# Gnnng/SVDFeature

Hardware: AMD Instinct MI355X
Metric: training instances/sec (SGD updates/s), basicMF k=64 (higher is better)
Workload: dtype f32; 1 GPU; basicMF synthetic 1000000x100000, 100000000 ratings, k=64 fp32 (BASELINE configs[1]); order=uniform random (file order preserved: result == sequential SGD), conflict_free_batches_per_pass=903, parallelism=1 GPU

## Files before the change

include/svdfeature_amd.h:

```cpp
#ifndef SVDFEATURE_AMD_H_
#define SVDFEATURE_AMD_H_

#include <stddef.h>
#include <stdint.h>
#include <stdio.h>

#ifdef __cplusplus
extern "C" {
#endif

typedef struct svdf_trainer svdf_trainer;
typedef struct svdf_dataset svdf_dataset;
typedef struct svdf_ranker svdf_ranker;

const char *svdf_version(void);
void svdf_set_error_mode(int mode);
const char *svdf_last_error(void);
int svdf_device_count(void);

svdf_trainer *svdf_create(uint8_t format_type, uint8_t active_type, uint8_t extend_type, uint8_t variant_type,
                          int device);
void svdf_destroy(svdf_trainer *t);

int svdf_set_param(svdf_trainer *t, const char *name, const char *val);
void svdf_seed(unsigned seed);
int svdf_init_model(svdf_trainer *t);
int svdf_load_model(svdf_trainer *t, FILE *fi);
int svdf_save_model(svdf_trainer *t, FILE *fo);
int svdf_save_model_begin(svdf_trainer *t, FILE *fo);
int svdf_save_model_end(svdf_trainer *t);
int svdf_init_trainer(svdf_trainer *t);
int svdf_set_round(svdf_trainer *t, int nround);
int svdf_finish_round(svdf_trainer *t);

int svdf_update_csr(svdf_trainer *t, float label, int num_global, int num_ufactor, int num_ifactor,
                    const unsigned *index, const float *value);
float svdf_predict_csr(svdf_trainer *t, float label, int num_global, int num_ufactor, int num_ifactor,
                       const unsigned *index, const float *value);
int svdf_update_csr_batch(svdf_trainer *t, int num_row, const float *row_label, const int *row_ptr,
                          const unsigned *feat_index, const float *feat_value);
int svdf_predict_csr_batch(svdf_trainer *t, int num_row, const float *row_label, const int *row_ptr,
                           const unsigned *feat_index, const float *feat_value, float *out);

int svdf_update_block(svdf_trainer *t, int num_ufeedback, int extend_tag,
                      const unsigned *index_ufeedback, const float *value_ufeedback,
                      int num_row, const float *row_label, const int *row_ptr,
                      const unsigned *feat_index, const float *feat_value);
int svdf_predict_block(svdf_trainer *t, int num_ufeedback, int extend_tag,
                       const unsigned *index_ufeedback, const float *value_ufeedback,
                       int num_row, const float *row_label, const int *row_ptr,
                       const unsigned *feat_index, const float *feat_value, float *out);

svdf_dataset *svdf_dataset_from_csr(svdf_trainer *t, long num_row, const float *row_label, const int64_t *row_ptr,
                                    const unsigned *feat_index, const float *feat_value);
svdf_dataset *svdf_dataset_from_triples(svdf_trainer *t, long n, const unsigned *user, const unsigned *item,
                                        const float *label);
svdf_dataset *svdf_dataset_from_pairs(svdf_trainer *t, long n, const unsigned *user, const unsigned *pos_item,
                                      const unsigned *neg_item);
svdf_dataset *svdf_dataset_from_blocks(svdf_trainer *t, long num_block, const int *extend_tag, const int64_t *fb_ptr,
                                       const unsigned *fb_index, const float *fb_value, const int64_t *block_row_ptr,
                                       const float *row_label, const int64_t *row_ptr, const unsigned *feat_index,
                                       const float *feat_value);
svdf_dataset *svdf_dataset_from_buffer_file(svdf_trainer *t, const char *path, int user_group_format);
svdf_dataset *svdf_dataset_from_rank_buffer_file(svdf_trainer *t, const char *path);
int svdf_rank_prefetch_buffer_file(svdf_trainer *t, const char *path);
int64_t svdf_rank_sample_buffer_file(svdf_trainer *t, const char *in_path, const char *out_path);
void svdf_dataset_destroy(svdf_dataset *ds);
int svdf_train_dataset(svdf_trainer *t, svdf_dataset *ds);
int svdf_predict_dataset(svdf_trainer *t, svdf_dataset *ds, float *out);
int64_t svdf_dataset_info(const svdf_dataset *ds, int what);

int svdf_item_delta_begin(svdf_trainer *t);
void *svdf_item_delta_buffer(svdf_trainer *t, int64_t *count);
int svdf_item_delta_apply(svdf_trainer *t);
int svdf_item_delta_export(svdf_trainer *t, float *device_dst);
int svdf_item_delta_import(svdf_trainer *t, const float *device_src);
int svdf_item_delta_into(svdf_trainer *t, float *device_dst, int64_t *count);
int svdf_item_delta_apply_from(svdf_trainer *t, const float *device_src);
int svdf_item_delta_pack(svdf_trainer *t, void *device_dst, int half, int64_t *count);
int svdf_item_delta_select(svdf_trainer *t, int part, int nparts);
int svdf_item_delta_unpack(svdf_trainer *t, const void *device_src, int half, int refresh_snapshot);

svdf_dataset *svdf_dataset_window_from_triples(svdf_trainer *t, long n, const unsigned *user, const unsigned *item, const float *label);
svdf_dataset *svdf_dataset_window_from_pairs(svdf_trainer *t, long n, const unsigned *user, const unsigned *pos_item, const unsigned *neg_item);
svdf_dataset *svdf_dataset_window_from_csr(svdf_trainer *t, long num_row, const float *row_label, const int64_t *row_ptr,
                                           const unsigned *feat_index, const float *feat_value);
svdf_dataset *svdf_dataset_window_from_blocks(svdf_trainer *t, long num_block, const int *extend_tag, const int64_t *fb_ptr,
                                              const unsigned *fb_index, const float *fb_value, const int64_t *block_row_ptr,
                                              const float *row_label, const int64_t *row_ptr, const unsigned *feat_index,
                                              const float *feat_value);
int svdf_window_delta_pack(svdf_trainer *t, svdf_dataset *ds, void *device_dst, int half, int64_t *count);
int svdf_window_delta_apply(svdf_trainer *t, const void *device_src, int half);
int svdf_window_delta_apply_local(svdf_trainer *t, svdf_dataset *ds);
int svdf_item_block_get(svdf_trainer *t, float *device_dst, int64_t *count);
int svdf_item_block_set(svdf_trainer *t, const float *device_src);
int svdf_stratum_step(svdf_trainer *t, svdf_dataset *const *windows, int num_windows, int block, int nblocks, float *device_out);
int svdf_item_block_set_at(svdf_trainer *t, int block, int nblocks, const float *device_src);
int svdf_ipc_setup(svdf_trainer *t, int rank, int world, int64_t wire_bytes, int64_t block_floats, unsigned char *handles_out);
int svdf_ipc_connect(svdf_trainer *t, const unsigned char *all_handles);
int svdf_ipc_window_pack(svdf_trainer *t, svdf_dataset *ds, int half);
int svdf_ipc_window_reduce(svdf_trainer *t, int half);
int svdf_ipc_window_apply(svdf_trainer *t, int half);
int svdf_ipc_block_send(svdf_trainer *t, int dst_rank, int slot);
int svdf_ipc_block_recv(svdf_trainer *t, int src_rank, int slot, unsigned seq);
int svdf_ipc_status(svdf_trainer *t);
int svdf_ipc_close(svdf_trainer *t);

int svdf_rccl_unique_id(unsigned char *out128);
int svdf_rccl_init(svdf_trainer *t, const unsigned char *id128, int rank, int world);
int svdf_rccl_window_allreduce(svdf_trainer *t, svdf_dataset *ds, int half);
int svdf_rccl_block_handoff(svdf_trainer *t, int dst_rank, int src_rank, int slot, int in_block, int nblocks);
int svdf_rccl_block_arrive(svdf_trainer *t, int slot);
int64_t svdf_rccl_counter(svdf_trainer *t, int what);
int svdf_rccl_close(svdf_trainer *t);

int svdf_debug_sort_labels(long n, const float *label, int *restated, int *library);
int svdf_debug_sort_scores(long n, const float *score, int threads, int *parallel, int *library);

int64_t svdf_get_view(svdf_trainer *t, int which, float *out, int64_t capacity);
int svdf_view_shape(svdf_trainer *t, int which, int *rows, int *cols);
int64_t svdf_set_view(svdf_trainer *t, int which, const float *in, int64_t count);
void *svdf_stream(svdf_trainer *t);
int svdf_set_stream(svdf_trainer *t, void *hip_stream);
int svdf_synchronize(svdf_trainer *t);
int64_t svdf_counter(svdf_trainer *t, int what);
int svdf_set_knob(svdf_trainer *t, const char *name, long value);

int svdf_eval_dataset(svdf_trainer *t, svdf_dataset *ds, float scale_score, double *sum_sq_err, int64_t *count);

svdf_ranker *svdf_ranker_create(uint8_t format_type, uint8_t active_type, uint8_t extend_type, uint8_t variant_type, int device);
void svdf_ranker_destroy(svdf_ranker *r);
int svdf_ranker_set_param(svdf_ranker *r, const char *name, const char *val);
int svdf_ranker_load_model(svdf_ranker *r, FILE *fi);
int svdf_ranker_init(svdf_ranker *r, int num_item_set);
int64_t svdf_ranker_process_csr(svdf_ranker *r, float label, int num_global, int num_ufactor, int num_ifactor, const unsigned *index,
                                const float *value, int *out, int64_t capacity);
int64_t svdf_ranker_process_rows(svdf_ranker *r, int num_row, const float *row_label, const int *row_ptr, const unsigned *feat_index,
                                 const float *feat_value, int *out, int64_t capacity);
int64_t svdf_ranker_process_block(svdf_ranker *r, int num_ufeedback, int extend_tag, const unsigned *index_ufeedback,
                                  const float *value_ufeedback, int num_row, const float *row_label, const int *row_ptr,
                                  const unsigned *feat_index, const float *feat_value, int *out, int64_t capacity);
int64_t svdf_ranker_counter(svdf_ranker *r, int what);

int svdf_rand_peek(long n, int *out);
int svdf_rand_skip(long n);

int svdf_device_expf(const float *in, unsigned first_bits, unsigned step_bits, float *out, long n);

int svdf_schedule_resources(long n, const int64_t *res_ptr, const unsigned *res, long num_res, int *order_out,
                            int64_t *level_ptr_out, long level_cap);

#ifdef __cplusplus
}
#endif
#endif
```

svdfeature_amd/__init__.py:

```python
import ctypes as C
import os

import numpy as np

from .data import BlockArrays, CSRData, PlusBlock, pairs_as_csr

HERE = os.path.dirname(os.path.abspath(__file__))
LIB_PATH = os.path.join(HERE, "libsvdfeature_amd.so")
HEADER_PATH = os.path.join(os.path.dirname(HERE), "include", "svdfeature_amd.h")

VIEW = {"u_bias": 0, "W_user": 1, "i_bias": 2, "W_item": 3, "g_bias": 4, "ufeedback_bias": 5, "W_ufeedback": 6}

_u32p = np.ctypeslib.ndpointer(dtype=np.uint32, flags="C_CONTIGUOUS")
_i32p = np.ctypeslib.ndpointer(dtype=np.int32, flags="C_CONTIGUOUS")
_i64p = np.ctypeslib.ndpointer(dtype=np.int64, flags="C_CONTIGUOUS")
_f32p = np.ctypeslib.ndpointer(dtype=np.float32, flags="C_CONTIGUOUS")

_lib = None
_libc = C.CDLL(None)
_libc.fopen.restype = C.c_void_p
_libc.fopen.argtypes = [C.c_char_p, C.c_char_p]
_libc.fclose.argtypes = [C.c_void_p]


class SvdfError(RuntimeError):
    pass


def load_library():
    global _lib
    if _lib is not None:
        return _lib
    if not os.path.exists(LIB_PATH):
        raise SvdfError("%s is missing: run `python -c 'import __graft_entry__ as g; g.build()'` "
                        "(hipcc --offload-arch=gfx950); there is no CPU fallback" % LIB_PATH)
    try:
        import torch
    except ImportError:
        pass
    lib = C.CDLL(LIB_PATH)
    P = C.c_void_p
    lib.svdf_version.restype = C.c_char_p
    lib.svdf_last_error.restype = C.c_char_p
    lib.svdf_set_error_mode.argtypes = [C.c_int]
    lib.svdf_device_count.restype = C.c_int
    lib.svdf_create.restype = P
    lib.svdf_create.argtypes = [C.c_uint8] * 4 + [C.c_int]
    lib.svdf_destroy.argtypes = [P]
    lib.svdf_set_param.argtypes = [P, C.c_char_p, C.c_char_p]
    lib.svdf_seed.argtypes = [C.c_uint]
    for f in ("svdf_init_model", "svdf_init_trainer", "svdf_finish_round", "svdf_synchronize",
              "svdf_item_delta_begin", "svdf_item_delta_apply"):
        getattr(lib, f).argtypes = [P]
    lib.svdf_set_round.argtypes = [P, C.c_int]
    lib.svdf_load_model.argtypes = [P, C.c_void_p]
    lib.svdf_save_model.argtypes = [P, C.c_void_p]
    lib.svdf_save_model_begin.argtypes = [P, C.c_void_p]
    lib.svdf_save_model_end.argtypes = [P]
    lib.svdf_update_csr.argtypes = [P, C.c_float, C.c_int, C.c_int, C.c_int, _u32p, _f32p]
    lib.svdf_predict_csr.argtypes = lib.svdf_update_csr.argtypes
    lib.svdf_predict_csr.restype = C.c_float
    lib.svdf_update_csr_batch.argtypes = [P, C.c_int, _f32p, _i32p, _u32p, _f32p]
    lib.svdf_predict_csr_batch.argtypes = [P, C.c_int, _f32p, _i32p, _u32p, _f32p, _f32p]
    lib.svdf_update_block.argtypes = [P, C.c_int, C.c_int, _u32p, _f32p, C.c_int, _f32p, _i32p, _u32p, _f32p]
    lib.svdf_predict_block.argtypes = lib.svdf_update_block.argtypes + [_f32p]
    lib.svdf_dataset_from_csr.restype = P
    lib.svdf_dataset_from_csr.argtypes = [P, C.c_long, _f32p, _i64p, _u32p, _f32p]
    lib.svdf_dataset_from_triples.restype = P
    lib.svdf_dataset_from_triples.argtypes = [P, C.c_long, _u32p, _u32p, _f32p]
    lib.svdf_dataset_from_pairs.restype = P
    lib.svdf_dataset_from_pairs.argtypes = [P, C.c_long, _u32p, _u32p, _u32p]
    lib.svdf_dataset_window_from_triples.restype = P
    lib.svdf_dataset_window_from_triples.argtypes = [P, C.c_long, _u32p, _u32p, _f32p]
    lib.svdf_dataset_window_from_pairs.restype = P
    lib.svdf_dataset_window_from_pairs.argtypes = [P, C.c_long, _u32p, _u32p, _u32p]
    lib.svdf_dataset_window_from_csr.restype = P
    lib.svdf_dataset_window_from_csr.argtypes = [P, C.c_long, _f32p, _i64p, _u32p, _f32p]
    lib.svdf_dataset_window_from_blocks.restype = P
    lib.svdf_dataset_window_from_blocks.argtypes = [P, C.c_long, _i32p, _i64p, _u32p, _f32p, _i64p, _f32p, _i64p, _u32p, _f32p]
    lib.svdf_ipc_setup.argtypes = [P, C.c_int, C.c_int, C.c_int64, C.c_int64, C.c_char_p]
    lib.svdf_ipc_connect.argtypes = [P, C.c_char_p]
    lib.svdf_ipc_window_pack.argtypes = [P, P, C.c_int]
    lib.svdf_ipc_window_reduce.argtypes = [P, C.c_int]
    lib.svdf_ipc_window_apply.argtypes = [P, C.c_int]
    lib.svdf_ipc_block_send.argtypes = [P, C.c_int, C.c_int]
    lib.svdf_ipc_block_recv.argtypes = [P, C.c_int, C.c_int, C.c_uint]
    lib.svdf_ipc_status.argtypes = [P]
    lib.svdf_ipc_close.argtypes = [P]
    lib.svdf_stratum_step.argtypes = [P, C.POINTER(C.c_void_p), C.c_int, C.c_int, C.c_int, P]
    lib.svdf_item_block_set_at.argtypes = [P, C.c_int, C.c_int, P]
    lib.svdf_rccl_unique_id.argtypes = [C.c_char_p]
    lib.svdf_rccl_init.argtypes = [P, C.c_char_p, C.c_int, C.c_int]
    lib.svdf_rccl_window_allreduce.argtypes = [P, P, C.c_int]
    lib.svdf_rccl_block_handoff.argtypes = [P, C.c_int, C.c_int, C.c_int, C.c_int, C.c_int]
    lib.svdf_rccl_block_arrive.argtypes = [P, C.c_int]
    lib.svdf_rccl_counter.restype = C.c_int64
    lib.svdf_rccl_counter.argtypes = [P, C.c_int]
    lib.svdf_rccl_close.argtypes = [P]
    lib.svdf_window_delta_pack.argtypes = [P, P, P, C.c_int, C.POINTER(C.c_int64)]
    lib.svdf_window_delta_apply.argtypes = [P, P, C.c_int]
    lib.svdf_window_delta_apply_local.argtypes = [P, P]
    lib.svdf_item_block_get.argtypes = [P, P, C.POINTER(C.c_int64)]
    lib.svdf_item_block_set.argtypes = [P, P]
    lib.svdf_set_view.restype = C.c_int64
    lib.svdf_set_view.argtypes = [P, C.c_int, _f32p, C.c_int64]
    lib.svdf_dataset_from_buffer_file.restype = P
    lib.svdf_dataset_from_buffer_file.argtypes = [P, C.c_char_p, C.c_int]
    lib.svdf_dataset_from_rank_buffer_file.restype = P
    lib.svdf_dataset_from_rank_buffer_file.argtypes = [P, C.c_char_p]
    lib.svdf_rank_prefetch_buffer_file.restype = C.c_int
    lib.svdf_rank_prefetch_buffer_file.argtypes = [P, C.c_char_p]
    lib.svdf_rank_sample_buffer_file.restype = C.c_int64
    lib.svdf_rank_sample_buffer_file.argtypes = [P, C.c_char_p, C.c_char_p]
    lib.svdf_dataset_from_blocks.restype = P
    lib.svdf_dataset_from_blocks.argtypes = [P, C.c_long, _i32p, _i64p, _u32p, _f32p, _i64p, _f32p, _i64p, _u32p, _f32p]
    lib.svdf_dataset_destroy.argtypes = [P]
    lib.svdf_train_dataset.argtypes = [P, P]
    lib.svdf_predict_dataset.argtypes = [P, P, _f32p]
    lib.svdf_dataset_info.restype = C.c_int64
    lib.svdf_dataset_info.argtypes = [P, C.c_int]
    lib.svdf_item_delta_buffer.restype = P
    lib.svdf_item_delta_buffer.argtypes = [P, C.POINTER(C.c_int64)]
    lib.svdf_item_delta_export.argtypes = [P, P]
    lib.svdf_item_delta_import.argtypes = [P, P]
    lib.svdf_item_delta_into.argtypes = [P, P, C.POINTER(C.c_int64)]
    lib.svdf_item_delta_apply_from.argtypes = [P, P]
    lib.svdf_item_delta_pack.argtypes = [P, P, C.c_int, C.POINTER(C.c_int64)]
    lib.svdf_item_delta_unpack.argtypes = [P, P, C.c_int, C.c_int]
    lib.svdf_set_stream.argtypes = [P, P]
    lib.svdf_item_delta_select.argtypes = [P, C.c_int, C.c_int]
    lib.svdf_get_view.restype = C.c_int64
    lib.svdf_get_view.argtypes = [P, C.c_int, _f32p, C.c_int64]
    lib.svdf_view_shape.argtypes = [P, C.c_int, C.POINTER(C.c_int), C.POINTER(C.c_int)]
    lib.svdf_stream.restype = P
    lib.svdf_stream.argtypes = [P]
    lib.svdf_counter.restype = C.c_int64
    lib.svdf_counter.argtypes = [P, C.c_int]
    lib.svdf_set_knob.argtypes = [P, C.c_char_p, C.c_long]
    lib.svdf_schedule_resources.argtypes = [C.c_long, _i64p, _u32p, C.c_long, _i32p, _i64p, C.c_long]
    lib.svdf_eval_dataset.argtypes = [P, P, C.c_float, C.POINTER(C.c_double), C.POINTER(C.c_int64)]
    lib.svdf_ranker_create.restype = P
    lib.svdf_ranker_create.argtypes = [C.c_uint8] * 4 + [C.c_int]
    lib.svdf_ranker_destroy.argtypes = [P]
    lib.svdf_ranker_set_param.argtypes = [P, C.c_char_p, C.c_char_p]
    lib.svdf_ranker_load_model.argtypes = [P, C.c_void_p]
    lib.svdf_ranker_init.argtypes = [P, C.c_int]
    lib.svdf_ranker_process_csr.restype = C.c_int64
    lib.svdf_ranker_process_csr.argtypes = [P, C.c_float, C.c_int, C.c_int, C.c_int, _u32p, _f32p, _i32p, C.c_int64]
    lib.svdf_ranker_process_rows.restype = C.c_int64
    lib.svdf_ranker_process_rows.argtypes = [P, C.c_int, _f32p, _i32p, _u32p, _f32p, _i32p, C.c_int64]
    lib.svdf_ranker_process_block.restype = C.c_int64
    lib.svdf_ranker_process_block.argtypes = [P, C.c_int, C.c_int, _u32p, _f32p, C.c_int, _f32p, _i32p, _u32p, _f32p, _i32p, C.c_int64]
    lib.svdf_ranker_counter.restype = C.c_int64
    lib.svdf_ranker_counter.argtypes = [P, C.c_int]
    lib.svdf_rand_peek.argtypes = [C.c_long, _i32p]
    lib.svdf_rand_skip.argtypes = [C.c_long]
    lib.svdf_device_expf.argtypes = [C.c_void_p, C.c_uint, C.c_uint, _f32p, C.c_long]
    lib.svdf_debug_sort_labels.argtypes = [C.c_long, _f32p, _i32p, _i32p]
    lib.svdf_debug_sort_scores.argtypes = [C.c_long, _f32p, C.c_int, _i32p, _i32p]
    lib.svdf_set_error_mode(1)
    _lib = lib
    return lib


def device_count():
    return load_library().svdf_device_count()


def rccl_unique_id():
    buf = C.create_string_buffer(128)
    if load_library().svdf_rccl_unique_id(buf) != 0:
        raise SvdfError(load_library().svdf_last_error().decode())
    return buf.raw


def rand_peek(n):
    out = np.zeros(max(int(n), 1), np.int32)
    if load_library().svdf_rand_peek(int(n), out) != 0:
        raise SvdfError(load_library().svdf_last_error().decode())
    return out[:n]


def rand_skip(n):
    if load_library().svdf_rand_skip(int(n)) != 0:
        raise SvdfError(load_library().svdf_last_error().decode())


def debug_sort_labels(label):
    label = np.ascontiguousarray(label, np.float32)
    a, b = np.zeros(max(len(label), 1), np.int32), np.zeros(max(len(label), 1), np.int32)
    if load_library().svdf_debug_sort_labels(len(label), _pad(label, np.float32), a, b) != 0:
        raise SvdfError(load_library().svdf_last_error().decode())
    return a[:len(label)], b[:len(label)]


def debug_sort_scores(score, threads=8):
    score = np.ascontiguousarray(score, np.float32)
    a, b = np.zeros(max(len(score), 1), np.int32), np.zeros(max(len(score), 1), np.int32)
    if load_library().svdf_debug_sort_scores(len(score), _pad(score, np.float32), int(threads), a, b) != 0:
        raise SvdfError(load_library().svdf_last_error().decode())
    return a[:len(score)], b[:len(score)]


def device_expf(x=None, first=0, step=1, n=None):
    lib = load_library()
    if x is not None:
        x = np.ascontiguousarray(x, np.float32)
        out = np.empty(len(x), np.float32)
        rc = lib.svdf_device_expf(x.ctypes.data_as(C.c_void_p), 0, 0, out, len(x))
    else:
        out = np.empty(n, np.float32)
        rc = lib.svdf_device_expf(None, first, step, out, n)
    if rc != 0:
        raise SvdfError("svdf_device_expf failed")
    return out


def _pad(a, dtype):
    a = np.ascontiguousarray(a, dtype=dtype)
    return a if a.size else np.zeros(1, dtype=dtype)


def schedule_resources(res_ptr, res, num_res):
    lib = load_library()
    n = len(res_ptr) - 1
    order = np.zeros(max(n, 1), np.int32)
    level_ptr = np.zeros(n + 2, np.int64)
    nl = lib.svdf_schedule_resources(n, _pad(res_ptr, np.int64), _pad(res, np.uint32), int(num_res), order, level_ptr, n + 2)
    if nl < 0:
        raise SvdfError(lib.svdf_last_error().decode())
    return order[:n], level_ptr[:nl + 1]


class Dataset:

    def __init__(self, trainer, handle):
        self.trainer, self.h = trainer, handle

    def info(self, what):
        return int(self.trainer.lib.svdf_dataset_info(self.h, what))

    num_row = property(lambda s: s.info(0))
    num_batches = property(lambda s: s.info(1))
    max_batch = property(lambda s: s.info(2))
    kind = property(lambda s: s.info(3))
    algorithmic_bytes = property(lambda s: s.info(4))
    num_units = property(lambda s: s.info(5))
    num_simple_units = property(lambda s: s.info(6))

    def close(self):
        if self.h:
            self.trainer.lib.svdf_dataset_destroy(self.h)
            self.h = None

    def __del__(self):
        try:
            self.close()
        except Exception:
            pass


class Trainer:

    def __init__(self, format_type=0, active_type=0, extend_type=0, variant_type=0, params=None, device=-1):
        self.lib = load_library()
        self.h = self.lib.svdf_create(format_type, active_type, extend_type, variant_type, device)
        if not self.h:
            raise SvdfError(self.lib.svdf_last_error().decode())
        self.mtype = bytes([format_type, active_type, extend_type, variant_type])
        for k, v in (params or {}).items():
            self.set_param(k, v)

    def _ok(self, rc):
        if rc != 0:
            raise SvdfError(self.lib.svdf_last_error().decode())

    def close(self):
        if getattr(self, "h", None):
            if getattr(self, "_async_fo", None) is not None:
                try:
                    self.save_model_end()
                except Exception:
                    pass
            self.lib.svdf_destroy(self.h)
            self.h = None

    def __del__(self):
        try:
            self.close()
        except Exception:
            pass

    def set_param(self, name, val):
        self._ok(self.lib.svdf_set_param(self.h, str(name).encode(), str(val).encode()))

    def seed(self, s):
        self.lib.svdf_seed(int(s))

    def init_model(self):
        self._ok(self.lib.svdf_init_model(self.h))

    def init_trainer(self):
        self._ok(self.lib.svdf_init_trainer(self.h))

    def set_round(self, r):
        self._ok(self.lib.svdf_set_round(self.h, int(r)))

    def finish_round(self):
        self._ok(self.lib.svdf_finish_round(self.h))

    def save_model_begin(self, path, with_type_header=True):
        assert getattr(self, "_async_fo", None) is None, "one asynchronous save at a time"
        fo = _libc.fopen(str(path).encode(), b"wb")
        if not fo:
            raise SvdfError("can not open file \"%s\"" % path)
        if with_type_header:
            hdr = (C.c_char * 4).from_buffer_copy(self.mtype)
            _libc.fwrite(hdr, 1, 4, C.c_void_p(fo))
        self._async_fo = fo
        try:
            self._ok(self.lib.svdf_save_model_begin(self.h, fo))
        except Exception:
            _libc.fclose(fo)
            self._async_fo = None
            raise

    def save_model_end(self):
        fo = getattr(self, "_async_fo", None)
        if fo is None:
            return
        try:
            self._ok(self.lib.svdf_save_model_end(self.h))
        finally:
            _libc.fclose(fo)
            self._async_fo = None

    def save_model(self, path, with_type_header=True):
        fo = _libc.fopen(str(path).encode(), b"wb")
        if not fo:
            raise SvdfError("can not open file \"%s\"" % path)
        try:
            if with_type_header:
                hdr = (C.c_char * 4).from_buffer_copy(self.mtype)
                _libc.fwrite(hdr, 1, 4, C.c_void_p(fo))
            self._ok(self.lib.svdf_save_model(self.h, fo))
        finally:
            _libc.fclose(fo)

    def load_model(self, path, with_type_header=True):
        fi = _libc.fopen(str(path).encode(), b"rb")
        if not fi:
            raise SvdfError("can not open file \"%s\"" % path)
        try:
            if with_type_header:
                buf = (C.c_char * 4)()
                _libc.fread(buf, 1, 4, C.c_void_p(fi))
            self._ok(self.lib.svdf_load_model(self.h, fi))
        finally:
            _libc.fclose(fi)

    def update_csr(self, label, ng, nu, ni, index, value):
        self._ok(self.lib.svdf_update_csr(self.h, float(label), ng, nu, ni, _pad(index, np.uint32), _pad(value, np.float32)))

    def predict_csr(self, label, ng, nu, ni, index, value):
        self.lib.svdf_last_error()
        return self.lib.svdf_predict_csr(self.h, float(label), ng, nu, ni, _pad(index, np.uint32), _pad(value, np.float32))

    def update_batch(self, d):
        self._ok(self.lib.svdf_update_csr_batch(self.h, d.num_row, _pad(d.row_label, np.float32), _pad(d.row_ptr, np.int32),
                                                _pad(d.feat_index, np.uint32), _pad(d.feat_value, np.float32)))

    def predict_batch(self, d):
        out = np.zeros(max(d.num_row, 1), dtype=np.float32)
        self._ok(self.lib.svdf_predict_csr_batch(self.h, d.num_row, _pad(d.row_label, np.float32), _pad(d.row_ptr, np.int32),
                                                 _pad(d.feat_index, np.uint32), _pad(d.feat_value, np.float32), out))
        return out[:d.num_row]

    def update_block(self, b):
        d = b.data
        self._ok(self.lib.svdf_update_block(self.h, b.num_ufeedback, b.extend_tag, _pad(b.index_ufeedback, np.uint32),
                                            _pad(b.value_ufeedback, np.float32), d.num_row, _pad(d.row_label, np.float32),
                                            _pad(d.row_ptr, np.int32), _pad(d.feat_index, np.uint32), _pad(d.feat_value, np.float32)))

    def predict_block(self, b):
        d = b.data
        out = np.zeros(max(d.num_row, 1), dtype=np.float32)
        self._ok(self.lib.svdf_predict_block(self.h, b.num_ufeedback, b.extend_tag, _pad(b.index_ufeedback, np.uint32),
                                             _pad(b.value_ufeedback, np.float32), d.num_row, _pad(d.row_label, np.float32),
                                             _pad(d.row_ptr, np.int32), _pad(d.feat_index, np.uint32), _pad(d.feat_value, np.float32), out))
        return out[:d.num_row]

    def dataset_from_csr(self, d):
        h = self.lib.svdf_dataset_from_csr(self.h, d.num_row, _pad(d.row_label, np.float32), _pad(d.row_ptr, np.int64),
                                           _pad(d.feat_index, np.uint32), _pad(d.feat_value, np.float32))
        if not h:
            raise SvdfError(self.lib.svdf_last_error().decode())
        return Dataset(self, h)

    def dataset_from_triples(self, user, item, label):
        n = len(label)
        h = self.lib.svdf_dataset_from_triples(self.h, n, _pad(user, np.uint32), _pad(item, np.uint32), _pad(label, np.float32))
# ... 321 lines not shown
```

svdfeature_amd/csrc/svdf_capi.cpp:

```cpp
#include <svdfeature_amd.h>

#include <algorithm>
#include <cstdlib>
#include <cstring>
#include <new>
#include <vector>

#include "svdf_engine.h"
#include "svdf_kernels.h"

namespace svdf {
void set_error_mode(int m);
const char *last_error();
void note_error(const std::string &m);
}

struct svdf_trainer { svdf::Engine *e; };
struct svdf_dataset { svdf::Dataset *d; };
struct svdf_ranker { svdf::Ranker *r; };

#define SVDF_GUARD(retval, ...)                                 \
    try { __VA_ARGS__; }                                        \
    catch (const std::exception &ex) { svdf::note_error(ex.what()); return retval; } \
    catch (...) { svdf::note_error("unknown error"); return retval; }

extern "C" {

const char *svdf_version(void) { return "svdfeature_amd 0.1 (gfx950)"; }
void svdf_set_error_mode(int mode) { svdf::set_error_mode(mode); }
const char *svdf_last_error(void) { return svdf::last_error(); }
int svdf_device_count(void) {
    int n = 0;
    if (hipGetDeviceCount(&n) != hipSuccess) return 0;
    return n;
}

svdf_trainer *svdf_create(uint8_t format_type, uint8_t active_type, uint8_t extend_type, uint8_t variant_type, int device) {
    SVDF_GUARD(nullptr, {
        svdf::TypeParam tp{format_type, active_type, extend_type, variant_type};
        svdf_trainer *t = new svdf_trainer();
        t->e = nullptr;
        try { t->e = new svdf::Engine(tp, device); } catch (...) { delete t; throw; }
        return t;
    })
}
void svdf_destroy(svdf_trainer *t) {
    if (!t) return;
    try { delete t->e; } catch (...) {}
    delete t;
}
int svdf_set_param(svdf_trainer *t, const char *name, const char *val) { SVDF_GUARD(-1, { t->e->set_param(name, val); return 0; }) }
void svdf_seed(unsigned seed) { srand(seed); }
int svdf_init_model(svdf_trainer *t) { SVDF_GUARD(-1, { t->e->init_model(); return 0; }) }
int svdf_load_model(svdf_trainer *t, FILE *fi) { SVDF_GUARD(-1, { t->e->load_model(fi); return 0; }) }
int svdf_save_model(svdf_trainer *t, FILE *fo) { SVDF_GUARD(-1, { t->e->save_model(fo); return 0; }) }
int svdf_save_model_begin(svdf_trainer *t, FILE *fo) { SVDF_GUARD(-1, { t->e->save_model_begin(fo); return 0; }) }
int svdf_save_model_end(svdf_trainer *t) { SVDF_GUARD(-1, { t->e->save_model_end(); return 0; }) }
int svdf_init_trainer(svdf_trainer *t) { SVDF_GUARD(-1, { t->e->init_trainer(); return 0; }) }
int svdf_set_round(svdf_trainer *t, int nround) { SVDF_GUARD(-1, { t->e->set_round(nround); return 0; }) }
int svdf_finish_round(svdf_trainer *t) { SVDF_GUARD(-1, { t->e->finish_round(); return 0; }) }

int svdf_update_csr(svdf_trainer *t, float label, int ng, int nu, int ni, const unsigned *index, const float *value) {
    SVDF_GUARD(-1, { t->e->update_csr(label, ng, nu, ni, index, value); return 0; })
}
float svdf_predict_csr(svdf_trainer *t, float label, int ng, int nu, int ni, const unsigned *index, const float *value) {
    SVDF_GUARD(0.0f, { return t->e->predict_csr(label, ng, nu, ni, index, value); })
}
int svdf_update_csr_batch(svdf_trainer *t, int num_row, const float *row_label, const int *row_ptr,
                          const unsigned *feat_index, const float *feat_value) {
    SVDF_GUARD(-1, { t->e->update_csr_batch(num_row, row_label, row_ptr, feat_index, feat_value); return 0; })
}
int svdf_predict_csr_batch(svdf_trainer *t, int num_row, const float *row_label, const int *row_ptr,
                           const unsigned *feat_index, const float *feat_value, float *out) {
    SVDF_GUARD(-1, { t->e->predict_csr_batch(num_row, row_label, row_ptr, feat_index, feat_value, out); return 0; })
}
int svdf_update_block(svdf_trainer *t, int nfb, int tag, const unsigned *ifb, const float *vfb, int num_row,
                      const float *row_label, const int *row_ptr, const unsigned *feat_index, const float *feat_value) {
    SVDF_GUARD(-1, { t->e->update_block(nfb, tag, ifb, vfb, num_row, row_label, row_ptr, feat_index, feat_value); return 0; })
}
int svdf_predict_block(svdf_trainer *t, int nfb, int tag, const unsigned *ifb, const float *vfb, int num_row,
                       const float *row_label, const int *row_ptr, const unsigned *feat_index, const float *feat_value, float *out) {
    SVDF_GUARD(-1, { t->e->predict_block(nfb, tag, ifb, vfb, num_row, row_label, row_ptr, feat_index, feat_value, out); return 0; })
}

svdf_dataset *svdf_dataset_from_csr(svdf_trainer *t, long num_row, const float *row_label, const int64_t *row_ptr,
                                    const unsigned *feat_index, const float *feat_value) {
    SVDF_GUARD(nullptr, {
        svdf::Dataset *d = t->e->dataset_from_csr(num_row, row_label, row_ptr, feat_index, feat_value);
        t->e->note_dataset(d);
        svdf_dataset *h = new svdf_dataset();
        h->d = d;
        return h;
    })
}
svdf_dataset *svdf_dataset_from_triples(svdf_trainer *t, long n, const unsigned *user, const unsigned *item, const float *label) {
    SVDF_GUARD(nullptr, {
        svdf::Dataset *d = t->e->dataset_from_triples(n, user, item, label);
        t->e->note_dataset(d);
        svdf_dataset *h = new svdf_dataset();
        h->d = d;
        return h;
    })
}
svdf_dataset *svdf_dataset_window_from_triples(svdf_trainer *t, long n, const unsigned *user, const unsigned *item, const float *label) {
    SVDF_GUARD(nullptr, {
        svdf::Dataset *d = t->e->dataset_window_from_triples(n, user, item, label);
        svdf_dataset *h = new svdf_dataset();
        h->d = d;
        return h;
    })
}
svdf_dataset *svdf_dataset_window_from_pairs(svdf_trainer *t, long n, const unsigned *user, const unsigned *pos_item, const unsigned *neg_item) {
    SVDF_GUARD(nullptr, {
        svdf::Dataset *d = t->e->dataset_window_from_pairs(n, user, pos_item, neg_item);
        svdf_dataset *h = new svdf_dataset();
        h->d = d;
        return h;
    })
}
svdf_dataset *svdf_dataset_window_from_csr(svdf_trainer *t, long num_row, const float *row_label, const int64_t *row_ptr, const unsigned *feat_index,
                                           const float *feat_value) {
    SVDF_GUARD(nullptr, {
        svdf::Dataset *d = t->e->dataset_window_from_csr(num_row, row_label, row_ptr, feat_index, feat_value);
        svdf_dataset *h = new svdf_dataset();
        h->d = d;
        return h;
    })
}
svdf_dataset *svdf_dataset_window_from_blocks(svdf_trainer *t, long num_block, const int *extend_tag, const int64_t *fb_ptr, const unsigned *fb_index,
                                              const float *fb_value, const int64_t *block_row_ptr, const float *row_label, const int64_t *row_ptr,
                                              const unsigned *feat_index, const float *feat_value) {
    SVDF_GUARD(nullptr, {
        svdf::Dataset *d = t->e->dataset_window_from_blocks(num_block, extend_tag, fb_ptr, fb_index, fb_value, block_row_ptr, row_label, row_ptr, feat_index, feat_value);
        svdf_dataset *h = new svdf_dataset();
        h->d = d;
        return h;
    })
}
int svdf_ipc_setup(svdf_trainer *t, int rank, int world, int64_t wire_bytes, int64_t block_floats, unsigned char *handles_out) { SVDF_GUARD(-1, { t->e->ipc_setup(rank, world, wire_bytes, block_floats, handles_out); return 0; }) }
int svdf_ipc_connect(svdf_trainer *t, const unsigned char *all_handles) { SVDF_GUARD(-1, { t->e->ipc_connect(all_handles); return 0; }) }
int svdf_ipc_window_pack(svdf_trainer *t, svdf_dataset *ds, int half) { SVDF_GUARD(-1, { t->e->ipc_window_pack(ds ? ds->d : nullptr, half); return 0; }) }
int svdf_ipc_window_reduce(svdf_trainer *t, int half) { SVDF_GUARD(-1, { t->e->ipc_window_reduce(half); return 0; }) }
int svdf_ipc_window_apply(svdf_trainer *t, int half) { SVDF_GUARD(-1, { t->e->ipc_window_apply(half); return 0; }) }
int svdf_ipc_block_send(svdf_trainer *t, int dst_rank, int slot) { SVDF_GUARD(-1, { t->e->ipc_block_send(dst_rank, slot); return 0; }) }
int svdf_ipc_block_recv(svdf_trainer *t, int src_rank, int slot, unsigned seq) { SVDF_GUARD(-1, { t->e->ipc_block_recv(src_rank, slot, seq); return 0; }) }
int svdf_ipc_status(svdf_trainer *t) { SVDF_GUARD(-1, { return t->e->ipc_status(); }) }
int svdf_ipc_close(svdf_trainer *t) { SVDF_GUARD(-1, { t->e->ipc_close(); return 0; }) }
int svdf_rccl_unique_id(unsigned char *out128) { SVDF_GUARD(-1, { svdf::rccl_unique_id(out128); return 0; }) }
int svdf_rccl_init(svdf_trainer *t, const unsigned char *id128, int rank, int world) { SVDF_GUARD(-1, { t->e->rccl_init(id128, rank, world); return 0; }) }
int svdf_rccl_window_allreduce(svdf_trainer *t, svdf_dataset *ds, int half) { SVDF_GUARD(-1, { t->e->rccl_window_allreduce(ds ? ds->d : nullptr, half); return 0; }) }
int svdf_rccl_block_handoff(svdf_trainer *t, int dst_rank, int src_rank, int slot, int in_block, int nblocks) { SVDF_GUARD(-1, { t->e->rccl_block_handoff(dst_rank, src_rank, slot, in_block, nblocks); return 0; }) }
int svdf_rccl_block_arrive(svdf_trainer *t, int slot) { SVDF_GUARD(-1, { t->e->rccl_block_arrive(slot); return 0; }) }
int64_t svdf_rccl_counter(svdf_trainer *t, int what) { SVDF_GUARD(-1, { return t->e->rccl_counter(what); }) }
int svdf_rccl_close(svdf_trainer *t) { SVDF_GUARD(-1, { t->e->rccl_close(); return 0; }) }
int svdf_window_delta_pack(svdf_trainer *t, svdf_dataset *ds, void *dst, int half, int64_t *count) {
    SVDF_GUARD(-1, { t->e->per_rank_api(); t->e->window_delta_pack(ds ? ds->d : nullptr, dst, half, count); return 0; })
}
int svdf_window_delta_apply_local(svdf_trainer *t, svdf_dataset *ds) { SVDF_GUARD(-1, { t->e->per_rank_api(); t->e->window_delta_apply_local(ds ? ds->d : nullptr); return 0; }) }
int svdf_item_block_get(svdf_trainer *t, float *dst, int64_t *count) { SVDF_GUARD(-1, { t->e->per_rank_api(); t->e->item_block_copy(dst, 0, count); return 0; }) }
int svdf_stratum_step(svdf_trainer *t, svdf_dataset *const *windows, int num_windows, int block, int nblocks, float *device_out) {
    SVDF_GUARD(-1, {
        t->e->per_rank_api();
// ... 37 lines not shown
        return h;
    })
}
svdf_dataset *svdf_dataset_from_blocks(svdf_trainer *t, long num_block, const int *extend_tag, const int64_t *fb_ptr,
                                       const unsigned *fb_index, const float *fb_value, const int64_t *block_row_ptr,
                                       const float *row_label, const int64_t *row_ptr, const unsigned *feat_index,
                                       const float *feat_value) {
    SVDF_GUARD(nullptr, {
        svdf::Dataset *d = t->e->dataset_from_blocks(num_block, extend_tag, fb_ptr, fb_index, fb_value, block_row_ptr, row_label, row_ptr,
                                                     feat_index, feat_value);
        t->e->note_dataset(d);
        svdf_dataset *h = new svdf_dataset();
        h->d = d;
        return h;
    })
}
svdf_dataset *svdf_dataset_from_buffer_file(svdf_trainer *t, const char *path, int user_group_format) {
    SVDF_GUARD(nullptr, {
        svdf::Dataset *d = t->e->dataset_from_buffer_file(path, user_group_format);
        t->e->note_dataset(d);
        svdf_dataset *h = new svdf_dataset();
        h->d = d;
        return h;
    })
}
svdf_dataset *svdf_dataset_from_rank_buffer_file(svdf_trainer *t, const char *path) {
    SVDF_GUARD(nullptr, {
        svdf::Dataset *d = t->e->dataset_from_rank_buffer_file(path);
        t->e->note_dataset(d);
        svdf_dataset *h = new svdf_dataset();
        h->d = d;
        return h;
    })
}
int svdf_rank_prefetch_buffer_file(svdf_trainer *t, const char *path) { SVDF_GUARD(-1, { t->e->rank_prefetch(path); return 0; }) }
int64_t svdf_rank_sample_buffer_file(svdf_trainer *t, const char *in_path, const char *out_path) {
    SVDF_GUARD(-1, { return (int64_t)t->e->rank_sample_buffer_file(in_path, out_path); })
}
void svdf_dataset_destroy(svdf_dataset *ds) {
    if (!ds) return;
    try { if (ds->d && ds->d->owner) ds->d->owner->synchronize(); } catch (...) {}
    delete ds->d;
    delete ds;
}
int svdf_train_dataset(svdf_trainer *t, svdf_dataset *ds) { SVDF_GUARD(-1, { t->e->train_dataset(ds->d); return 0; }) }
int svdf_predict_dataset(svdf_trainer *t, svdf_dataset *ds, float *out) { SVDF_GUARD(-1, { t->e->predict_dataset(ds->d, out); return 0; }) }
int64_t svdf_dataset_info(const svdf_dataset *ds, int what) {
    if (!ds || !ds->d) return -1;
    switch (what) {
    case 0: return ds->d->num_row;
    case 1: return ds->d->kind == 8 ? (int64_t)ds->d->wchild.size() : (int64_t)ds->d->sched.num_levels();
    case 2: return ds->d->sched.max_level_size;
    case 3: return ds->d->kind;
    case 4: return ds->d->algorithmic_bytes;
    case 5: return ds->d->num_units;
    case 6: return ds->d->num_simple_units;
    case 7: {
        uint64_t h = 1469598103934665603ull;
        auto mix = [&h](uint64_t v) { for (int b = 0; b < 8; b++) { h ^= (v >> (8 * b)) & 0xFFu; h *= 1099511628211ull; } };
        for (long v : ds->d->sched.level_ptr) mix((uint64_t)v);
        for (long v : ds->d->sched.level_mid) mix((uint64_t)v);
        for (int v : ds->d->sched.order) mix((uint64_t)(unsigned)v);
        return (int64_t)(h >> 1);
    }
    default: return -1;
    }
}

int svdf_item_delta_begin(svdf_trainer *t) { SVDF_GUARD(-1, { t->e->per_rank_api(); t->e->item_delta_begin(); return 0; }) }
void *svdf_item_delta_buffer(svdf_trainer *t, int64_t *count) { SVDF_GUARD(nullptr, { t->e->per_rank_api(); return t->e->item_delta_buffer(count); }) }
int svdf_item_delta_apply(svdf_trainer *t) { SVDF_GUARD(-1, { t->e->per_rank_api(); t->e->item_delta_apply(); return 0; }) }
int svdf_item_delta_export(svdf_trainer *t, float *dst) { SVDF_GUARD(-1, { t->e->per_rank_api(); t->e->item_delta_copy(dst, nullptr); return 0; }) }
int svdf_item_delta_import(svdf_trainer *t, const float *src) { SVDF_GUARD(-1, { t->e->per_rank_api(); t->e->item_delta_copy(nullptr, src); return 0; }) }

int svdf_item_delta_into(svdf_trainer *t, float *dst, int64_t *count) { SVDF_GUARD(-1, { t->e->per_rank_api(); t->e->item_delta_into(dst, count); return 0; }) }
int svdf_item_delta_pack(svdf_trainer *t, void *dst, int half, int64_t *count) { SVDF_GUARD(-1, { t->e->per_rank_api(); t->e->item_delta_pack(dst, half, count); return 0; }) }
int svdf_item_delta_unpack(svdf_trainer *t, const void *src, int half, int refresh_snapshot) {
    SVDF_GUARD(-1, { t->e->per_rank_api(); t->e->item_delta_unpack(src, half, refresh_snapshot); return 0; })
}
int svdf_item_delta_select(svdf_trainer *t, int part, int nparts) { SVDF_GUARD(-1, { t->e->per_rank_api(); t->e->item_delta_select(part, nparts); return 0; }) }
int svdf_item_delta_apply_from(svdf_trainer *t, const float *src) { SVDF_GUARD(-1, { t->e->per_rank_api(); t->e->item_delta_apply_from(src); return 0; }) }
int svdf_set_stream(svdf_trainer *t, void *hip_stream) { SVDF_GUARD(-1, { t->e->set_stream((hipStream_t)hip_stream); return 0; }) }

int64_t svdf_get_view(svdf_trainer *t, int which, float *out, int64_t capacity) { SVDF_GUARD(-1, { return t->e->get_view(which, out, capacity); }) }
int64_t svdf_set_view(svdf_trainer *t, int which, const float *in, int64_t count) { SVDF_GUARD(-1, { return t->e->set_view(which, in, count); }) }
int svdf_view_shape(svdf_trainer *t, int which, int *rows, int *cols) { SVDF_GUARD(-1, { t->e->view_shape(which, rows, cols); return 0; }) }
void *svdf_stream(svdf_trainer *t) { return (void *)t->e->stream(); }
int svdf_synchronize(svdf_trainer *t) { SVDF_GUARD(-1, { t->e->synchronize(); return 0; }) }
int64_t svdf_counter(svdf_trainer *t, int what) { return t->e->counter(what); }
int svdf_set_knob(svdf_trainer *t, const char *name, long value) { SVDF_GUARD(-1, { return t->e->set_knob(name, value); }) }

int svdf_eval_dataset(svdf_trainer *t, svdf_dataset *ds, float scale_score, double *sum_sq_err, int64_t *count) {
    SVDF_GUARD(-1, { t->e->eval_dataset(ds->d, scale_score, sum_sq_err, count); return 0; })
}

svdf_ranker *svdf_ranker_create(uint8_t format_type, uint8_t active_type, uint8_t extend_type, uint8_t variant_type, int device) {
    SVDF_GUARD(nullptr, {
        svdf::TypeParam tp{format_type, active_type, extend_type, variant_type};
        svdf_ranker *h = new svdf_ranker();
        h->r = nullptr;
        try { h->r = new svdf::Ranker(tp, device); } catch (...) { delete h; throw; }
        return h;
    })
}
void svdf_ranker_destroy(svdf_ranker *r) {
    if (!r) return;
    try { delete r->r; } catch (...) {}
    delete r;
}
int svdf_ranker_set_param(svdf_ranker *r, const char *name, const char *val) { SVDF_GUARD(-1, { r->r->set_param(name, val); return 0; }) }
int svdf_ranker_load_model(svdf_ranker *r, FILE *fi) { SVDF_GUARD(-1, { r->r->load_model(fi); return 0; }) }
int svdf_ranker_init(svdf_ranker *r, int num_item_set) { SVDF_GUARD(-1, { r->r->init_ranker(num_item_set); return 0; }) }
int64_t svdf_ranker_process_csr(svdf_ranker *r, float label, int ng, int nu, int ni, const unsigned *index, const float *value, int *out,
                                int64_t capacity) {
    SVDF_GUARD(-1, { return (int64_t)r->r->process(label, ng, nu, ni, index, value, out, (long)capacity); })
}
int64_t svdf_ranker_process_rows(svdf_ranker *r, int num_row, const float *row_label, const int *row_ptr, const unsigned *feat_index,
                                 const float *feat_value, int *out, int64_t capacity) {
    SVDF_GUARD(-1, { return (int64_t)r->r->process_rows(num_row, row_label, row_ptr, feat_index, feat_value, out, (long)capacity); })
}
int64_t svdf_ranker_process_block(svdf_ranker *r, int nfb, int tag, const unsigned *ifb, const float *vfb, int num_row, const float *row_label,
                                  const int *row_ptr, const unsigned *feat_index, const float *feat_value, int *out, int64_t capacity) {
    SVDF_GUARD(-1, { return (int64_t)r->r->process_block(nfb, tag, ifb, vfb, num_row, row_label, row_ptr, feat_index, feat_value, out, (long)capacity); })
}
int64_t svdf_ranker_counter(svdf_ranker *r, int what) { return r->r->counter(what); }

int svdf_rand_peek(long n, int *out) { SVDF_GUARD(-1, { svdf::libc_rand_peek(n, out); return 0; }) }
int svdf_rand_skip(long n) { SVDF_GUARD(-1, { svdf::libc_rand_skip(n); return 0; }) }

int svdf_device_expf(const float *in, unsigned first_bits, unsigned step_bits, float *out, long n) {
    SVDF_GUARD(-1, { return svdf::device_expf(in, first_bits, step_bits, out, n); })
}

int svdf_schedule_resources(long n, const int64_t *res_ptr, const unsigned *res, long num_res, int *order_out,
                            int64_t *level_ptr_out, long level_cap) {
    SVDF_GUARD(-1, {
        std::vector<int> last((size_t)num_res, 0), levels((size_t)n);
        for (long r = 0; r < n; r++) {
            int l = 0;
            for (int64_t j = res_ptr[r]; j < res_ptr[r + 1]; j++) l = std::max(l, last[res[j]]);
            l += 1;
            for (int64_t j = res_ptr[r]; j < res_ptr[r + 1]; j++) last[res[j]] = l;
            levels[(size_t)r] = l;
        }
        svdf::Schedule s;
        svdf::build_schedule(levels, 0, s);
        if ((long)s.num_levels() + 1 > level_cap) return -2;
        for (long r = 0; r < n; r++) order_out[r] = s.order[(size_t)r];
        for (size_t l = 0; l <= s.num_levels(); l++) level_ptr_out[l] = s.level_ptr[l];
        return (int)s.num_levels();
    })
}

}
```

svdfeature_amd/csrc/svdf_config.cpp:

```cpp
#include "svdf_engine.h"

#include <algorithm>
#include <chrono>
#include <cmath>
#include <cstdlib>
#include <cstring>
#include <memory>
#include <mutex>
#include <atomic>
#include <thread>

#include "svdf_kernels.h"
#include "svdf_internal.h"

namespace svdf {

void ParamSet::set_param(const char *name, const char *val) {
    if (!strncmp(name, prefix_a.c_str(), prefix_a.size())) name += prefix_a.size();
    else if (!strncmp(name, prefix_b.c_str(), prefix_b.size())) name += prefix_b.size();
    else return;
    if (!strcmp("bound", name)) {
        unsigned bd = (unsigned)atoi(val);
        check(bd > 0, "can't give 0 as bound");
        check(bound.empty() || bound.back() < bd, "bound must be given in order");
// ... 51 lines not shown
const KeyRow<TrainParam> kTrainKeys[] = {
    KF(TrainParam, "learning_rate", learning_rate),
    KF(TrainParam, "wd_user", wd_user), KF(TrainParam, "wd_item", wd_item), KF2(TrainParam, "wd_uiset", wd_user, wd_item),
    KF(TrainParam, "wd_user_bias", wd_user_bias), KF(TrainParam, "wd_item_bias", wd_item_bias), KF2(TrainParam, "wd_uiset_bias", wd_user_bias, wd_item_bias),
    KF(TrainParam, "wd_global", wd_global),
    KI(TrainParam, "reg_method", reg_method), KI(TrainParam, "reg_global", reg_global), KU(TrainParam, "num_regfree_global", num_regfree_global),
    KI(TrainParam, "decay_learning_rate", decay_learning_rate), KF(TrainParam, "min_learning_rate", min_learning_rate), KF(TrainParam, "decay_rate", decay_rate),
    KF(TrainParam, "scale_lr_ufeedback", scale_lr_ufeedback), KF(TrainParam, "wd_ufeedback", wd_ufeedback), KF(TrainParam, "wd_ufeedback_bias", wd_ufeedback_bias),
};
const KeyRow<ModelParam> kModelKeys[] = {
    KI(ModelParam, "num_user", num_user), KI(ModelParam, "num_item", num_item), KI2(ModelParam, "num_uiset", num_user, num_item),
    KI(ModelParam, "num_global", num_global), KI(ModelParam, "num_factor", num_factor), KI(ModelParam, "num_ufeedback", num_ufeedback),
    KF(ModelParam, "u_init_sigma", u_init_sigma), KF(ModelParam, "i_init_sigma", i_init_sigma), KF2(ModelParam, "ui_init_sigma", u_init_sigma, i_init_sigma),
    KF(ModelParam, "ufeedback_init_sigma", ufeedback_init_sigma), KF(ModelParam, "base_score", base_score), KI(ModelParam, "no_user_bias", no_user_bias),
    KI(ModelParam, "num_randinit_ufactor", num_randinit_ufactor), KI(ModelParam, "num_randinit_ifactor", num_randinit_ifactor),
    KI2(ModelParam, "num_randinit_uifactor", num_randinit_ifactor, num_randinit_ufactor),
    KI(ModelParam, "common_latent_space", common_latent_space), KI(ModelParam, "common_feedback_space", common_feedback_space),
    KI(ModelParam, "user_nonnegative", user_nonnegative), KI(ModelParam, "item_nonnegative", item_nonnegative),
};
#undef KF
#undef KF2
#undef KI
#undef KI2
#undef KU
}
void config_set_train_param(TrainParam &p, const char *name, const char *val) { apply_key(kTrainKeys, sizeof(kTrainKeys) / sizeof(kTrainKeys[0]), p, name, val); }
void config_set_model_param(ModelParam &p, const char *name, const char *val) { apply_key(kModelKeys, sizeof(kModelKeys) / sizeof(kModelKeys[0]), p, name, val); }

void Engine::set_param(const char *name, const char *val) {
    if (save_async_.active) save_model_end();
    if (trainer_ready_ && !host_only_) flush();
    if (!strcmp(name, "amd:gpus")) {
        check(!multi_ && !space_allocated_, "amd:gpus must be set before the model is created");
        check(atoi(val) <= 1 || !shared_user(), "amd:shared_user_from: one GPU only (amd:gpus = 1); the N-rank exchange has no place for user rows");
        gpus_ = std::max(1, atoi(val));
    }
    else if (!is_peer_) param_log_.emplace_back(name, val);
    if (!strcmp(name, "amd:delta_half")) delta_half_ = atoi(val) != 0;
    if (!strcmp(name, "amd:exchange")) {
        check(!strcmp(val, "p2p") || !strcmp(val, "rccl"), "amd:exchange must be p2p or rccl");
        check(!multi_, "amd:exchange must be set before the model is created");
        multi_exchange_mode_ = !strcmp(val, "rccl") ? 1 : 0;
    }
    if (!strcmp(name, "amd:step")) {
        check(!strcmp(val, "minibatch") || !strcmp(val, "levels") || !strcmp(val, "auto"), "amd:step must be minibatch, levels or auto");
        check(!multi_, "amd:step must be set before the model is created");
        multi_step_levels_ = !strcmp(val, "levels");
        step_minibatch_set_ = !strcmp(val, "minibatch");
        step_auto_set_ = !strcmp(val, "auto");
    }
    if (!strcmp(name, "amd:contrib")) {
        check(!strcmp(val, "fp32") || !strcmp(val, "bf16"), "amd:contrib must be fp32 or bf16");
        contrib_bf16_ = !strcmp(val, "bf16");
    }
    if (!strcmp(name, "amd:window")) { stage_window_ = std::max<long>(1, atol(val)); window_set_ = true; }
    if (!strcmp(name, "amd:window_per_target")) { check(atoi(val) >= 1, "amd:window_per_target must be positive"); wseq_per_target_ = atoi(val); }
    if (!strcmp(name, "amd:window_per_target_max")) { check(atoi(val) >= 1, "amd:window_per_target_max must be positive"); wseq_per_target_max_ = atoi(val); }
    if (multi_) for (int d = 1; d < gpus_; d++) rank_engine(d)->set_param(name, val);
    if (!strcmp(name, "feature_user")) name_feat_user_ = val;
    if (!strcmp(name, "feature_item")) name_feat_item_ = val;
    if (imfb() && !strcmp(name, "ufeedback_disable_level")) {
        const int level = atoi(val);
        check(level >= 0, "ufeedback_disable_level must not be negative");
        if (level < 32) imfb_disable_ |= 1u << level;
    }
    if (bilinear()) {
        if (!strcmp(name, "reg_bi_feedback")) reg_bi_feedback_ = atoi(val);
        if (!bi_allocated_) {
            if (!strcmp(name, "num_bi_feedback")) bi_param_.num_bi_feedback = atoi(val);
            if (!strcmp(name, "start_ufeedback")) bi_param_.start_ufeedback = atoi(val);
        }
    }
    if (!strcmp(name, "amd:relax_global")) relax_global_ = atoi(val) != 0;
    if (!strcmp(name, "amd:relax_feedback")) relax_feedback_ = atoi(val) != 0;
    if (!strcmp(name, "amd:relax_user_from")) relax_user_from_ = (unsigned)strtoul(val, nullptr, 10);
    if (!strcmp(name, "amd:relax_item_from")) relax_item_from_ = (unsigned)strtoul(val, nullptr, 10);
    if (!strcmp(name, "amd:shared_user_from")) {
        const long b = atol(val);
        check(b >= 1 && b < 0xFFFFFFFFL, "amd:shared_user_from must be in 1 .. num_user");
        check(gpus_ == 1 && !multi_, "amd:shared_user_from: one GPU only (amd:gpus = 1); the N-rank exchange has no place for user rows");
        check(!space_allocated_ || b <= (long)mp_.num_user, "amd:shared_user_from must be in 1 .. num_user");
        shared_user_from_ = (unsigned)b;
    }
    pair_sampler_.set_param(name, val);
    config_set_train_param(tp_, name, val);
    u_param_.set_param(name, val);
    i_param_.set_param(name, val);
    g_param_.set_param(name, val);
    if (!space_allocated_) config_set_model_param(mp_, name, val);
    params_dirty_ = true;
}
int64_t Engine::counter(int what) const {
    switch (what) {
    case 0: return n_instances_;
    case 1: return n_launches_;
    case 2: return n_batches_;
    case 3: return n_flushes_;
    case 4: return n_kind_[0];
    case 5: return n_kind_[1];
    case 6: return n_kind_[2];
    case 7: return n_device_rank_passes_;
    case 8: return multi_counter(0);
    case 9: return multi_counter(1);
    case 10: return multi_counter(2);
    case 11: return multi_counter(3);
    case 12: return multi_counter(4);
    case 13: return n_init_reports_;
    case 14: return n_init_draws_;
    case 15: return n_chained_levels_;
    case 16: return auto_last_.decided;
    case 17: return auto_last_.levels;
    case 18: return (int64_t)(auto_last_.dag_ms * 1000.0);
    case 19: return (int64_t)(auto_last_.stream_ms * 1000.0);
    case 20: return auto_last_.windows;
    case 23: return n_runs_passes_;
    case 22: return n_pivot_passes_;
    case 24: return unit_sched_us_;
    case 25: return unit_sched_on_device_ ? 1 : 0;
    case 26: return n_guard_warnings_;
    case 27: return (int64_t)(guard_last_.dag_ms * 1000.0);
    case 28: return (int64_t)(guard_last_.stream_ms * 1000.0);
    case 29: return n_punit_passes_;
    case 21: return 0;
    default: return -1;
    }
}
int Engine::set_knob(const char *name, long value) {
    launch_version_++;
    if (multi_ && !is_peer_ && strcmp(name, "stage_window") != 0 && strcmp(name, "async_flush") != 0)
        for (int d = 1; d < gpus_; d++) (void)rank_engine(d)->set_knob(name, value);
    if (!strcmp(name, "use_graph")) { use_graph_ = value != 0; return 0; }
    if (!strcmp(name, "stage_window")) { check(value >= 1, "stage_window must be >= 1"); stage_window_ = value; window_set_ = true; return 0; }
    if (!strcmp(name, "groups_per_wave")) {
        check(value >= 0 && value <= 8 && value != 7, "groups_per_wave must be 0 (auto), 1 ... 6 or 8");
        groups_per_wave_ = (int)value;
        return 0;
    }
    if (!strcmp(name, "xcd_remap")) { xcd_remap_ = value != 0; params_dirty_ = true; return 0; }
    if (!strcmp(name, "fewrow_i16")) { check(value >= 0 && value <= 1, "fewrow_i16 must be 0 or 1"); fewrow_i16_ = (int)value; params_dirty_ = true; return 0; }
    if (!strcmp(name, "svdpp_helpers")) { check(value == 1 || value == 4 || value == 8 || value == 16, "svdpp_helpers must be 1, 4, 8 or 16"); svdpp_helpers_ = (int)value; params_dirty_ = true; return 0; }
    if (!strcmp(name, "basic_i8")) { check(value >= 0 && value <= 1, "basic_i8 must be 0 or 1"); basic_i8_ = (int)value; params_dirty_ = true; return 0; }
    if (!strcmp(name, "load_mode")) { check(value >= 0 && value <= 2, "load_mode must be 0, 1 or 2 (auto)"); load_mode_ = (int)value; params_dirty_ = true; return 0; }
    if (!strcmp(name, "store_mode")) { check(value >= 0 && value <= 2, "store_mode must be 0, 1 or 2"); store_mode_ = (int)value; params_dirty_ = true; return 0; }
    if (!strcmp(name, "sort_batches")) { check(value >= 0 && value <= 2, "sort_batches must be 0, 1 (by item) or 2 (by user)"); sort_batches_ = (int)value; return 0; }
    if (!strcmp(name, "async_flush")) { flush(); async_flush_ = value != 0; return 0; }
    if (!strcmp(name, "use_fused")) { use_fused_ = value != 0; return 0; }
    if (!strcmp(name, "device_schedule")) { device_sched_ = value != 0; return 0; }
    if (!strcmp(name, "device_rank")) { device_rank_ = value != 0; return 0; }
    if (!strcmp(name, "device_init")) { device_init_ = value != 0; return 0; }
    if (!strcmp(name, "device_window")) { device_window_ = value != 0; return 0; }
    if (!strcmp(name, "device_load")) { device_load_ = value != 0; return 0; }
    if (!strcmp(name, "runs_exec")) { check(value == 0 || value == 1, "runs_exec must be 0 or 1"); runs_exec_ = (int)value; return 0; }
    if (!strcmp(name, "runs_len")) { check(value >= 2 && value <= 7, "runs_len must be in 2 .. 7"); runs_len_ = (int)value; return 0; }
    if (!strcmp(name, "runs_sets")) { check(value >= 1 && value <= 2, "runs_sets must be 1 or 2"); runs_sets_ = (int)value; return 0; }
    if (!strcmp(name, "runs_block")) { check(value == 64 || value == 128 || value == 256, "runs_block must be 64, 128 or 256"); runs_block_ = (int)value; return 0; }
    if (!strcmp(name, "runs_min_rows")) { check(value >= 0, "runs_min_rows must not be negative"); runs_min_rows_ = value; return 0; }
    if (!strcmp(name, "pair_units")) { check(value == 0 || value == 1, "pair_units must be 0 or 1"); pair_units_ = (int)value; return 0; }
    if (!strcmp(name, "pair_unit_cap")) { check(value >= 1 && value <= 4096, "pair_unit_cap must be in 1 .. 4096"); pair_unit_cap_ = (int)value; return 0; }
    if (!strcmp(name, "pivot_exec")) { check(value == 0 || value == 1, "pivot_exec must be 0 or 1"); pivot_exec_ = (int)value; return 0; }
    if (!strcmp(name, "pivot_run")) { check(value >= 1 && value <= 65536, "pivot_run must be in 1 .. 65536"); pivot_run_ = (int)value; return 0; }
    if (!strcmp(name, "pivot_min")) { check(value >= 2, "pivot_min must be at least 2"); pivot_min_ = (int)value; return 0; }
    if (!strcmp(name, "ipc_spin_limit")) { ipc_set_spin_limit(value); return 0; }
    if (!strcmp(name, "chain_width")) { check(value >= 0, "chain_width must not be negative"); chain_width_ = value; return 0; }
    if (!strcmp(name, "device_init_margin_log2")) { check(value >= 8 && value <= 52, "device_init_margin_log2 must be in 8 .. 52"); device_init_margin_log2_ = (int)value; return 0; }
    if (!strcmp(name, "device_schedule_min")) { check(value >= 1, "device_schedule_min must be >= 1"); device_sched_min_ = value; return 0; }
    if (!strcmp(name, "use_simple_units")) { use_simple_units_ = value != 0; return 0; }
    if (!strcmp(name, "rows_without_feedback")) { rows_without_feedback_ = value != 0; return 0; }
    if (!strcmp(name, "fewrow_gslots")) { fewrow_gslots_ = value != 0; launch_version_++; return 0; }
    if (!strcmp(name, "wunit_inplace")) { wunit_inplace_ = value != 0; return 0; }
    if (!strcmp(name, "wunit_defer_fb")) { wunit_defer_fb_ = value != 0; return 0; }
    if (!strcmp(name, "wunit_fast")) { check(value >= 0 && value <= 2, "wunit_fast must be 0, 1 or 2"); wunit_fast_ = (int)value; return 0; }
    if (!strcmp(name, "window_per_target_child")) { check(value >= 1, "window_per_target_child must be positive"); wseq_per_target_child_ = (int)value; return 0; }
    if (!strcmp(name, "window_per_target_shared")) { check(value >= 1, "window_per_target_shared must be positive"); wseq_per_target_shared_ = (int)value; return 0; }
    if (!strcmp(name, "window_per_target_fb")) { check(value >= 1, "window_per_target_fb must be positive"); wseq_per_target_fb_ = (int)value; return 0; }
    if (!strcmp(name, "window_shared_sub")) { check(value >= 0 && value <= 4096, "window_shared_sub must be in 0 .. 4096"); wseq_shared_sub_ = (int)value; return 0; }
    if (!strcmp(name, "window_shared_max")) { check(value >= 1, "window_shared_max must be positive"); wseq_shared_max_ = (int)value; return 0; }
    if (!strcmp(name, "window_hot_sub")) { check(value >= 0 && value <= 4096, "window_hot_sub must be in 0 .. 4096"); wseq_hot_sub_ = (int)value; return 0; }
    if (!strcmp(name, "window_hot_max")) { check(value >= 1, "window_hot_max must be positive"); wseq_hot_max_ = (int)value; return 0; }
    if (!strcmp(name, "window_per_target_max")) { check(value >= 1, "window_per_target_max must be positive"); wseq_per_target_max_ = (int)value; return 0; }
    if (!strcmp(name, "window_per_target")) { check(value >= 1, "window_per_target must be positive"); wseq_per_target_ = (int)value; return 0; }
    if (!strcmp(name, "window_slots")) { window_slots_ = value != 0; return 0; }
    if (!strcmp(name, "window_groups")) { check(value >= 0 && value <= 2, "window_groups must be 0 (auto), 1 or 2"); window_groups_ = (int)value; return 0; }
    if (!strcmp(name, "block_threads")) {
        check(value == 0 || value == 64 || value == 128 || value == 256, "block_threads must be 0 (auto), 64, 128 or 256");
        block_threads_ = (int)value;
        return 0;
    }
    return -1;
}

}
```

svdfeature_amd/csrc/svdf_dataset.cpp:

```cpp
#include "svdf_engine.h"

#include <algorithm>
#include <chrono>
#include <cmath>
#include <cstdlib>
#include <cstring>
#include <memory>
#include <mutex>
#include <atomic>
#include <thread>

#include "svdf_kernels.h"
#include "svdf_internal.h"

namespace svdf {

Dataset *Engine::dataset_from_blocks(long num_block, const int *extend_tag, const int64_t *fb_ptr, const unsigned *fb_index, const float *fb_value,
                                     const int64_t *block_row_ptr, const float *row_label, const int64_t *row_ptr, const unsigned *feat_index,
                                     const float *feat_value) {
    check(trainer_ready_, "dataset: init_trainer has not been called");
    need_device("dataset");
    check(user_group(), "svdfeature_amd: block datasets are for user-group (format_type 1) trainers");
    if (multi_ && !in_multi_scope()) {
        check(mp_.common_feedback_space == 0, "svdfeature_amd: amd:gpus > 1 needs a feedback space of its own (common_feedback_space = 0)");
// ... 431 lines not shown
        }
    }
    if (!basic && device_sched_ && n > 0 && fused_allowed() && !user_group() && !relaxed())
        if (Dataset *d = dataset_fewrow_on_device(n, row_label, row_ptr, feat_index, feat_value)) return d;
    std::unique_ptr<Dataset> ds(new Dataset());
    adopt(ds.get()); ds->num_row = n;
    std::vector<int> levels((size_t)n);
    LevelTracker saved;
    std::swap(saved, tracker_);
    tracker_.resize(num_resources() + 1);
    long nnz = 0, nrows_touched = 0, nbias = 0, ng_total = 0;
    for (long r = 0; r < n; r++) {
        const int64_t *p = row_ptr + 3 * r;
        const unsigned *ig = feat_index + p[0], *iu = feat_index + p[1], *ii = feat_index + p[2];
        const int ng = (int)(p[1] - p[0]), nu = (int)(p[2] - p[1]), ni = (int)(p[3] - p[2]);
        const int lvl = level_of_row(ig, ng, iu, nu, ii, ni, 0) + 1;
        touch_row(ig, ng, iu, nu, ii, ni, lvl);
        levels[(size_t)r] = lvl;
        long nc_u = 0, nc_i = 0;
        for (int j = 0; j < nu; j++) if (iu[j] < feat_user_.num_row()) nc_u += feat_user_.row_ptr[iu[j] + 1] - feat_user_.row_ptr[iu[j]];
        for (int j = 0; j < ni; j++) if (ii[j] < feat_item_.num_row()) nc_i += feat_item_.row_ptr[ii[j] + 1] - feat_item_.row_ptr[ii[j]];
        nnz += ng + nu + ni; ng_total += ng;
        nrows_touched += nu + ni + nc_u + nc_i;
        nbias += (mp_.no_user_bias ? 0 : nu + nc_u) + ni + nc_i;
    }
    std::swap(saved, tracker_);
    build_schedule(levels, 0, ds->sched);
    ds->algorithmic_bytes = 8L * mp_.num_factor * nrows_touched + 8 * nbias + 8 * ng_total + 16 * n + 8 * nnz;
    if (basic) {
        ds->kind = 0; ds->unit_values = false;
        const int *order = ds->sched.order.data();
        std::vector<unsigned> tu((size_t)n), ti((size_t)n);
        std::vector<float> tl((size_t)n), tva((size_t)n), tvb((size_t)n);
        for (long s = 0; s < n; s++) {
            const int64_t p = row_ptr[3 * (long)order[s]];
            tu[(size_t)s] = feat_index[p]; ti[(size_t)s] = feat_index[p + 1];
            tva[(size_t)s] = feat_value[p]; tvb[(size_t)s] = feat_value[p + 1];
            tl[(size_t)s] = row_label[order[s]];
        }
        ds->user.upload(tu.data(), (size_t)n, stream_); ds->item.upload(ti.data(), (size_t)n, stream_);
        ds->label.upload(tl.data(), (size_t)n, stream_);
        ds->uval.upload(tva.data(), (size_t)n, stream_); ds->ival.upload(tvb.data(), (size_t)n, stream_);
        HIPCHECK(hipStreamSynchronize(stream_));
        return ds.release();
    }
    {
        FusedHost fh;
        if (fused_allowed() && fused_shape_ok(n, row_ptr, feat_index, fh)) {
            ds->kind = 2;
            if (sort_batches_ != 0) {
                std::vector<unsigned> key((size_t)n, 0u);
                for (long r = 0; r < n; r++) {
                    const int64_t *p = row_ptr + 3 * r;
                    if (relax_user_from_ != 0xFFFFFFFFu) {
                        key[(size_t)r] = (p[2] - p[1] == 2 && feat_index[p[1] + 1] >= relax_user_from_) ? feat_index[p[1] + 1] : 0xFFFFFFFFu;
                    } else if (sort_batches_ == 1 && p[3] > p[2]) key[(size_t)r] = feat_index[p[2]];
                    else if (sort_batches_ == 2 && p[2] > p[1]) key[(size_t)r] = feat_index[p[1]];
                }
                sort_batches(ds->sched, key.data());
            }
            fill_fused(n, row_label, row_ptr, feat_index, feat_value, ds->sched.order.data(), fh);
            ds->fused.upload(fh, stream_);
            HIPCHECK(hipStreamSynchronize(stream_));
            return ds.release();
        }
    }
    check(!relaxed(), "svdfeature_amd: relaxed shared ids need few-row instances (at most 2 user and 2 item ids, no side tables)");
    ds->kind = 1;
    std::vector<int> ptr32((size_t)3 * n + 1);
    for (long j = 0; j <= 3 * n; j++) ptr32[(size_t)j] = (int)(row_ptr[j] - p00);
    ds->row_label.upload(row_label, (size_t)n, stream_);
    ds->row_ptr.upload(ptr32.data(), ptr32.size(), stream_);
    ds->feat_index.upload(feat_index + p00, (size_t)ptr32.back(), stream_);
    ds->feat_value.upload(feat_value + p00, (size_t)ptr32.back(), stream_);
    ds->order.upload(ds->sched.order.data(), (size_t)n, stream_);
    HIPCHECK(hipStreamSynchronize(stream_));
    return ds.release();
}

static void auto_measures(const Dataset *ex, long &levels, double &unit_us, double &dag_ms, double &stream_ms, int pivot_run = 256) {
    levels = (long)ex->sched.num_levels();
    const long units = ex->kind == 3 || ex->kind == 4 ? std::max<long>(ex->num_units, 1) : std::max<long>(ex->num_row, 1);
    unit_us = (ex->kind == 3 || ex->kind == 4) ? 5.0 + 0.42 * (double)ex->num_row / (double)units : (ex->kind == 9 ? 5.0 + 0.3 * pivot_run : (ex->kind == 10 ? 6.0 : (ex->kind == 11 ? 3.0 + 0.7 * (double)ex->num_row / (double)std::max<long>(ex->num_units, 1) : 4.5)));
    dag_ms = (double)levels * unit_us * 1e-3;
    stream_ms = (double)ex->algorithmic_bytes / (0.57 * 8.0e12) * 1e3;
}
bool Engine::auto_probe_deep(Dataset *probe, long n_full) {
    std::unique_ptr<Dataset> p(probe);
    long levels; double unit_us, dag_ms, stream_ms;
    auto_measures(p.get(), levels, unit_us, dag_ms, stream_ms);
    if (dag_ms <= 16.0 * stream_ms) return false;
    const double scale = (double)n_full / (double)std::max<long>(p->num_row, 1);
    auto_probe_ = AutoDecision();
    auto_probe_.levels = (long)((double)levels * scale);
    auto_probe_.dag_ms = dag_ms * scale;
    auto_probe_.stream_ms = stream_ms * scale;
    auto_probe_.decided = -1;
    return true;
}
Dataset *Engine::auto_step(Dataset *exact, bool window_ok, const std::function<Dataset *()> &build_window) {
    std::unique_ptr<Dataset> ex(exact);
    AutoDecision D;
    double unit_us = 4.5;
    const bool from_probe = !ex;
    if (from_probe) { D = auto_probe_; D.decided = 0; }
    else auto_measures(ex.get(), D.levels, unit_us, D.dag_ms, D.stream_ms, pivot_run_);
    const bool deep = D.dag_ms > 2.0 * D.stream_ms;
    const char *why;
    if (!deep) { D.decided = 1; why = "exact levels kept (wide enough to stream)"; }
    else if (!window_ok) { D.decided = 3; why = "exact levels kept: the dependency depth binds, but the window step does not cover this configuration / these rows"; }
    else { D.decided = 2; why = "window step chosen: the dependency depth of exact sequential semantics binds"; }
    Dataset *out = ex.get();
    if (D.decided == 2) {
        ex.reset();
        out = build_window();
        D.windows = (long)out->wchild.size();
    } else {
        ex.release();
    }
    auto_last_ = D;
    if (!getenv("SVDF_QUIET"))
        fprintf(stderr, "[svdfeature_amd] amd:step = auto: %ld rows, %s%ld conflict-free levels: dag bound %.2f ms, stream model %.2f ms -> %s%s\n",
                (long)out->num_row, from_probe ? "extrapolated from the first 2 M rows: ~" : "", D.levels, D.dag_ms, D.stream_ms, why,
                D.decided == 2 ? (" (" + std::to_string(D.windows) + " windows)").c_str() : "");
    return out;
}

std::string Engine::path_for(const Dataset *ds) const {
    const DevParams &P = const_cast<Engine *>(this)->params();
    const long L = (long)ds->sched.num_levels();
    char buf[512];
    auto levels = [&](const char *what) { snprintf(buf, sizeof(buf), "exact, %ld conflict-free levels: %s", L, what); return std::string(buf); };
    switch (ds->kind) {
    case 0: return levels(chain_width_ > 0 ? "contract kernel k_basicmf / k_basicmf_slots, one (user, item) instance per lane group; narrow levels chained (k_basicmf_slots_chain)"
                                           : "contract kernel k_basicmf / k_basicmf_slots, one (user, item) instance per lane group");
    case 1: return levels("general sparse kernel k_general (any number of ids per row, side tables, lazy decay)");
    case 2: {
        const FusedSchedule S = ds->fused.view();
        if (fewrow_gslots_ && fewrow_fast_ && fewrow_gslots_applies(P, S, ds->fused.max_nu, ds->fused.max_ni, ds->fused.dense_slots))
            return levels("few-row kernel with global ids k_fewrow_gslots (neighbourhood shape)");
        return levels(fewrow_fast_ && fewrow_fast_applies(P, S) ? "few-row kernel k_fewrow_slots (<= 2 user + 2 item rows per instance: rank pairs, side ids); narrow levels chained"
                                                                 : "fused few-row kernel k_fused");
    }
    case 3: snprintf(buf, sizeof(buf), "exact, %ld conflict-free levels of user units: k_svdpp_wave (one wave per user, %ld of %ld units) + k_svdpp (general units)",
                     L, ds->num_simple_units, ds->num_units); return buf;
    case 4: return levels("multi-level implicit feedback units k_imfb");
    case 5: return "window data set (one window of the window-minibatch step, user side exact): k_window_users / k_window_items";
    case 6: return "amd:gpus handle: per-rank windows (svdf_multi.cpp)";
    case 7: return "window data set of user units: k_wunit_* (svdf_k_wunit.hip)";
    case 8: snprintf(buf, sizeof(buf), "window sequence (amd:step = minibatch / auto): %zu windows, each trained and applied in place%s; NOT the reference's sequential semantics (|dRMSE| <= 1e-4 contract)",
                     ds->wchild.size(), side_tables() ? ", feature_user / feature_item children as shared rows (general walk k_wunit_walk)" : ""); return buf;
    case 9: snprintf(buf, sizeof(buf), "exact, %ld levels: hot rows walked as units (k_svdpp_wave on %s parameters, %ld units) + cold ratings through the contract kernel",
                     L, ds->pv_item_pivot ? "transposed" : "plain", ds->num_units); return buf;
    case 10: snprintf(buf, sizeof(buf), "exact, %ld levels of runs: k_basicmf_runs_soa (up to %d consecutive ratings of one item per lane group, the item's row in registers)", L, ds->rn_len); return buf;
    case 11: snprintf(buf, sizeof(buf), "exact, %ld levels of user-run units: k_pair_units (%ld units of up to %d consecutive pairs of one user, the user's row in registers)",
                      L, ds->num_units, pair_unit_cap_); return buf;
    default: return "unknown";
    }
}
void Engine::note_dataset(Dataset *ds) {
    if (!ds || host_only_ || is_peer_) return;
    const bool verbose = getenv("SVDF_VERBOSE") != nullptr, quiet = getenv("SVDF_QUIET") != nullptr;
    if (verbose && !quiet) fprintf(stderr, "[svdfeature_amd] data set of %ld rows -> %s\n", (long)ds->num_row, path_for(ds).c_str());
    if (step_auto_set_ || step_minibatch_set_ || multi_ || gpus_ != 1) return;
    if (!(ds->kind == 0 || ds->kind == 1 || ds->kind == 2 || ds->kind == 3 || ds->kind == 4 || ds->kind == 9 || ds->kind == 10 || ds->kind == 11) || ds->num_row <= 0) return;
    AutoDecision D;
    double unit_us = 4.5;
    auto_measures(ds, D.levels, unit_us, D.dag_ms, D.stream_ms, pivot_run_);
    guard_last_ = D;
    if (D.dag_ms <= 10.0 * D.stream_ms || D.dag_ms < 50.0) return;
    n_guard_warnings_++;
    if (quiet) return;
    const bool window_ok = wunit_config_ok() && (ds->kind == 3 || ds->kind == 4 || basic_fast_path_allowed());
    fprintf(stderr, "[svdfeature_amd] default (exact) step: %ld rows in %ld conflict-free levels -- the data's dependency depth binds: about %.0f ms per pass "
                    "(%.2f M rows/s; levels x %.1f us) against %.1f ms if the rows streamed.  The exact pass keeps the reference's sequential result bit for bit; "
                    "%s\n",
            (long)ds->num_row, D.levels, D.dag_ms, (double)ds->num_row / D.dag_ms * 1e-3, unit_us, D.stream_ms,
            window_ok ? "`amd:step = auto` would train this data set with the window step (user side exact, shared rows once per window; |dRMSE| <= 1e-4 contract) near the streaming rate"
                      : "the window step of `amd:step = auto` does not cover this configuration");
}

Dataset::~Dataset() {
    for (auto &per_rank : mchild) for (Dataset *c : per_rank) delete c;
    for (Dataset *c : wchild) delete c;
    if (graph_exec) (void)hipGraphExecDestroy(graph_exec);
    if (owner) owner->disown(this);
}
void Engine::adopt(Dataset *ds) { ds->owner = this; ds->sched_signature = schedule_signature(); datasets_.push_back(ds); }
uint64_t Engine::schedule_signature() const {
    uint64_t h = 1469598103934665603ull;
    auto mix = [&](uint64_t v) { h = (h ^ v) * 1099511628211ull; };
    mix(relax_global_); mix(relax_feedback_); mix(relax_user_from_); mix(relax_item_from_);
    mix(feat_user_.num_row()); mix(feat_user_.index.size()); mix(feat_item_.num_row()); mix(feat_item_.index.size());
    mix(user_group()); mix(lazy_decay()); mix((uint64_t)mp_.num_factor); mix(use_fused_); mix(use_simple_units_);
    mix((uint64_t)mtype_.extend_type);
    if (shared_user()) mix(0x5u + ((uint64_t)shared_user_from_ << 8));
    return h;
}
void Engine::disown(Dataset *ds) {
    if (window_trained_ == ds) window_trained_ = nullptr;
    for (size_t i = 0; i < datasets_.size(); i++)
        if (datasets_[i] == ds) { datasets_[i] = datasets_.back(); datasets_.pop_back(); break; }
}

void Engine::predict_dataset(Dataset *ds, float *out) {
    check(ds && ds->owner == this, "predict_dataset: dataset belongs to another trainer");
    check(ds->kind != 7 && ds->kind != 8, "predict_dataset: window data sets are training sets (their rows are regrouped by user); score rows with svdf_predict_csr_batch / svdf_predict_block or a level-scheduled data set of the same rows");
    check(ds->kind != 5 && ds->kind != 6, "predict_dataset: window / multi-GPU data sets are training sets (their rows are regrouped: there is no file order to report predictions in); svdf_eval_dataset gives their squared error, svdf_predict_csr_batch scores rows (routed to the owner of each user)");
    check(ds->sched_signature == schedule_signature(),
          "predict_dataset: the dataset was scheduled under another configuration; build it again");
    flush();
    const DevParams &P = params();
    const long n = ds->num_row;
    if (n == 0) return;
    w_out_.reserve((size_t)n);
    if (ds->kind == 4) {
        const UnitDev &d = ds->unitdev;
        launch_imfb(P, d.csr(), d.units.p, d.blks.p, d.fbidx.p, d.fbval.p, nullptr, 0, ds->num_units, sample_counter_, w_out_.p, stream_);
        HIPCHECK(hipMemcpyAsync(out, w_out_.p, (size_t)n * sizeof(float), hipMemcpyDeviceToHost, stream_));
        HIPCHECK(hipStreamSynchronize(stream_));
    } else if (ds->kind == 3) {
        const UnitDev &d = ds->unitdev;
        const DevCSR D = d.csr();
        launch_svdpp_predict(P, D, d.units.p, d.fbidx.p, d.fbval.p, ds->num_units, w_out_.p, stream_);
        HIPCHECK(hipMemcpyAsync(out, w_out_.p, (size_t)n * sizeof(float), hipMemcpyDeviceToHost, stream_));
        HIPCHECK(hipStreamSynchronize(stream_));
    } else if (ds->kind == 11) {
        punit_predict(ds, w_out_.p);
        HIPCHECK(hipMemcpyAsync(out, w_out_.p, (size_t)n * sizeof(float), hipMemcpyDeviceToHost, stream_));
        HIPCHECK(hipStreamSynchronize(stream_));
    } else if (ds->kind == 10) {
        BasicSchedule S{ds->user.p, ds->item.p, ds->label.p, nullptr, nullptr};
        launch_predict_basic(P, S, n, w_out_.p, stream_);
        HIPCHECK(hipMemcpyAsync(out, w_out_.p, (size_t)n * sizeof(float), hipMemcpyDeviceToHost, stream_));
        HIPCHECK(hipStreamSynchronize(stream_));
    } else if (ds->kind == 0 || ds->kind == 2 || ds->kind == 9) {
        if (ds->kind != 2) {
            BasicSchedule S{ds->user.p, ds->item.p, ds->label.p, ds->unit_values ? nullptr : ds->uval.p, ds->unit_values ? nullptr : ds->ival.p};
            launch_predict_basic(P, S, n, w_out_.p, stream_);
        } else {
            launch_predict_fused(P, ds->fused.view(), ds->fused.max_nu, ds->fused.max_ni, n, w_out_.p, stream_);
        }
        if (!ds->order_dev.p) { check(ds->sched.order.size() == (size_t)n, "predict_dataset: the data set keeps no file order"); ds->order_dev.upload(ds->sched.order.data(), (size_t)n, stream_); }
        w_pred_.reserve((size_t)n);
        device_scatter_f32(w_out_.p, ds->order_dev.p, w_pred_.p, n, stream_);
        HIPCHECK(hipMemcpyAsync(out, w_pred_.p, (size_t)n * sizeof(float), hipMemcpyDeviceToHost, stream_));
        HIPCHECK(hipStreamSynchronize(stream_));
    } else {
        DevCSR D{ds->row_label.p, ds->row_ptr.p, ds->feat_index.p, ds->feat_value.p};
        launch_predict(P, D, n, w_out_.p, stream_);
        HIPCHECK(hipMemcpyAsync(out, w_out_.p, (size_t)n * sizeof(float), hipMemcpyDeviceToHost, stream_));
        HIPCHECK(hipStreamSynchronize(stream_));
    }
    n_launches_++;
}

void Engine::eval_dataset(Dataset *ds, float scale, double *sum_sq, int64_t *count) {
    check(ds && ds->owner == this, "eval_dataset: dataset belongs to another trainer");
    if (ds->kind == 6 && multi_ && !in_multi_scope()) {
        flush();
        MultiScope local;
        long double acc = 0.0L;
        int64_t cnt = 0;
        for (int d = 0; d < gpus_; d++) {
            Engine *e = rank_engine(d);
            HIPCHECK(hipSetDevice(e->device_));
            for (Dataset *c : ds->mchild[(size_t)d]) {
                double s = 0.0; int64_t m = 0;
                e->eval_dataset(c, scale, &s, &m);
                acc += (long double)s; cnt += m;
            }
        }
        HIPCHECK(hipSetDevice(device_));
        *sum_sq = (double)acc; *count = cnt;
        return;
    }
    check(ds->kind != 6, "eval_dataset: not a data set of this handle");
    check(ds->kind != 7 && ds->kind != 8, "eval_dataset: user-unit window data sets are training sets; evaluate a level-scheduled data set of the same rows");
    check(ds->kind != 5 || ds->fused.max_ni == 1, "eval_dataset: rank-pair window data sets have no label to compare a score with");
    check(ds->sched_signature == schedule_signature(), "eval_dataset: the dataset was scheduled under another configuration; build it again");
    flush();
    const DevParams &P = params();
    const long n = ds->num_row;
    *sum_sq = 0.0; *count = n;
    if (n == 0) return;
    w_out_.reserve((size_t)n);
    const float *labels = nullptr;
    if (ds->kind == 4) {
        const UnitDev &d = ds->unitdev;
        launch_imfb(P, d.csr(), d.units.p, d.blks.p, d.fbidx.p, d.fbval.p, nullptr, 0, ds->num_units, sample_counter_, w_out_.p, stream_);
        labels = d.label.p;
    } else if (ds->kind == 3) {
        const UnitDev &d = ds->unitdev;
        launch_svdpp_predict(P, d.csr(), d.units.p, d.fbidx.p, d.fbval.p, ds->num_units, w_out_.p, stream_);
        labels = d.label.p;
    } else if (ds->kind == 5) {
        w_pred_.reserve((size_t)n);
        unsigned *ucol = reinterpret_cast<unsigned *>(w_pred_.p);
        launch_window_user_column(ds->win_urec.p, (int)ds->num_units, ucol, stream_);
        BasicSchedule S{ucol, ds->item.p, ds->label.p, nullptr, nullptr};
        launch_predict_basic(P, S, n, w_out_.p, stream_);
        labels = ds->label.p;
    } else if (ds->kind == 0 || ds->kind == 9 || ds->kind == 10) {
        BasicSchedule S{ds->user.p, ds->item.p, ds->label.p, ds->unit_values ? nullptr : ds->uval.p, ds->unit_values ? nullptr : ds->ival.p};
        launch_predict_basic(P, S, n, w_out_.p, stream_);
        labels = ds->label.p;
    } else if (ds->kind == 11) {
// ... 25 lines not shown
```

svdfeature_amd/csrc/svdf_engine.h:

```cpp
#ifndef SVDF_ENGINE_H_
#define SVDF_ENGINE_H_

#include <hip/hip_runtime.h>

#include <condition_variable>
#include <cstdio>
#include <memory>
#include <mutex>
#include <stdexcept>
#include <thread>
#include <string>
#include <deque>
#include <functional>
#include <future>
#include <vector>

#include "svdf_types.h"

namespace svdf {

struct Error : std::runtime_error {
    explicit Error(const std::string &m) : std::runtime_error(m) {}
};
[[noreturn]] void fail(const std::string &msg);
// ... 35 lines not shown
    int base = 0;
    void resize(size_t nres) { if (last.size() < nres) last.resize(nres, 0); }
};
struct Schedule {
    std::vector<int> order;
    std::vector<long> level_ptr;
    std::vector<long> level_mid;
    long max_level_size = 0;
    size_t num_levels() const { return level_ptr.empty() ? 0 : level_ptr.size() - 1; }
};
void build_schedule(const std::vector<int> &levels, int base, Schedule &out);

struct SideTable {
    std::vector<unsigned> row_ptr{0};
    std::vector<unsigned> index;
    std::vector<float> value;
    unsigned num_row() const { return (unsigned)row_ptr.size() - 1; }
    void load(const char *fname);
};
struct ParamSet {
    std::vector<float> wd;
    std::vector<unsigned> bound;
    std::string prefix_a, prefix_b;
    void set_param(const char *name, const char *val);
};

struct HostCSR {
    std::vector<float> row_label;
    std::vector<int> row_ptr{0};
    std::vector<unsigned> feat_index;
    std::vector<float> feat_value;
    long num_row() const { return (long)row_label.size(); }
    void clear() { row_label.clear(); row_ptr.assign(1, 0); feat_index.clear(); feat_value.clear(); }
};

struct FusedHost {
    std::vector<float> label, uval[2], ival[2], gval;
    std::vector<unsigned> uidx[2], iidx[2], gidx;
    std::vector<int> gptr;
    std::vector<unsigned> gsi[4];
    std::vector<float> gsv[4];
    int max_nu = 1, max_ni = 1;
    bool has_g = false, inline_g = false;
};
struct FusedDev {
    DevBuf<float> label, uval[2], ival[2], gval, gsv[4];
    DevBuf<unsigned> uidx[2], iidx[2], gidx, gsi[4];
    DevBuf<int> gptr;
    int max_nu = 1, max_ni = 1;
    bool has_g = false, inline_g = false;
    bool dense_slots = false;
    void upload(const FusedHost &h, hipStream_t st);
    FusedSchedule view() const;
};

struct UnitDev {
    DevBuf<float> label, value, fbval;
    DevBuf<int> ptr, order;
    DevBuf<unsigned> index, fbidx;
    DevBuf<DevUnit> units;
    DevBuf<DevUnitX> xunits;
    DevBuf<DevBlk> blks;
    DevBuf<unsigned char> fresh;
    bool has_fresh = false, unit_values = false;
    DevCSR csr() const { return DevCSR{label.p, ptr.p, index.p, value.p, unit_values ? 1 : 0, has_fresh ? fresh.p : nullptr}; }
};

struct RankRow {
    float label;
    int ng, nu, ni;
    const unsigned *index;
    const float *value;
};

struct WUnitHost;
struct LibcRand { uint32_t x[31]; char *handle = nullptr; };
bool libc_rand_capture(LibcRand &s);
void libc_rand_restore(const LibcRand &s);
void libc_jump_poly(uint64_t J, uint32_t a[31]);
void libc_rand_chunk_states(const LibcRand &s0, long nchunks, long C, std::vector<uint32_t> &states);
void libc_rand_peek(long n, int *out);
void libc_rand_skip(long n);

class PairSampler {
public:
    void set_param(const char *name, const char *val);
    void init();
    void sample_block(const std::vector<RankRow> &rows, std::vector<float> &label, std::vector<int64_t> &row_ptr,
                      std::vector<unsigned> &index, std::vector<float> &value);
    int method() const { return method_; }
    int pointwise() const { return pointwise_; }
    int sample_num() const { return sample_num_; }
    int sample_max() const { return sample_max_; }
    float pos_lowerb() const { return pos_lowerb_; }
    float neg_upperb() const { return neg_upperb_; }
    int seed_bytime() const { return seed_bytime_; }
    float gap() const { return gap_; }
private:
    int sample_num_ = -1, sample_max_ = 0x7fffffff, method_ = 0, pointwise_ = 0, seed_bytime_ = 0;
    float gap_ = 0.0001f, pos_lowerb_ = 0.8f, neg_upperb_ = 1e-6f;
    bool init_done_ = false;
    std::vector<RankRow> pos_, neg_;
};

struct RankPrefetch;
struct UserGroupArrays;
struct MultiState;
struct MultiDeleter { void operator()(MultiState *m) const; };
struct IpcState;
struct IpcDeleter { void operator()(IpcState *s) const; };
struct RcclState;
struct RcclDeleter { void operator()(RcclState *s) const; };
void rccl_unique_id(unsigned char *out128);
struct RankSource {
    std::string path;
    long file_size = -1, file_mtime = -1, file_ino = -1;
    bool eligible = false;
    long num_block = 0, num_row = 0;
    DevBuf<long> block_row_ptr, draws, pairs, draw_off, pair_off;
    DevBuf<float> label, uval, ival;
    DevBuf<unsigned> uidx, iidx, raw, tables;
    DevBuf<int> pos_list, neg_list;
    bool general = false;
    std::vector<int> h_tag;
    std::vector<int64_t> h_fb_ptr;
    std::vector<unsigned> h_fb_index;
    std::vector<float> h_fb_value;
    DevBuf<int> g_row_ptr, pair_p, pair_n, lens, optr;
    DevBuf<unsigned> g_index, out_index;
    DevBuf<float> g_value, out_label, out_value;
    void *scan_tmp = nullptr;
    size_t scan_tmp_bytes = 0;
    ~RankSource() { if (scan_tmp) (void)hipFree(scan_tmp); }
};
class Engine;
class Ranker;

struct Dataset {
    Engine *owner = nullptr;
    long num_row = 0;
    int kind = 0;
    DevBuf<WinUser> win_urec;
    DevBuf<int> win_slot, win_iptr, win_slot1;
    DevBuf<unsigned> win_item1;
    DevBuf<float> win_ival1;
    long win_item_lo = 0, win_item_hi = -1;
    DevBuf<long> d_level_ptr;
    bool d_level_ptr_ok = false;
    DevBuf<PairUnit> pu_units;
    DevBuf<unsigned> pu_lo, pu_hi;
    DevBuf<float> pu_vlo, pu_one;
    DevBuf<unsigned> rn_item, rn_user[8];
    DevBuf<float> rn_label[8];
    int rn_len = 0;
    std::vector<long> pv_unit_ptr;
    bool pv_item_pivot = false;
    long pv_cold = 0, pv_hot_rows = 0;
    int64_t chained_levels = 0;
    bool win_hot = false;
    long win_slots = 0;
    DevBuf<WinUnit> wu_units;
    DevBuf<WinSeg> wu_segs;
    DevBuf<int> wu_rptr, wu_tptr, wu_gptr;
    DevBuf<WinEnt> wu_ent, wu_fbent;
    DevBuf<WinTouched> wu_touched;
    long wu_ntouched = -1;
    DevBuf<WinFbRec> wu_fbrec;
    long wu_nseg = 0;
    bool wu_defer_fb = false;
    long wu_gslots = 0;
    int wu_estride = 0;
    bool wu_feedback = false;
    DevBuf<int> wu_uptr, wu_upos;
    DevBuf<WinEnt> wu_uent;
    long wu_nshared = 0;
    DevBuf<int> wu_iptr;
    DevBuf<WinEnt> wu_ient;
    bool wu_ichild = false;
    DevBuf<WinHot> wu_hot;
    DevBuf<WinHotRec> wu_hrec;
    long wu_nhot = 0;
    int wseq_shared_sub = -1;
    std::vector<Dataset *> wchild;
    std::vector<std::vector<Dataset *>> mchild;
    bool m_minibatch = false;
    FusedDev fused;
    UnitDev unitdev;
    Schedule sched;
    DevBuf<int> order_dev;
    DevBuf<unsigned> user, item;
    DevBuf<float> label, uval, ival;
    bool unit_values = true;
    DevBuf<float> row_label, feat_value;
    DevBuf<int> row_ptr, order;
    DevBuf<unsigned> feat_index;
    long algorithmic_bytes = 0;
    long num_units = 0, num_simple_units = 0;
    uint64_t sched_signature = 0;
    hipGraphExec_t graph_exec = nullptr;
    uint64_t graph_version = 0;
    hipStream_t graph_stream = nullptr;
    Dataset() = default;
    ~Dataset();
    Dataset(const Dataset &) = delete;
    Dataset &operator=(const Dataset &) = delete;
};

class Engine {
  public:
    Engine(TypeParam mtype, int device);
    ~Engine();

    void set_param(const char *name, const char *val);
    void init_model();
    void load_model(FILE *fi);
    void save_model(FILE *fo);
    void save_model_begin(FILE *fo);
    void save_model_end();
    void init_trainer();
    void set_round(int nround);
    void finish_round();
    void update_csr(float label, int ng, int nu, int ni, const unsigned *index, const float *value);
    float predict_csr(float label, int ng, int nu, int ni, const unsigned *index, const float *value);
    void update_csr_batch(int num_row, const float *row_label, const int *row_ptr, const unsigned *feat_index, const float *feat_value);
    void predict_csr_batch(int num_row, const float *row_label, const int *row_ptr, const unsigned *feat_index, const float *feat_value, float *out);
    void update_block(int nfb, int tag, const unsigned *ifb, const float *vfb, int num_row, const float *row_label,
                      const int *row_ptr, const unsigned *feat_index, const float *feat_value);
    void predict_block(int nfb, int tag, const unsigned *ifb, const float *vfb, int num_row, const float *row_label,
                       const int *row_ptr, const unsigned *feat_index, const float *feat_value, float *out);

    Dataset *dataset_from_csr(long num_row, const float *row_label, const int64_t *row_ptr, const unsigned *feat_index, const float *feat_value);
    Dataset *dataset_from_triples(long n, const unsigned *user, const unsigned *item, const float *label);
    Dataset *dataset_from_pairs(long n, const unsigned *user, const unsigned *pos, const unsigned *neg);
    Dataset *dataset_from_blocks(long num_block, const int *extend_tag, const int64_t *fb_ptr, const unsigned *fb_index, const float *fb_value,
                                 const int64_t *block_row_ptr, const float *row_label, const int64_t *row_ptr, const unsigned *feat_index,
                                 const float *feat_value);
    Dataset *dataset_from_buffer_file(const char *path, int user_group_format);
    Dataset *dataset_from_rank_buffer_file(const char *path);
    long rank_sample_buffer_file(const char *in_path, const char *out_path);
    void rank_prefetch(const char *path);
    void rank_prefetch_drop();
    Dataset *dataset_window_from_triples(long n, const unsigned *user, const unsigned *item, const float *label);
    Dataset *dataset_window_from_pairs(long n, const unsigned *user, const unsigned *pos, const unsigned *neg);
    void window_delta_pack(Dataset *ds, void *device_dst, int half, int64_t *count);
    void window_delta_apply(const void *device_src, int half);
    void window_delta_apply_local(Dataset *ds);
    void ipc_setup(int rank, int world, int64_t wire_bytes, int64_t block_floats, unsigned char *handles_out);
    void ipc_connect(const unsigned char *all_handles);
    void ipc_window_pack(Dataset *ds, int half);
    void ipc_window_reduce(int half);
    void ipc_window_apply(int half);
    void ipc_block_send(int dst, int slot);
    void ipc_block_recv(int src, int slot, unsigned seq);
    int ipc_status() const;
    void ipc_set_spin_limit(long polls);
    long ipc_spin_limit_ = 0;
    void ipc_fail_if_dead(const char *where);
    void ipc_close();
    void stratum_step(Dataset *const *ds, int n, int block, int nblocks, float *device_out);
    void item_block_set_at(int block, int nblocks, const float *device_src);
    void rccl_init(const unsigned char *id128, int rank, int world);
    void rccl_window_allreduce(Dataset *ds, int half);
    void rccl_block_handoff(int dst, int src, int slot, int in_block, int nblocks);
    void rccl_block_arrive(int slot);
    int64_t rccl_counter(int what) const;
    void rccl_close();
    Dataset *dataset_window_from_csr(long n, const float *row_label, const int64_t *row_ptr, const unsigned *feat_index, const float *feat_value);
    Dataset *dataset_window_from_blocks(long num_block, const int *extend_tag, const int64_t *fb_ptr, const unsigned *fb_index, const float *fb_value,
                                        const int64_t *block_row_ptr, const float *row_label, const int64_t *row_ptr, const unsigned *feat_index,
                                        const float *feat_value);
    void item_block_copy(float *device_buf, int set, int64_t *count);
    void train_dataset(Dataset *ds);
    void predict_dataset(Dataset *ds, float *out);
    void eval_dataset(Dataset *ds, float scale, double *sum_sq, int64_t *count);

    void per_rank_api() const {
        if (multi_ && !in_multi_scope())
            fail("svdfeature_amd: svdf_item_delta_* / svdf_window_delta_* / svdf_item_block_* are the per-rank entry points of the one-process-per-GPU "
                 "scheme; an amd:gpus > 1 handle exchanges by itself (train through svdf_update* / svdf_train_dataset)");
    }
    void item_delta_begin();
    void *item_delta_buffer(int64_t *count);
    void item_delta_apply();
    void item_delta_copy(float *device_dst, const float *device_src);
    void item_delta_into(float *device_dst, int64_t *count);
    void item_delta_apply_from(const float *device_src);
    void item_delta_select(int part, int nparts);
    void item_delta_pack(void *device_dst, int half, int64_t *count);
    void item_delta_unpack(const void *device_src, int half, int refresh_snapshot);
    void set_stream(hipStream_t s);

    int64_t get_view(int which, float *out, int64_t capacity);
    int64_t set_view(int which, const float *in, int64_t count);
    void view_shape(int which, int *rows, int *cols);
    hipStream_t stream() const { return stream_; }
    std::string path_for(const Dataset *ds) const;
    void note_dataset(Dataset *ds);
    void synchronize();
    int64_t counter(int what) const;
    int set_knob(const char *name, long value);
    void flush();

  private:
    TypeParam mtype_;
    ModelParam mp_;
    TrainParam tp_;
    ParamSet u_param_, i_param_, g_param_;
// ... 62 lines not shown
    std::vector<unsigned char> staged_fresh_;
    bool any_fresh_ = false, simple_unit_values_ = false;
    bool relax_global_ = false, relax_feedback_ = false;
    int g_stride_ = 1;
    int wanted_g_stride() const { return (relax_global_ && mp_.num_global <= (1 << 24)) ? 32 : 1; }
    void upload_globals(int stride);
    void download_globals(float *dst);
    unsigned relax_user_from_ = 0xFFFFFFFFu, relax_item_from_ = 0xFFFFFFFFu;
    unsigned shared_user_from_ = 0xFFFFFFFFu;
    bool shared_user() const { return shared_user_from_ != 0xFFFFFFFFu; }
    unsigned shared_user_for_auto() const { return shared_user() && !contrib_bf16_ ? shared_user_from_ : 0xFFFFFFFFu; }
    PairSampler pair_sampler_;
    RankPrefetch *rank_prefetch_ = nullptr;
    std::vector<Dataset *> datasets_;
    void adopt(Dataset *ds);
    struct UCol { const unsigned *src; DevBuf<unsigned> *dst; };
    struct FCol { const float *src; DevBuf<float> *dst; };
    void schedule_columns_on_device(Dataset *ds, long n, int K, const int *res_col, const unsigned *off, const unsigned *limit,
                                    const char *const *msg, int sort_col, unsigned sort_max, const std::vector<UCol> &ucols, const std::vector<FCol> &fcols);
    const int *host_order(Dataset *ds);
    bool device_sched_ = true;
    long device_sched_min_ = 1 << 16;
    Dataset w_dataset_;
    uint64_t schedule_signature() const;
    void disown(Dataset *ds);
    void rank_pass(const char *path, UserGroupArrays &g);
    Dataset *rank_pass_device(const char *path);
    bool rank_source_load(const char *path);
    bool rank_pass_device_general(const char *path, UserGroupArrays &g);
    std::unique_ptr<RankSource> rank_source_;
    bool device_rank_ = true;
    bool device_load_ = true;
    bool device_window_ = true;
    bool device_init_ = true;
    int device_init_margin_log2_ = 46;
    int64_t n_init_reports_ = 0, n_init_draws_ = 0, n_chained_levels_ = 0;
    long chain_width_ = 128;
    bool fewrow_fast_ = true;
    Dataset *dataset_fewrow_on_device(long n, const float *row_label, const int64_t *row_ptr, const unsigned *feat_index, const float *feat_value);
    struct DUCol { const unsigned *src; DevBuf<unsigned> *dst; };
    struct DFCol { const float *src; DevBuf<float> *dst; };
    void schedule_device_columns(Dataset *ds, long n, int K, const unsigned *const *res_col, const unsigned *off, const unsigned *limit,
                                 const char *const *msg, const unsigned *sort_key, unsigned sort_max, const std::vector<DUCol> &ucols,
                                 const std::vector<DFCol> &fcols);
    bool rows_without_feedback_ = true;
    bool rows_as_instances_ = false;
    bool relaxed() const { return relax_global_ || relax_feedback_ || relax_user_from_ != 0xFFFFFFFFu || relax_item_from_ != 0xFFFFFFFFu; }
    unsigned sample_counter_ = 0;
    DevBuf<unsigned> d_ref_ui_, d_ref_global_;
    bool lazy_decay() const { return tp_.reg_method >= 4 || tp_.reg_global >= 4; }
    int groups_per_wave_ = 0, block_threads_ = 0, store_mode_ = 0, load_mode_ = 2, basic_i8_ = 1, svdpp_helpers_ = 8, svdpp_xunits_ = 1, small_blocks_ = 1, fewrow_i16_ = 1, sort_batches_ = 1, xcd_remap_ = 1, hot_reduce_ = 1;
    LevelTracker tracker_;
    void stage_rows(int num_row, const float *row_label, const int *row_ptr, const unsigned *feat_index, const float *feat_value);
    void stage_rows_into(HostCSR &dst, int num_row, const float *row_label, const int *row_ptr, const unsigned *feat_index, const float *feat_value);
    void check_row(int ng, int nu, int ni, const unsigned *index);
    bool basic_fast_path_allowed() const;
    bool fused_allowed() const;
    bool fused_allowed_for_rows() const;
    template <typename PtrT> bool fused_shape_ok(long n, const PtrT *row_ptr, const unsigned *idx, FusedHost &out);
    template <typename PtrT> void fill_fused(long n, const float *row_label, const PtrT *row_ptr, const unsigned *idx, const float *val,
                                             const int *order, FusedHost &out);
    FusedHost w_fused_host_;
    FusedDev w_fused_;
    bool use_fused_ = true, use_simple_units_ = true;
    size_t num_resources() const { return (size_t)n_uiset_ + (size_t)mp_.num_global; }
    int level_of_row(const unsigned *ig, int ng, const unsigned *iu, int nu, const unsigned *ii, int ni, int lvl0);
    void touch_row(const unsigned *ig, int ng, const unsigned *iu, int nu, const unsigned *ii, int ni, int lvl);
    void flush_csr(HostCSR &src);
    void flush_units();
    void submit_window();
    void wait_worker();
    void worker_main();
    std::thread worker_;
    std::mutex mu_;
    std::condition_variable cv_;
    HostCSR job_;
    bool worker_busy_ = false, worker_stop_ = false, async_flush_ = true;
    std::string worker_error_;
    void schedule_units(int base, Schedule &sched, std::vector<DevUnit> &du);
    void upload_unit_arrays(UnitDev &dst);
    void upload_units(UnitDev &dst, const Schedule &sched, const std::vector<DevUnit> &du, bool scheduled_on_device = false);
    bool schedule_units_on_device(UnitDev &dst, Schedule &sched, std::vector<DevUnit> &du);
    int64_t unit_sched_us_ = 0;
    bool unit_sched_on_device_ = false;
    std::vector<int64_t> stamp_;
    int64_t stamp_epoch_ = 0;
    DevBuf<float> w_label_, w_value_, w_uval_, w_ival_, w_fbval_, w_out_, w_pred_;
    DevBuf<int> w_ptr_, w_order_;
    DevBuf<unsigned> w_index_, w_user_, w_item_, w_fbidx_;
    DevBuf<DevUnit> w_units_;
    UnitDev w_unitdev_;
    DevBuf<float> d_snap_, d_delta_;
    DevBuf<unsigned> wb_user_, wb_item_, wb_neg_, wb_k0_, wb_k1_, wb_v0_, wb_v1_, wb_inst_, wb_state_;
    DevBuf<float> wb_label_;
    DevBuf<int> wb_slot_e_, wb_head_, wb_mark_, wb_run_user_, wb_run_start_, wb_run_begin_;
    DevBuf<char> wb_tmp_;
    bool window_build_device(Dataset *ds, long n, const unsigned *user, const unsigned *item, const float *label, const unsigned *neg);
    void window_build_resident(Dataset *ds, long n, const unsigned *d_user, const unsigned *d_item, const float *d_label, const unsigned *d_neg);
    void window_build_header(Dataset *ds, long n, bool pairs);
    bool device_window_ready() const { return !host_only_ && device_window_; }
    DevBuf<float> d_dvec_, d_dbias_;
    DevBuf<float> d_contrib_, d_cbias_;
    std::unique_ptr<IpcState, IpcDeleter> ipc_;
    std::unique_ptr<RcclState, RcclDeleter> rccl_;
    void rccl_check(const char *what);
    void ipc_check(const char *what);
    DevBuf<float> d_gcontrib_;
    WUnitSchedule wunit_view(const Dataset *ds) const;
    void wunit_check_config(const char *what, bool side_tables = false) const;
    bool side_tables() const { return feat_user_.num_row() != 0 || feat_item_.num_row() != 0; }
    void side_children_ok(const int64_t *row_ptr3, const unsigned *feat_index, std::vector<unsigned> &seen) const;
    bool wunit_config_ok() const;
    void wunit_build(Dataset *ds, const void *segs, size_t nseg, const std::vector<int64_t> &seg_rows, bool by_row_order, long num_src_row,
                     const float *row_label, const int64_t *row_ptr, const unsigned *feat_index, const float *feat_value,
                     const unsigned *fb_index, const float *fb_value);
    void wunit_build_host(WUnitHost &H, bool inplace, const void *segs, size_t nseg, const std::vector<int64_t> &seg_rows, bool by_row_order, long num_src_row,
                          const float *row_label, const int64_t *row_ptr, const unsigned *feat_index, const float *feat_value,
                          const unsigned *fb_index, const float *fb_value, const int64_t *priv_pos = nullptr, bool children = false, int shared_sub = 0) const;
    void wunit_adopt(Dataset *ds, const WUnitHost &H);
    void wunit_host_from_csr(WUnitHost &H, bool inplace, long n, const float *row_label, const int64_t *row_ptr, const unsigned *feat_index, const float *feat_value,
                             bool shared = false, int shared_sub = 0) const;
    void wunit_host_from_blocks(WUnitHost &H, bool inplace, long b0, long b1, const int *extend_tag, const int64_t *fb_ptr, const unsigned *fb_index, const float *fb_value,
                                const int64_t *block_row_ptr, const float *row_label, const int64_t *row_ptr, const unsigned *feat_index, const float *feat_value) const;
    int wseq_build_threads_ = 32;
    void wunit_fill_from_csr(Dataset *ds, long n, const float *row_label, const int64_t *row_ptr, const unsigned *feat_index, const float *feat_value);
    void wunit_fill_from_blocks(Dataset *ds, long b0, long b1, const int *extend_tag, const int64_t *fb_ptr, const unsigned *fb_index, const float *fb_value,
                                const int64_t *block_row_ptr, const float *row_label, const int64_t *row_ptr, const unsigned *feat_index, const float *feat_value);
    void wunit_train(Dataset *ds);
    void wunit_sum(Dataset *ds, void *dst, int half);
    bool step_minibatch_set_ = false;
    bool contrib_bf16_ = false;
    int fewrow_gslots_ = 1;
    int wunit_defer_fb_ = 1;
    int wunit_inplace_ = 1;
    bool wunit_inplace_build_ = false;
    int wunit_fast_ = 2;
    int wseq_per_target_fb_ = 16;
    int wseq_per_target_child_ = 3;
    int wseq_per_target_shared_ = 12;
    int wseq_per_target_max_ = 128;
    int wseq_shared_sub_ = 0;
    int wseq_shared_max_ = 512;
    int wseq_hot_sub_ = 128;
    int wseq_hot_max_ = 2048;
    DevBuf<float> d_clabel_;
    bool wseq_hot_ok() const;
    long wseq_windows_hot(long n, const std::vector<long> &item_count) const;
    long wseq_windows_shared(long n, const std::vector<long> &plain, const std::vector<long> &child) const;
    double wseq_max_ratio() const { return (double)wseq_per_target_ / (double)wseq_per_target_max_; }
    int wseq_per_target_ = 24;
    bool single_minibatch() const { return step_minibatch_set_ && gpus_ == 1 && !multi_ && !is_peer_; }
    int runs_exec_ = 1;
    int runs_len_ = 4;
    int runs_sets_ = 1, runs_block_ = 64;
    long runs_min_rows_ = 1 << 20;
    int64_t n_runs_passes_ = 0;
    bool runs_config_ok() const;
    Dataset *runs_dataset_from_triples(long n, const unsigned *user, const unsigned *item, const float *label);
    void runs_train(Dataset *ds);
    int pivot_exec_ = 1;
    int pivot_run_ = 256, pivot_run_long_ = 256;
    int pivot_min_ = 2048;
    int64_t n_pivot_passes_ = 0;
    int pair_units_ = 1, pair_unit_cap_ = 16;
    int64_t n_punit_passes_ = 0;
    bool punit_config_ok() const;
    Dataset *punit_dataset_from_pairs(long n, const unsigned *user, const unsigned *pos, const unsigned *neg);
    bool punit_build(long n, const unsigned *user, const unsigned *lo, const unsigned *hi, std::vector<PairUnit> &sorted, std::vector<long> &level_ptr) const;
    bool punit_flush(HostCSR &src);
    DevBuf<PairUnit> w_pu_units_;
    PairUnitSchedule punit_view(const Dataset *ds) const;
    void punit_train(Dataset *ds);
    void punit_predict(Dataset *ds, float *d_out);
    bool pivot_config_ok() const;
    Dataset *pivot_dataset_from_triples(long n, const unsigned *user, const unsigned *item, const float *label);
    void pivot_train(Dataset *ds);
    bool step_auto_set_ = false, auto_building_ = false;
    struct AutoDecision { int decided = 0; long levels = 0, windows = 0; double dag_ms = 0.0, stream_ms = 0.0; } auto_last_;
    bool auto_step_active() const { return step_auto_set_ && !auto_building_ && gpus_ == 1 && !multi_ && !is_peer_ && !host_only_; }
    Dataset *auto_step(Dataset *exact, bool window_ok, const std::function<Dataset *()> &build_window);
    static constexpr long AUTO_PROBE_ROWS = 2000000, AUTO_PROBE_MIN = 8000000;
    AutoDecision auto_probe_;
    std::string auto_rank_path_;
    int auto_rank_decision_ = 0;
    bool auto_probe_deep(Dataset *probe, long n_full);
    int64_t n_guard_warnings_ = 0;
    AutoDecision guard_last_;
    long wseq_windows(long n, const std::vector<double> &updates_per_target) const;
    Dataset *wseq_from_csr(long n, const float *row_label, const int64_t *row_ptr, const unsigned *feat_index, const float *feat_value);
    Dataset *wseq_from_blocks(long num_block, const int *extend_tag, const int64_t *fb_ptr, const unsigned *fb_index, const float *fb_value,
                              const int64_t *block_row_ptr, const float *row_label, const int64_t *row_ptr, const unsigned *feat_index, const float *feat_value);
    Dataset *wseq_from_triples(long n, const unsigned *user, const unsigned *item, const float *label);
    Dataset *wseq_from_pairs(long n, const unsigned *user, const unsigned *pos, const unsigned *neg);
    void wseq_train(Dataset *ds);
    WindowSchedule window_view(const Dataset *ds) const;
    Dataset *window_trained_ = nullptr;
    int window_slots_ = 1, window_groups_ = 0;
    int delta_part_ = 0, delta_nparts_ = 1;
    DevBuf<double> d_partials_;
    struct Range { float *base; long n; };
    std::vector<Range> shared_ranges();
    int gpus_ = 1;
    bool is_peer_ = false, delta_half_ = true, window_set_ = false;
    std::vector<std::pair<std::string, std::string>> param_log_;
    std::unique_ptr<MultiState, MultiDeleter> multi_;
    Engine *rank_engine(int d);
    void multi_setup();
    void multi_copy_model_to_peers();
    void multi_flush(HostCSR &src);
    void multi_prepare();
    void multi_window(const std::function<void(int, Engine *)> &train, bool minibatch, Dataset *const *mb);
    bool multi_minibatch_allowed() const;
    Dataset *multi_dataset_from_triples(long n, const unsigned *user, const unsigned *item, const float *label);
    Dataset *multi_dataset_from_pairs(long n, const unsigned *user, const unsigned *pos, const unsigned *neg);
    Dataset *multi_dataset_from_csr(long num_row, const float *row_label, const int64_t *row_ptr, const unsigned *feat_index, const float *feat_value);
    Dataset *multi_dataset_from_blocks(long num_block, const int *extend_tag, const int64_t *fb_ptr, const unsigned *fb_index, const float *fb_value,
                                       const int64_t *block_row_ptr, const float *row_label, const int64_t *row_ptr, const unsigned *feat_index,
                                       const float *feat_value);
    void multi_train_dataset(Dataset *ds);
    long multi_windows_for(long n, const std::vector<long> &item_count, bool minibatch) const;
    void multi_synchronize();
    int multi_predict_rank_ = 0;
    int multi_exchange_mode_ = 0;
    bool multi_step_levels_ = false;
    std::unique_ptr<Dataset> w_window_;
    void window_build(Dataset *ds, long n, const unsigned *user, const unsigned *item, const float *label, const unsigned *neg = nullptr);
    void multi_predict(int num_row, const float *row_label, const int *row_ptr, const unsigned *feat_index, const float *feat_value, float *out);
    void multi_gather_user_rows();
    int64_t multi_counter(int what) const;
    void item_delta_begin_local();
    void predict_csr_batch_local(int num_row, const float *row_label, const int *row_ptr, const unsigned *feat_index, const float *feat_value, float *out);
    int64_t n_instances_ = 0, n_launches_ = 0, n_batches_ = 0, n_flushes_ = 0;
    static constexpr size_t PRED_PIN_WORDS = 1 << 16;
    unsigned *pred_pin_ = nullptr;
    static constexpr size_t SAVE_PIN_FLOATS = (size_t)8 << 20;
    struct SavePipe { float *pin[2] = {nullptr, nullptr}; hipEvent_t ev[2] = {nullptr, nullptr}; hipStream_t st = nullptr; };
    SavePipe save_pipe_;
    struct SaveAsync { DevBuf<float> W, bias; std::vector<float> g; hipEvent_t ready = nullptr; hipStream_t st = nullptr; SavePipe pipe; std::thread th;
                       std::string error; bool active = false; } save_async_;
    void save_pipe_init(SavePipe &sp, hipStream_t st);
    static void save_pipe_free(SavePipe &sp);
    void dev_to_file(SavePipe &sp, FILE *fo, const float *dsrc, long rows, long cols, long pitch);
    void write_model_from_device(SavePipe &sp, FILE *fo, const float *W, const float *bias, const float *g);
    void write_model_from_device(FILE *fo);
    int64_t ns_flush_ = 0, ns_model_ = 0;
    int64_t n_device_rank_passes_ = 0;
    int64_t n_kind_[3] = {0, 0, 0};
    DeltaRanges delta_ranges();
    friend struct Dataset;
    friend class Ranker;
};

class Ranker {
  public:
    Ranker(TypeParam mtype, int device);
    ~Ranker();
    void set_param(const char *name, const char *val);
    void load_model(FILE *fi);
    void init_ranker(int num_item_set);
    long process(float label, int ng, int nu, int ni, const unsigned *index, const float *value, int *out, long cap);
    long process_rows(int num_row, const float *row_label, const int *row_ptr, const unsigned *feat_index, const float *feat_value, int *out, long cap);
    long process_block(int nfb, int tag, const unsigned *ifb, const float *vfb, int num_row, const float *row_label, const int *row_ptr,
                       const unsigned *feat_index, const float *feat_value, int *out, long cap);
    int64_t counter(int what) const {
        return what == 0 ? n_sections_ : (what == 1 ? n_host_sorts_ : (what == 2 ? (int64_t)pos_item_.size() : (what == 3 ? n_tiles_ : (what == 4 ? tie_copy_ns_ : (what == 5 ? tie_wait_ns_ : (what == 6 ? event_wait_ns_ : (what == 7 ? flush_ns_ : -1)))))));
    }
  private:
    std::unique_ptr<Engine> eng_;
    int top_k_ = 0, num_item_set_ = 0, num_item_processed_ = 0;
    long items_on_device_ = 0;
    bool init_end_ = false, user_open_ = false;
    HostCSR items_, spec_;
    std::vector<int> spec_idx_, pos_item_;
    std::vector<int> tagged_, dev_tagged_;
    long n_banned_ = 0;
    static constexpr int RANK_SLOTS = 8;
    struct RankSlot {
        unsigned *pin = nullptr, *back = nullptr;
        size_t pin_words = 0, back_words = 0;
        DevBuf<unsigned> d_stage, d_flag;
        DevBuf<int> d_cnt;
        DevBuf<float> d_ps, d_score;
        hipEvent_t ev = nullptr;
    };
    struct RankPending { int slot = 0, npos = 0, take = 0; long n = 0; std::vector<int> pos_item, banned;
                         int nsec = 0; std::vector<std::vector<int>> tile_pos, tile_ban; std::vector<int> tile_take; long out_stride = 0; };
    struct TileSec { std::vector<unsigned> user_idx; std::vector<float> user_val; std::vector<int> pos_item, banned; int take = 0; };
    std::vector<TileSec> tile_;
    long tile_n_ = 0;
    std::vector<int> tile_prev_ban_;
    DevBuf<unsigned> d_banmask_;
    DevBuf<float> d_tu_tile_;
    void flush_tile();
    bool tile_enabled_ = true;
    int64_t n_tiles_ = 0;
    RankSlot slots_[RANK_SLOTS];
    struct RankChunk { std::vector<int> vals; std::future<std::vector<int>> fut; bool pending = false; };
    std::deque<RankPending> pending_;
    std::deque<RankChunk> chunks_;
    void flush_chunks();
    int next_slot_ = 0;
    bool deferred_ = false;
    int *out_ptr_ = nullptr;
    long out_cap_ = 0, out_n_ = 0;
    void slot_reserve_pin(RankSlot &S, size_t words);
    void slot_reserve_back(RankSlot &S, size_t words);
// ... 27 lines not shown
```

svdfeature_amd/csrc/svdf_k_runs.hip:

```cpp
#include "svdf_device.h"

namespace svdf {

__global__ __launch_bounds__(256) void k_runs_check(const unsigned *user, const unsigned *item, long n, unsigned nu, unsigned ni, unsigned *flag) {
    const long stride = (long)gridDim.x * blockDim.x;
    unsigned bad = 0u;
    for (long p = (long)blockIdx.x * blockDim.x + threadIdx.x; p < n; p += stride) {
        if (user[p] >= nu) bad |= 1u;
        if (item[p] >= ni) bad |= 2u;
    }
    if (bad) atomicOr(flag, bad);
}
__global__ __launch_bounds__(256) void k_runs_prev(const unsigned *keys, const unsigned *pos, long n, unsigned *prev) {
    const long stride = (long)gridDim.x * blockDim.x;
    for (long j = (long)blockIdx.x * blockDim.x + threadIdx.x; j < n; j += stride)
        prev[pos[j]] = (j > 0 && keys[j - 1] == keys[j]) ? pos[j - 1] : 0xFFFFFFFFu;
}
__global__ __launch_bounds__(256) void k_runs_form(const unsigned *ikeys, const unsigned *ipos, long n, unsigned num_item, const unsigned *prev, int R,
                                                   unsigned *head, unsigned *head_of, unsigned char *idx) {
    const long stride = (long)gridDim.x * blockDim.x;
    for (long it = (long)blockIdx.x * blockDim.x + threadIdx.x; it < (long)num_item; it += stride) {
        long lo = 0, hi = n;
        while (lo < hi) { const long mid = (lo + hi) >> 1; if (ikeys[mid] < (unsigned)it) lo = mid + 1; else hi = mid; }
        unsigned h = 0u;
        int len = 0;
        for (long j = lo; j < n && ikeys[j] == (unsigned)it; j++) {
            const unsigned p = ipos[j];
            const unsigned pv = prev[p];
            if (len > 0 && len < R && (pv == 0xFFFFFFFFu || pv < h)) {
                head[p] = 0u; head_of[p] = h; idx[p] = (unsigned char)len;
                len++;
            } else {
                head[p] = 1u; head_of[p] = p; idx[p] = 0;
                h = p; len = 1;
            }
        }
    }
}
__global__ __launch_bounds__(256) void k_runs_fill(const unsigned *user, const unsigned *item, const float *label, long n, const unsigned *unit_at,
                                                   const unsigned *head_of, const unsigned char *idx, long nunit, unsigned *c_item, unsigned *c_user, float *c_label) {
    const long stride = (long)gridDim.x * blockDim.x;
    for (long p = (long)blockIdx.x * blockDim.x + threadIdx.x; p < n; p += stride) {
        const unsigned un = unit_at[head_of[p]];
        const int j = idx[p];
        c_user[(size_t)j * (size_t)nunit + un] = user[p];
        c_label[(size_t)j * (size_t)nunit + un] = label[p];
        if (j == 0) c_item[un] = item[p];
    }
}
__global__ __launch_bounds__(256) void k_runs_fill_u32(unsigned *v, long n, unsigned x) {
    const long stride = (long)gridDim.x * blockDim.x;
    for (long j = (long)blockIdx.x * blockDim.x + threadIdx.x; j < n; j += stride) v[j] = x;
}
static inline int runs_grid(long n) { long g = (n + 255) / 256; return (int)(g < 1 ? 1 : (g > 16384 ? 16384 : g)); }
void launch_runs_check(const unsigned *user, const unsigned *item, long n, unsigned nu, unsigned ni, unsigned *flag, hipStream_t st) {
    if (n > 0) hipLaunchKernelGGL(k_runs_check, dim3(runs_grid(n)), dim3(256), 0, st, user, item, n, nu, ni, flag);
}
void launch_runs_prev(const unsigned *keys, const unsigned *pos, long n, unsigned *prev, hipStream_t st) {
    if (n > 0) hipLaunchKernelGGL(k_runs_prev, dim3(runs_grid(n)), dim3(256), 0, st, keys, pos, n, prev);
}
void launch_runs_form(const unsigned *ikeys, const unsigned *ipos, long n, unsigned num_item, const unsigned *prev, int R, unsigned *head, unsigned *head_of,
                      unsigned char *idx, hipStream_t st) {
    if (n > 0 && num_item > 0) hipLaunchKernelGGL(k_runs_form, dim3(runs_grid((long)num_item)), dim3(256), 0, st, ikeys, ipos, n, num_item, prev, R, head, head_of, idx);
}
void launch_runs_fill(const unsigned *user, const unsigned *item, const float *label, long n, const unsigned *unit_at, const unsigned *head_of,
                      const unsigned char *idx, long nunit, unsigned *c_item, unsigned *c_user, float *c_label, hipStream_t st) {
    if (n > 0) hipLaunchKernelGGL(k_runs_fill, dim3(runs_grid(n)), dim3(256), 0, st, user, item, label, n, unit_at, head_of, idx, nunit, c_item, c_user, c_label);
}
__global__ __launch_bounds__(256) void k_runs_iota(unsigned *v, long n) {
    const long stride = (long)gridDim.x * blockDim.x;
    for (long j = (long)blockIdx.x * blockDim.x + threadIdx.x; j < n; j += stride) v[j] = (unsigned)j;
}
void launch_runs_iota(unsigned *v, long n, hipStream_t st) {
    if (n <= 0) return;
    long grid = (n + 255) / 256;
    if (grid > 16384) grid = 16384;
    hipLaunchKernelGGL(k_runs_iota, dim3((int)grid), dim3(256), 0, st, v, n);
}
void launch_runs_fill_u32(unsigned *v, long n, unsigned x, hipStream_t st) {
    if (n > 0) hipLaunchKernelGGL(k_runs_fill_u32, dim3(runs_grid(n)), dim3(256), 0, st, v, n, x);
}

template <int LANES, int V, int R, int G>
__global__ __launch_bounds__(256) void k_basicmf_runs_soa(const DevParams P, const RunSchedule S, long begin, long end) {
    constexpr int T = 16 / LANES;
    constexpr int IPS = 64 / LANES;
    constexpr int K = 4 * LANES * V;
    const int lane = threadIdx.x & 63;
    long tile = blockIdx.x;
    if (P.xcd_remap) tile = (long)(blockIdx.x & 7) * (gridDim.x >> 3) + (blockIdx.x >> 3);
    const long wave = tile * (blockDim.x >> 6) + (threadIdx.x >> 6);
    const int m = (lane & 15) / T;
    const int gslot = (lane >> 4) * T + (lane & (T - 1));
    const int pitch = P.pitch;
    const float dec_u1 = snap_to_one(1.0f - P.lr * P.wd_user), dec_i1 = snap_to_one(1.0f - P.lr * P.wd_item);
#pragma unroll 1
    for (int g = 0; g < G; g++) {
        const long w0 = begin + (wave * G + g) * IPS;
        if (w0 >= end) return;
        const long s = w0 + gslot;
        const bool live = s < end;
        const long sc = live ? s : w0;
        const unsigned ir = P.item_off + S.item[sc];
        unsigned ur[R];
        float label[R], bu[R];
        float4 p[R][V], q[V];
        int n = 0;
#pragma unroll
        for (int j = 0; j < R; j++) {
            const unsigned u = S.user[j][sc];
            label[j] = S.label[j][sc];
            const bool on = live && u != (unsigned)SLOT_ABSENT;
            ur[j] = P.user_off + (on ? u : 0u);
            if (on) n = j + 1;
        }
#pragma unroll
        for (int v = 0; v < V; v++) q[v] = live ? load_row_nt<K / 4>(P.W, ir, pitch, m + v * LANES, K) : f4zero();
        float bi = live ? P.bias[ir] : 0.0f;
#pragma unroll
        for (int j = 0; j < R; j++) {
#pragma unroll
            for (int v = 0; v < V; v++) p[j][v] = f4zero();
            bu[j] = 0.0f;
            if (j < n) {
#pragma unroll
                for (int v = 0; v < V; v++) p[j][v] = load_row_nt<K / 4>(P.W, ur[j], pitch, m + v * LANES, K);
                bu[j] = P.bias[ur[j]];
            }
        }
        int nmax = n;
#pragma unroll
        for (int o = 32; o > 0; o >>= 1) nmax = max(nmax, __shfl_xor(nmax, o));
#pragma unroll
        for (int j = 0; j < R; j++) {
            if (j >= nmax) break;
            double bs = 0.0;
            bs += (double)(1.0f * bu[j]); bs += 0.0;
            bs += 0.0;
            bs += (double)(1.0f * bi);
            double sum = (double)P.base_score + bs;
            float4 tu[V], ti[V];
#pragma unroll
            for (int v = 0; v < V; v++) { tu[v] = f4zero(); ti[v] = f4zero(); axpy4(tu[v], p[j][v], 1.0f); axpy4(ti[v], q[v], 1.0f); }
            sum += (double)dot_slots<LANES, V>(tu, ti, m, lane);
            const float pred = (float)sum;
            const float err = (label[j] - pred) * 1.0f;
            const float su = P.lr * err * 1.0f;
            const float si = P.lr * err * 1.0f;
            float nbu = bu[j] + su, nbi = bi + si;
            nbu = nbu * (1.0f - P.lr * P.wd_user_bias);
            nbi = nbi * (1.0f - P.lr * P.wd_item_bias);
            const bool act = j < n;
#pragma unroll
            for (int v = 0; v < V; v++) {
                float4 wu = p[j][v], wi = q[v];
                axpy4(wu, ti[v], su);
                axpy4(wi, tu[v], si);
                wu.x = wu.x * dec_u1; wu.y = wu.y * dec_u1; wu.z = wu.z * dec_u1; wu.w = wu.w * dec_u1;
                wi.x = wi.x * dec_i1; wi.y = wi.y * dec_i1; wi.z = wi.z * dec_i1; wi.w = wi.w * dec_i1;
                if (act) {
                    store_row<K / 4>(P.W, ur[j], pitch, m + v * LANES, K, wu);
                    q[v] = wi;
                }
            }
            if (act) {
                P.bias[ur[j]] = nbu;
                bi = nbi;
            }
        }
        if (live) {
#pragma unroll
            for (int v = 0; v < V; v++) store_row<K / 4>(P.W, ir, pitch, m + v * LANES, K, q[v]);
            P.bias[ir] = bi;
        }
    }
}
bool basicmf_runs_soa_applies(const DevParams &P) {
    return P.basic_i8 && P.active_type == ACT_LINEAR && P.reg_method == 0 && P.no_user_bias == 0 && P.user_nonnegative == 0 && P.u_rng.n == 0 && P.i_rng.n == 0 &&
           P.store_mode == 0 && (P.k == 64 || P.k == 128);
}
void launch_basicmf_runs_soa(const DevParams &P, const RunSchedule &S, long begin, long end, int R, int G, int block_threads, hipStream_t st) {
    if (end <= begin) return;
    if (G < 1) G = 1;
    if (block_threads != 64 && block_threads != 128 && block_threads != 256) block_threads = 64;
    const int per_wave = P.k == 128 ? 4 : 8;
    const long per_block = (long)(block_threads / 64) * G * per_wave;
    int grid = (int)((end - begin + per_block - 1) / per_block);
    if (P.xcd_remap) grid = (grid + 7) & ~7;
#define RUNS_LAUNCH(L_, R_, G_) hipLaunchKernelGGL((k_basicmf_runs_soa<L_, 2, R_, G_>), dim3(grid), dim3(block_threads), 0, st, P, S, begin, end)
#define RUNS_BY_R(L_)                                                                                                          \
    if (R == 2) { if (G >= 2) RUNS_LAUNCH(L_, 2, 2); else RUNS_LAUNCH(L_, 2, 1); }       \
    else if (R == 4) { if (G >= 2) RUNS_LAUNCH(L_, 4, 2); else RUNS_LAUNCH(L_, 4, 1); }                                       \
    else { if (G >= 2) RUNS_LAUNCH(L_, 7, 2); else RUNS_LAUNCH(L_, 7, 1); }
    if (P.k == 128) { RUNS_BY_R(16) } else { RUNS_BY_R(8) }
#undef RUNS_BY_R
#undef RUNS_LAUNCH
}

}
```

svdfeature_amd/csrc/svdf_kernels.h:

```cpp
#ifndef SVDF_KERNELS_H_
#define SVDF_KERNELS_H_

#include <hip/hip_runtime.h>

#include <type_traits>
#include <vector>

#include "svdf_types.h"

namespace svdf {

int lanes_per_instance(int k);
int max_supported_factor();
int max_fast_path_factor();

void launch_basicmf(const DevParams &P, const BasicSchedule &S, long begin, long end, int groups_per_wave, int block_threads, hipStream_t st);
bool launch_basicmf_chain(const DevParams &P, const BasicSchedule &S, const long *d_level_ptr, long l0, long l1, hipStream_t st);
void launch_fused(const DevParams &P, const FusedSchedule &S, int max_nu, int max_ni, long begin, long end, int groups_per_wave,
                  int block_threads, hipStream_t st);
bool fewrow_fast_applies(const DevParams &P, const FusedSchedule &S);
bool launch_fewrow_chain(const DevParams &P, const FusedSchedule &S, int max_nu, int max_ni, const long *d_level_ptr, long l0, long l1, hipStream_t st);
bool fewrow_gslots_applies(const DevParams &P, const FusedSchedule &S, int max_nu, int max_ni, bool dense_slots);
void launch_fewrow_gslots(const DevParams &P, const FusedSchedule &S, long begin, long end, hipStream_t st);
void launch_fewrow_fast(const DevParams &P, const FusedSchedule &S, int max_nu, int max_ni, long begin, long end, int block_threads, hipStream_t st);
void launch_predict_fused(const DevParams &P, const FusedSchedule &S, int max_nu, int max_ni, long n, float *out, hipStream_t st);
void launch_general(const DevParams &P, const DevCSR &D, const int *order, long begin, long end, unsigned counter_base, hipStream_t st);
void launch_svdpp(const DevParams &P, const DevCSR &D, const DevUnit *units, const unsigned *fb_index, const float *fb_value,
                  const int *order, long begin, long end, unsigned counter_base, hipStream_t st);
void launch_svdpp_wave(const DevParams &P, const DevCSR &D, const DevUnit *units, const unsigned *fb_index, const float *fb_value,
                       const int *order, const DevUnitX *xunits, long begin, long end, hipStream_t st);
void launch_imfb(const DevParams &P, const DevCSR &D, const DevUnit *units, const DevBlk *blks, const unsigned *fb_index, const float *fb_value,
                 const int *order, long begin, long end, unsigned counter_base, float *predict_out, hipStream_t st);
void launch_predict(const DevParams &P, const DevCSR &D, long n, float *out, hipStream_t st);
void launch_predict_basic(const DevParams &P, const BasicSchedule &S, long n, float *out, hipStream_t st);
void launch_svdpp_predict(const DevParams &P, const DevCSR &D, const DevUnit *units, const unsigned *fb_index, const float *fb_value,
                          long nunit, float *out, hipStream_t st);
void launch_delta_pack(const DeltaRanges &R, const float *snap, void *dst, int half, hipStream_t st);
void launch_delta_unpack(const DeltaRanges &R, float *snap, const void *src, int half, int refresh, hipStream_t st);
bool window_slots_applies(const DevParams &P, const WindowSchedule &S);
void launch_window_apply(const DevParams &P, const WindowSchedule &S, long num_item, float *w_item, float *i_bias, hipStream_t st);
void launch_window_users(const DevParams &P, const WindowSchedule &S, int slots, int groups_per_wave, hipStream_t st);
void launch_window_items(const WindowSchedule &S, int pitch, int k, long lo, long hi, long nglobal, void *dst, int half, hipStream_t st, long nslots = -1);
void launch_delta_addto(const DeltaRanges &R, const void *src, int half, hipStream_t st);
void launch_window_items_local(const WindowSchedule &S, int pitch, int k, long lo, long hi, float *w_item, float *i_bias, hipStream_t st, long nslots = -1);
void launch_ranges_copy(const DeltaRanges &R, float *buf, int set, hipStream_t st);
void launch_wunit_walk(const DevParams &P, const WUnitSchedule &S, bool feedback, int fast, hipStream_t st);
bool wunit_wave_applies(const DevParams &P, const WUnitSchedule &S, bool feedback);
void launch_wunit_wave(const DevParams &P, const WUnitSchedule &S, hipStream_t st);
void launch_wunit_apply_shared(const DevParams &P, const WUnitSchedule &S, hipStream_t st);
void launch_wunit_sum(const DevParams &P, const WUnitSchedule &S, void *dst, int half, hipStream_t st);
void launch_ipc_signal(unsigned *const *pages, int n, int phase, int me, unsigned seq, const unsigned *err, hipStream_t st);
void launch_ipc_wait(unsigned *page, int phase, int n, unsigned seq, unsigned *err, unsigned long long spin_limit, hipStream_t st);
void launch_ipc_copy(float *dst, const float *src, long n, const unsigned *err, hipStream_t st);
void launch_window_user_column(const WinUser *urec, int nusers, unsigned *user_out, hipStream_t st);
void launch_pairs_prepare(long n, const unsigned *pos, const unsigned *neg, unsigned *lo, unsigned *hi, float *vlo, float *vhi, float *ones,
                          unsigned *flag, hipStream_t st);
void launch_delta_sum(const void *const *srcs, int n, void *dst, long total, int half, hipStream_t st);
void launch_delta_reduce_gather(void *const *bufs, int n, long begin, long end, int half, hipStream_t st, const unsigned *err = nullptr);
void launch_rows_strided_copy(float *dst, long dst_first, long dst_stride, const float *src, long src_first, long src_stride, long nrows, int width,
                              hipStream_t st);
void launch_delta_sub(const float *cur, const float *snap, float *delta, long n, hipStream_t st);
void launch_delta_add(float *cur, const float *snap, const float *delta, long n, hipStream_t st);
void launch_rank_items(const DevParams &P, const DevCSR &D, long first, long n, float *ifactors, float *ibias, hipStream_t st);
void launch_rank_feedback(const DevParams &P, const unsigned *fidx, const float *fval, int nfb, float *fb_out, hipStream_t st);
struct RankSection { int nu, npos, nprev, nnew; };
void launch_rank_user(const DevParams &P, const unsigned *stage, const RankSection &S, const float *fb_in, float *tu_out, signed char *tag, int *cnt,
                      unsigned *flag, long cap, const float *ifT, const float *ibias, float *pos_score, unsigned *zero_words, int nzero, hipStream_t st);
void launch_rank_spec(const DevParams &P, const DevCSR &D, long n, const int *spec_idx, const float *tu, float *item_score, hipStream_t st);
void launch_rank_transpose(const DevParams &P, long first, long n, long cap, const float *ifactors, float *ifT, hipStream_t st);
struct RankFused { int mode; const int *pos_item; const float *pos_score; int npos; int *greater, *ties; unsigned *keys, *vals, *flag, *hist1; };
void launch_rank_score(const DevParams &P, long n, long cap, const float *tu, const float *ifT, const float *ibias, const signed char *tag,
                       float *item_score, int fresh, const RankFused &F, hipStream_t st);
#define RANK_TILE 32
struct RankTile { int nsec; int off[RANK_TILE], nu[RANK_TILE], npos[RANK_TILE], nban[RANK_TILE], pos0[RANK_TILE]; };
void launch_rank_tile_open(const DevParams &P, const unsigned *stage, const RankTile &T, const float *fb_in, float *tuT, unsigned *banmask,
                           const unsigned *prev_ban, int nprev, int *cnt, unsigned *flag, long cap, const float *ifT, const float *ibias, float *pos_score,
                           unsigned *zero_words, long nzero, hipStream_t st);
void launch_rank_score_tile(const DevParams &P, long n, long cap, const float *tuT, const float *ifT, const float *ibias, const unsigned *banmask, unsigned *out,
                            const unsigned *stage, const RankTile &T, const float *pos_score, int *cnt, int mode, unsigned *wmin, unsigned *flag, hipStream_t st);
struct RselSecs { unsigned K1[RANK_TILE]; };
long rank_tile_minima(long n);
bool rank_tile_select_applies(long n, long cap, long K1max);
void launch_rank_tile_select(long n, long cap, int nsec, const unsigned *keys, const unsigned *wmin, const RselSecs &Ks, unsigned *out, long out_stride,
                             const unsigned *flag, hipStream_t st);
void launch_rank_select_tile(long n, long cap, int nsec, const unsigned *keys, const RselSecs &Ks, unsigned *work, unsigned *ck, unsigned *cv, unsigned *out,
                             long out_stride, unsigned *flag, hipStream_t st);
void launch_rank_positions(long n, const float *score, const signed char *tag, const int *pos_item, int npos, int *greater, int *ties, hipStream_t st);
long rank_select_work_words();
long rank_select_cap();
void launch_rank_select(long n, const unsigned *keys, const unsigned *vals, unsigned K1, unsigned *work, unsigned *ck, unsigned *cv, unsigned *out,
                        const unsigned *flag, hipStream_t st);
long device_exclusive_scan_u32(const unsigned *in, unsigned *out, long n, void **tmp, size_t *tmp_bytes, hipStream_t st);
void launch_runs_check(const unsigned *user, const unsigned *item, long n, unsigned nu, unsigned ni, unsigned *flag, hipStream_t st);
void launch_runs_prev(const unsigned *keys, const unsigned *pos, long n, unsigned *prev, hipStream_t st);
void launch_runs_form(const unsigned *ikeys, const unsigned *ipos, long n, unsigned num_item, const unsigned *prev, int R, unsigned *head, unsigned *head_of,
                      unsigned char *idx, hipStream_t st);
void launch_runs_fill(const unsigned *user, const unsigned *item, const float *label, long n, const unsigned *unit_at, const unsigned *head_of,
                      const unsigned char *idx, long nunit, unsigned *c_item, unsigned *c_user, float *c_label, hipStream_t st);
bool pair_units_applies(const DevParams &P);
void launch_pair_units(const DevParams &P, const PairUnitSchedule &S, long begin, long end, float *out, hipStream_t st);
void launch_runs_iota(unsigned *v, long n, hipStream_t st);
void launch_runs_fill_u32(unsigned *v, long n, unsigned x, hipStream_t st);
bool basicmf_runs_soa_applies(const DevParams &P);
void launch_basicmf_runs_soa(const DevParams &P, const RunSchedule &S, long begin, long end, int R, int G, int block_threads, hipStream_t st);
void device_sort_pairs_u32(unsigned *keys_in, unsigned *keys_out, unsigned *vals_in, unsigned *vals_out, long n, void **tmp, size_t *tmp_bytes, hipStream_t st);
int sqerr_partials_grid(long n);
void launch_sqerr_partials(const float *pred, const float *label, long n, float scale, double *partials, hipStream_t st);
struct RankSourceDev {
    long num_block, num_row;
    const long *block_row_ptr;
    const float *label, *uval, *ival;
    const unsigned *uidx, *iidx;
};
struct SamplerParams { float pos_lowerb, neg_upperb; int sample_num, sample_max; };
struct PairColumns { float *label, *uval, *v0, *v1; unsigned *uidx, *i0, *i1; };
struct RankRowsDev {
    long num_block, num_row;
    const long *block_row_ptr;
    const float *label;
    const int *row_ptr;
    const unsigned *index;
    const float *value;
};
struct GSamplerParams { float pos_lowerb, neg_upperb, gap; int sample_num, sample_max, method, method_raw, pointwise; };
void launch_gsample_counts(const RankRowsDev &S, const GSamplerParams &sp, int *scratch, long *draws, long *pairs, hipStream_t st);
void launch_gsample_pairs(const RankRowsDev &S, const GSamplerParams &sp, const long *draw_off, const long *pair_off, const unsigned *raw, int *pos_list,
                          int *neg_list, int *pair_p, int *pair_n, hipStream_t st);
void launch_gpair_sizes(const RankRowsDev &S, const GSamplerParams &sp, long npairs, const int *pair_p, const int *pair_n, int *lens, hipStream_t st);
void launch_gpair_write(const RankRowsDev &S, const GSamplerParams &sp, long npairs, const int *pair_p, const int *pair_n, const int *optr, float *olabel,
                        unsigned *oi, float *ov, hipStream_t st);
void device_exclusive_scan_i32(const int *in, int *out, long n, void **tmp, size_t *tmp_bytes, hipStream_t st);
void host_sort_by_label(const float *label, long n, int *ids);
void host_parallel_sort_scores(const float *score, int *ids, long n, int nthreads);
void launch_rand_expand(const unsigned *tables, long nchunks, long C, long D, unsigned *raw, hipStream_t st);
struct WBuildIn { long n; int pairs; const unsigned *user, *item, *neg; const float *label; long num_user, num_item; };
struct WBuildBuffers {
    unsigned *k0, *k1, *v0, *v1;
    unsigned *inst;
    int *slot_e;
    int *head, *mark;
    int *run_user, *run_start, *run_begin;
    void *tmp; size_t tmp_bytes;
    unsigned *state;
};
struct WBuildOut { WinUser *urec; unsigned *item, *item1; float *label, *v0, *v1; int *slot, *slot1, *iptr; };
size_t wbuild_tmp_bytes(long m);
void device_window_build(const WBuildIn &in, const WBuildBuffers &B, const WBuildOut &out, long *nact, long *item_lo, long *item_hi, hipStream_t st);
struct InitSeg { long begin, count; long row0; int k; float sigma; int absf; };
struct InitPlan { InitSeg seg[3]; int nseg; long total; int pitch; double margin; };
struct InitReport { long j; unsigned r1, r2; };
void launch_init_expand(const unsigned *tables, long nchunks, long C, long D, unsigned *raw, hipStream_t st);
size_t init_scan_tmp_bytes(long A);
void launch_init_patch(long n, const long *idx, const float *val, float *W, hipStream_t st);
void launch_init_tile(const unsigned *raw, long A, long base, const InitPlan &plan, float *W, unsigned *flag, unsigned *off, void *tmp, size_t tmp_bytes,
                      unsigned long long *state, InitReport *reports, int report_cap, hipStream_t st);
void launch_sample_counts(const RankSourceDev &S, const SamplerParams &sp, long *draws, long *pairs, hipStream_t st);
void launch_sample_posneg(const RankSourceDev &S, const SamplerParams &sp, const long *draw_off, const long *pair_off, const unsigned *raw,
                          int *pos_list, int *neg_list, const PairColumns &out, hipStream_t st);
#define SVDF_SCHED_MAX_SLOTS 8
struct SchedColumns {
    int K;
    long n;
    const unsigned *col[SVDF_SCHED_MAX_SLOTS];
    unsigned off[SVDF_SCHED_MAX_SLOTS], limit[SVDF_SCHED_MAX_SLOTS];
    const char *limit_msg[SVDF_SCHED_MAX_SLOTS];
    unsigned num_res;
    const unsigned *sort_key;
    unsigned sort_key_max;
};
long device_schedule(const SchedColumns &in, int *order_out, std::vector<long> &level_ptr, long *max_level_size, hipStream_t st);
struct UnitSchedIn {
    long n, nrow;
    const DevUnit *units;
    const int *row_ptr;
    const unsigned *index;
    const float *value;
    const unsigned *fb_index;
    unsigned goff, user_off, item_off, fb_off, num_item, num_fb, state_res;
    int simple_ok, fast_ok;
};
struct UnitSchedOut {
    std::vector<long> level_ptr;
    long max_level_size;
    bool any_fresh, unit_values;
};
long device_schedule_units(const UnitSchedIn &in, int *order_out, unsigned char *simple_out, unsigned char *fresh_out, UnitSchedOut &out, hipStream_t st);
void device_gather_u32(const unsigned *src, const int *order, unsigned *dst, long n, hipStream_t st);
void device_gather_f32(const float *src, const int *order, float *dst, long n, hipStream_t st);
void device_scatter_f32(const float *src, const int *order, float *dst, long n, hipStream_t st);
int device_expf(const float *in, unsigned first, unsigned step, float *out, long n);

}
#endif
```

svdfeature_amd/csrc/svdf_runs.cpp:

```cpp
#include <algorithm>
#include <cstring>
#include <memory>

#include "svdf_engine.h"
#include "svdf_kernels.h"
#include "svdf_internal.h"

namespace svdf {

bool Engine::runs_config_ok() const {
    return runs_exec_ != 0 && !host_only_ && device_sched_ && !user_group() && basic_fast_path_allowed() && mtype_.extend_type == 0 && mtype_.active_type == ACT_LINEAR &&
           tp_.reg_method == 0 && mp_.user_nonnegative == 0 && mp_.no_user_bias == 0 && u_param_.bound.empty() && i_param_.bound.empty() && (mp_.num_factor == 64 || mp_.num_factor == 128) &&
           basic_i8_ != 0 && store_mode_ == 0;
}

Dataset *Engine::runs_dataset_from_triples(long n, const unsigned *user, const unsigned *item, const float *label) {
    if (!runs_config_ok() || n < runs_min_rows_ || n >= 0x7FFFFFF0L) return nullptr;
    const int RF = std::max(2, std::min(7, runs_len_));
    const int R = RF <= 2 ? 2 : (RF <= 4 ? 4 : 7);
    const unsigned NU = (unsigned)mp_.num_user, NI = (unsigned)mp_.num_item;
    std::unique_ptr<Dataset> ds(new Dataset());
    adopt(ds.get());
    ds->kind = 10; ds->num_row = n; ds->rn_len = R;
    ds->user.upload(user, (size_t)n, stream_);
    ds->item.upload(item, (size_t)n, stream_);
    ds->label.upload(label, (size_t)n, stream_);
    ds->unit_values = true;
    DevBuf<unsigned> flag, ka, kb, va, vb, prev, head, head_of, unit_at, c_item, c_user;
    DevBuf<unsigned char> idx;
    DevBuf<float> c_label;
    flag.reserve(4);
    HIPCHECK(hipMemsetAsync(flag.p, 0, 4 * sizeof(unsigned), stream_));
    launch_runs_check(ds->user.p, ds->item.p, n, NU, NI, flag.p, stream_);
    unsigned hflag = 0;
    HIPCHECK(hipMemcpyAsync(&hflag, flag.p, sizeof(unsigned), hipMemcpyDeviceToHost, stream_));
    HIPCHECK(hipStreamSynchronize(stream_));
    if (hflag & 1u) fail("user feature index exceed bound");
    if (hflag & 2u) fail("item feature index exceed bound");
    ka.reserve((size_t)n); kb.reserve((size_t)n); va.reserve((size_t)n); vb.reserve((size_t)n);
    prev.reserve((size_t)n); head.reserve((size_t)n); head_of.reserve((size_t)n); unit_at.reserve((size_t)n); idx.reserve((size_t)n);
    void *tmp = nullptr;
    size_t tmp_bytes = 0;
    struct FreeTmp { void *&p; ~FreeTmp() { if (p) (void)hipFree(p); } } free_tmp{tmp};
    HIPCHECK(hipMemcpyAsync(ka.p, ds->user.p, (size_t)n * sizeof(unsigned), hipMemcpyDeviceToDevice, stream_));
    launch_runs_iota(va.p, n, stream_);
    device_sort_pairs_u32(ka.p, kb.p, va.p, vb.p, n, &tmp, &tmp_bytes, stream_);
    launch_runs_prev(kb.p, vb.p, n, prev.p, stream_);
    HIPCHECK(hipMemcpyAsync(ka.p, ds->item.p, (size_t)n * sizeof(unsigned), hipMemcpyDeviceToDevice, stream_));
    launch_runs_iota(va.p, n, stream_);
    device_sort_pairs_u32(ka.p, kb.p, va.p, vb.p, n, &tmp, &tmp_bytes, stream_);
    launch_runs_form(kb.p, vb.p, n, NI, prev.p, RF, head.p, head_of.p, idx.p, stream_);
    const long nunit = device_exclusive_scan_u32(head.p, unit_at.p, n, &tmp, &tmp_bytes, stream_);
    HIPCHECK(hipGetLastError());
    c_item.reserve((size_t)nunit); c_user.reserve((size_t)R * (size_t)nunit); c_label.reserve((size_t)R * (size_t)nunit);
    launch_runs_fill_u32(c_user.p, (long)R * nunit, (unsigned)SLOT_ABSENT, stream_);
    HIPCHECK(hipMemsetAsync(c_label.p, 0, (size_t)R * (size_t)nunit * sizeof(float), stream_));
    launch_runs_fill(ds->user.p, ds->item.p, ds->label.p, n, unit_at.p, head_of.p, idx.p, nunit, c_item.p, c_user.p, c_label.p, stream_);
    HIPCHECK(hipGetLastError());
    HIPCHECK(hipStreamSynchronize(stream_));
    ka.release(); kb.release(); va.release(); vb.release(); prev.release(); head.release(); head_of.release(); unit_at.release(); idx.release();
    const unsigned *res[SVDF_SCHED_MAX_SLOTS];
    unsigned off[SVDF_SCHED_MAX_SLOTS], limit[SVDF_SCHED_MAX_SLOTS];
    const char *msg[SVDF_SCHED_MAX_SLOTS];
    res[0] = c_item.p; off[0] = NU; limit[0] = NI; msg[0] = "item feature index exceed bound";
    std::vector<DUCol> du{DUCol{c_item.p, &ds->rn_item}};
    std::vector<DFCol> df;
    for (int j = 0; j < R; j++) {
        res[1 + j] = c_user.p + (size_t)j * (size_t)nunit; off[1 + j] = 0u; limit[1 + j] = NU; msg[1 + j] = "user feature index exceed bound";
        du.push_back(DUCol{c_user.p + (size_t)j * (size_t)nunit, &ds->rn_user[j]});
        df.push_back(DFCol{c_label.p + (size_t)j * (size_t)nunit, &ds->rn_label[j]});
    }
    schedule_device_columns(ds.get(), nunit, 1 + R, res, off, limit, msg, sort_batches_ == 1 ? c_item.p : nullptr, NI, du, df);
    ds->num_units = nunit;
    ds->algorithmic_bytes = n * (8L * mp_.num_factor * 2 + 8 * 2 + 16 + 8 * 2);
    return ds.release();
}

void Engine::runs_train(Dataset *ds) {
    const DevParams &P = params();
    RunSchedule S;
    memset(&S, 0, sizeof(S));
    S.item = ds->rn_item.p;
    for (int j = 0; j < ds->rn_len; j++) { S.user[j] = ds->rn_user[j].p; S.label[j] = ds->rn_label[j].p; }
    const Schedule &sc = ds->sched;
    for (size_t l = 0; l < sc.num_levels(); l++) launch_basicmf_runs_soa(P, S, sc.level_ptr[l], sc.level_ptr[l + 1], ds->rn_len, runs_sets_, runs_block_, stream_);
    HIPCHECK(hipGetLastError());
    n_launches_ += (int64_t)sc.num_levels();
    n_batches_ += (int64_t)sc.num_levels();
    n_runs_passes_++;
}

}
```

svdfeature_amd/csrc/svdf_types.h:

```cpp
#ifndef SVDF_TYPES_H_
#define SVDF_TYPES_H_

#include <stdint.h>

namespace svdf {

struct TypeParam {
    uint8_t format_type, active_type, extend_type, variant_type;
};
static_assert(sizeof(TypeParam) == 4, "SVDTypeParam is 4 bytes");

struct ModelParam {
    int num_user, num_item, num_factor, num_global;
    float u_init_sigma, i_init_sigma, base_score;
    int no_user_bias, num_ufeedback;
    float ufeedback_init_sigma;
    int num_randinit_ufactor, num_randinit_ifactor;
    int common_latent_space, user_nonnegative, common_feedback_space, extend_flag, item_nonnegative;
    int reserved[247];
};
static_assert(sizeof(ModelParam) == 1056, "SVDModelParam is 1056 bytes on disk");

struct TrainParam {
    float learning_rate;
    int decay_learning_rate;
    float decay_rate, min_learning_rate;
    float wd_user, wd_item, wd_user_bias, wd_item_bias;
    int reg_method;
    float wd_global;
    int reg_global;
    unsigned num_regfree_global;
    float scale_lr_ufeedback, wd_ufeedback_user, wd_ufeedback, wd_ufeedback_bias;
};

enum { ACT_LINEAR = 0, ACT_SIGMOID_L2 = 1, ACT_SIGMOID_LIKELIHOOD = 2, ACT_SIGMOID_RANK = 3,
       ACT_HINGE_SMOOTH = 5, ACT_HINGE_L2 = 6, ACT_SIGMOID_QSGRAD = 7 };
enum { TAG_DEFAULT = 0, TAG_START = 1, TAG_END = 2, TAG_MIDDLE = 3 };

struct DevRanges {
    const unsigned *bound;
    const float *wd;
    int n;
};
struct DevSideTable {
    const unsigned *row_ptr;
    const unsigned *index;
    const float *value;
    unsigned num_row;
};

struct DevParams {
    float *W;
    float *bias;
    float *g_bias;
    float *svdpp_state;
    int pitch, k;
    unsigned user_off, item_off, fb_off;
    int num_user, num_item, num_global, num_ufeedback;
    float base_score;
    int active_type, no_user_bias, user_nonnegative, user_group;
    unsigned *ref_ui;
    unsigned *ref_global;
    unsigned relax_user_from, relax_item_from;
    int relax_global;
    int relax_feedback;
    int g_stride;
    int hot_reduce;
    int xcd_remap;
    unsigned imfb_disable;
    int imfb_deep;
    int fewrow_fast;
    int store_mode;
    int fewrow_i16;
    int svdpp_helpers;
    int small_blocks;
    int basic_i8;
    int load_mode;
    float lr, wd_user, wd_item, wd_user_bias, wd_item_bias, wd_global;
    int reg_method, reg_global;
    unsigned num_regfree_global;
    float scale_lr_ufeedback, wd_ufeedback, wd_ufeedback_bias;
    DevRanges u_rng, i_rng, g_rng;
    DevSideTable feat_user, feat_item;
};

struct BasicSchedule {
    const unsigned *user;
    const unsigned *item;
    const float *label;
    const float *uval;
    const float *ival;
};

struct RunSchedule {
    const unsigned *item;
    const unsigned *user[8];
    const float *label[8];
};

struct PairUnit { unsigned user; int begin; int count; int pad; };
struct PairUnitSchedule {
    const PairUnit *units;
    const unsigned *lo, *hi;
    const float *vlo;
};

struct FusedSchedule {
    const float *label;
    const unsigned *uidx[2];
    const float *uval[2];
    const unsigned *iidx[2];
    const float *ival[2];
    const int *gptr;
    const unsigned *gidx;
    const float *gval;
    const unsigned *gsi[4];
    const float *gsv[4];
};
enum { SLOT_ABSENT = 0xFFFFFFFFu };

struct DevCSR {
    const float *row_label;
    const int *row_ptr;
    const unsigned *feat_index;
    const float *feat_value;
    int unit_values;
    const unsigned char *row_fresh;
};

struct DevUnit {
    int fb_begin, fb_end;
    int row_begin, row_end;
    int flags;
};
struct DevUnitX {
    DevUnit u;
    int e0;
    unsigned user;
    int pad;
};
struct DevBlk {
    int fb_begin, fb_end, sc_begin, sc_end;
    int row_begin, row_end;
    int tag;
};
#define IMFB_DEPTH 4
#define IMFB_DEPTH_MAX 16
enum { UNIT_START = 1, UNIT_END = 2, UNIT_SAVE = 4, UNIT_LOAD = 8,
       UNIT_SIMPLE = 16 };

struct WinUser { unsigned user; int begin; int count; int pad; };
struct WindowSchedule {
    const WinUser *urec;
    long nusers;
    const unsigned *item;
    const float *label;
    const int *slot;
    const float *uval, *ival;
    const int *iptr;
    float *contrib;
    float *cbias;
    const unsigned *item1;
    const int *slot1;
    const float *ival1;
    int contrib_bf16;
    int hot_sub;
    float *clabel;
};

struct WinSeg { int fb_begin, fb_count, row_begin, row_count; };
struct WinUnit { unsigned user; int seg_begin; int seg_count; int rows; WinSeg first; };
struct WinEnt { unsigned idx; float val; int slot; int pad; };
struct WinFbRec { int seg; float val; };
struct WinTouched { int t, b, e; };
struct WinHot { int j, b, e, rec; };
struct WinHotRec { int row, pos; };
struct WUnitSchedule {
    const WinUnit *units;
    long nunits;
    const WinSeg *segs;
    const float *label;
    const float *uval;
    const int *rptr;
    int estride;
    const WinEnt *ent;
    const WinEnt *fbent;
    float *contrib, *cbias, *gcontrib;
    const int *tptr;
    const int *gptr;
    long nfb_rows, nitem_rows, nglobal;
    int contrib_bf16;
    const WinFbRec *fbrec;
    float *dvec, *dbias;
    int user_bias;
    const WinTouched *touched;
    long ntouched;
    const int *uptr, *upos;
    const WinEnt *uent;
    long nshared_rows;
    unsigned shared_from;
    const int *iptr;
    const WinEnt *ient;
    const WinHot *hot;
    const WinHotRec *hrec;
    long nhot;
    int hot_sub;
};

}
#define SVDF_MAX_DELTA_RANGES 6
struct DeltaRanges {
    float *base[SVDF_MAX_DELTA_RANGES];
    long off[SVDF_MAX_DELTA_RANGES + 1];
    long snap_off[SVDF_MAX_DELTA_RANGES];
    int n;
};

#endif
```

Measured before the change: 5.821 billion instances/s.

## Form item runs and their levels together in one device peel

Replaces the separate run-forming pass and generic level scheduler with an iterative device peel. Each round, every open item takes as many consecutive ratings as are ready (up to the run cap) and assigns them the current level, so runs and conflict-free levels are built jointly. Units are then sorted by level, optionally longest-first within a level, and written straight into the per-dataset columns. The aim is fewer levels and fuller runs during training, at the cost of a more complex setup with many small kernel launches and host syncs.

```diff
diff --git a/include/svdfeature_amd.h b/include/svdfeature_amd.h
--- a/include/svdfeature_amd.h
+++ b/include/svdfeature_amd.h
@@ -150,6 +150,9 @@
 int svdf_schedule_resources(long n, const int64_t *res_ptr, const unsigned *res, long num_res, int *order_out,
                             int64_t *level_ptr_out, long level_cap);
 
+int64_t svdf_runs_peel_host(long n, const unsigned *user, const unsigned *item, int cap, int *lvl_out, int *idx_out);
+int svdf_dataset_runs_plan(const svdf_dataset *ds, int64_t *level_ptr_out, unsigned *item_out, unsigned *user_out, float *label_out);
+
 #ifdef __cplusplus
 }
 #endif
diff --git a/svdfeature_amd/__init__.py b/svdfeature_amd/__init__.py
--- a/svdfeature_amd/__init__.py
+++ b/svdfeature_amd/__init__.py
@@ -138,6 +138,9 @@
     lib.svdf_counter.argtypes = [P, C.c_int]
     lib.svdf_set_knob.argtypes = [P, C.c_char_p, C.c_long]
     lib.svdf_schedule_resources.argtypes = [C.c_long, _i64p, _u32p, C.c_long, _i32p, _i64p, C.c_long]
+    lib.svdf_runs_peel_host.restype = C.c_int64
+    lib.svdf_runs_peel_host.argtypes = [C.c_long, _u32p, _u32p, C.c_int, _i32p, _i32p]
+    lib.svdf_dataset_runs_plan.argtypes = [P, _i64p, _u32p, _u32p, _f32p]
     lib.svdf_eval_dataset.argtypes = [P, P, C.c_float, C.POINTER(C.c_double), C.POINTER(C.c_int64)]
     lib.svdf_ranker_create.restype = P
     lib.svdf_ranker_create.argtypes = [C.c_uint8] * 4 + [C.c_int]
@@ -232,6 +235,16 @@
     return order[:n], level_ptr[:nl + 1]
 
 
+def runs_peel_host(user, item, cap):
+    lib = load_library()
+    n = len(user)
+    lvl, idx = np.zeros(max(n, 1), np.int32), np.zeros(max(n, 1), np.int32)
+    nl = lib.svdf_runs_peel_host(n, _pad(user, np.uint32), _pad(item, np.uint32), int(cap), lvl, idx)
+    if nl < 0:
+        raise SvdfError(lib.svdf_last_error().decode())
+    return lvl[:n], idx[:n], int(nl)
+
+
 class Dataset:
 
     def __init__(self, trainer, handle):
@@ -247,6 +260,16 @@
     algorithmic_bytes = property(lambda s: s.info(4))
     num_units = property(lambda s: s.info(5))
     num_simple_units = property(lambda s: s.info(6))
+
+    def runs_plan(self):
+        nu, nl = self.num_units, self.num_batches
+        level_ptr = np.zeros(nl + 1, np.int64)
+        item = np.zeros(max(nu, 1), np.uint32)
+        user, label = np.zeros(8 * max(nu, 1), np.uint32), np.zeros(8 * max(nu, 1), np.float32)
+        w = self.trainer.lib.svdf_dataset_runs_plan(self.h, level_ptr, item, user, label)
+        if w < 0:
+            raise SvdfError("runs_plan: not a runs data set")
+        return level_ptr, item[:nu], user[:w * nu].reshape(w, nu), label[:w * nu].reshape(w, nu)
 
     def close(self):
         if self.h:
diff --git a/svdfeature_amd/csrc/svdf_capi.cpp b/svdfeature_amd/csrc/svdf_capi.cpp
--- a/svdfeature_amd/csrc/svdf_capi.cpp
+++ b/svdfeature_amd/csrc/svdf_capi.cpp
@@ -8,6 +8,7 @@
 
 #include "svdf_engine.h"
 #include "svdf_kernels.h"
+#include "svdf_internal.h"
 
 namespace svdf {
 void set_error_mode(int m);
@@ -351,4 +352,24 @@
     })
 }
 
-}
+int64_t svdf_runs_peel_host(long n, const unsigned *user, const unsigned *item, int cap, int *lvl_out, int *idx_out) {
+    SVDF_GUARD(-1, { return (int64_t)svdf::runs_peel_host(n, user, item, cap, lvl_out, idx_out); })
+}
+int svdf_dataset_runs_plan(const svdf_dataset *ds, int64_t *level_ptr_out, unsigned *item_out, unsigned *user_out, float *label_out) {
+    SVDF_GUARD(-1, {
+        using svdf::fail;
+        if (!ds || !ds->d || ds->d->kind != 10) return -1;
+        const svdf::Dataset &d = *ds->d;
+        const size_t nu = (size_t)d.num_units;
+        for (size_t l = 0; l < d.sched.level_ptr.size(); l++) level_ptr_out[l] = d.sched.level_ptr[l];
+        if (nu == 0) return d.rn_len;
+        HIPCHECK(hipMemcpy(item_out, d.rn_item.p, nu * sizeof(unsigned), hipMemcpyDeviceToHost));
+        for (int j = 0; j < d.rn_len; j++) {
+            HIPCHECK(hipMemcpy(user_out + (size_t)j * nu, d.rn_user[j].p, nu * sizeof(unsigned), hipMemcpyDeviceToHost));
+            HIPCHECK(hipMemcpy(label_out + (size_t)j * nu, d.rn_label[j].p, nu * sizeof(float), hipMemcpyDeviceToHost));
+        }
+        return d.rn_len;
+    })
+}
+
+}
diff --git a/svdfeature_amd/csrc/svdf_config.cpp b/svdfeature_amd/csrc/svdf_config.cpp
--- a/svdfeature_amd/csrc/svdf_config.cpp
+++ b/svdfeature_amd/csrc/svdf_config.cpp
@@ -227,6 +227,7 @@
     if (!strcmp(name, "device_load")) { device_load_ = value != 0; return 0; }
     if (!strcmp(name, "runs_exec")) { check(value == 0 || value == 1, "runs_exec must be 0 or 1"); runs_exec_ = (int)value; return 0; }
     if (!strcmp(name, "runs_len")) { check(value >= 2 && value <= 7, "runs_len must be in 2 .. 7"); runs_len_ = (int)value; return 0; }
+    if (!strcmp(name, "runs_order")) { check(value == 0 || value == 1, "runs_order must be 0 or 1"); runs_order_ = (int)value; return 0; }
     if (!strcmp(name, "runs_sets")) { check(value >= 1 && value <= 2, "runs_sets must be 1 or 2"); runs_sets_ = (int)value; return 0; }
     if (!strcmp(name, "runs_block")) { check(value == 64 || value == 128 || value == 256, "runs_block must be 64, 128 or 256"); runs_block_ = (int)value; return 0; }
     if (!strcmp(name, "runs_min_rows")) { check(value >= 0, "runs_min_rows must not be negative"); runs_min_rows_ = value; return 0; }
diff --git a/svdfeature_amd/csrc/svdf_dataset.cpp b/svdfeature_amd/csrc/svdf_dataset.cpp
--- a/svdfeature_amd/csrc/svdf_dataset.cpp
+++ b/svdfeature_amd/csrc/svdf_dataset.cpp
@@ -607,7 +607,7 @@
                      ds->wchild.size(), side_tables() ? ", feature_user / feature_item children as shared rows (general walk k_wunit_walk)" : ""); return buf;
     case 9: snprintf(buf, sizeof(buf), "exact, %ld levels: hot rows walked as units (k_svdpp_wave on %s parameters, %ld units) + cold ratings through the contract kernel",
                      L, ds->pv_item_pivot ? "transposed" : "plain", ds->num_units); return buf;
-    case 10: snprintf(buf, sizeof(buf), "exact, %ld levels of runs: k_basicmf_runs_soa (up to %d consecutive ratings of one item per lane group, the item's row in registers)", L, ds->rn_len); return buf;
+    case 10: snprintf(buf, sizeof(buf), "exact, %ld levels of runs formed with their levels in one peel, %s inside a level: k_basicmf_runs_soa (up to %d consecutive ratings of one item per lane group, the item's row in registers)", L, ds->rn_order ? "longest first" : "by item", ds->rn_cap); return buf;
     case 11: snprintf(buf, sizeof(buf), "exact, %ld levels of user-run units: k_pair_units (%ld units of up to %d consecutive pairs of one user, the user's row in registers)",
                       L, ds->num_units, pair_unit_cap_); return buf;
     default: return "unknown";
diff --git a/svdfeature_amd/csrc/svdf_engine.h b/svdfeature_amd/csrc/svdf_engine.h
--- a/svdfeature_amd/csrc/svdf_engine.h
+++ b/svdfeature_amd/csrc/svdf_engine.h
@@ -211,7 +211,7 @@
     DevBuf<float> pu_vlo, pu_one;
     DevBuf<unsigned> rn_item, rn_user[8];
     DevBuf<float> rn_label[8];
-    int rn_len = 0;
+    int rn_len = 0, rn_cap = 0, rn_order = 0;
     std::vector<long> pv_unit_ptr;
     bool pv_item_pivot = false;
     long pv_cold = 0, pv_hot_rows = 0;
@@ -580,6 +580,7 @@
     bool single_minibatch() const { return step_minibatch_set_ && gpus_ == 1 && !multi_ && !is_peer_; }
     int runs_exec_ = 1;
     int runs_len_ = 4;
+    int runs_order_ = 0;
     int runs_sets_ = 1, runs_block_ = 64;
     long runs_min_rows_ = 1 << 20;
     int64_t n_runs_passes_ = 0;
diff --git a/svdfeature_amd/csrc/svdf_k_runs.hip b/svdfeature_amd/csrc/svdf_k_runs.hip
--- a/svdfeature_amd/csrc/svdf_k_runs.hip
+++ b/svdfeature_amd/csrc/svdf_k_runs.hip
@@ -16,36 +16,105 @@
     for (long j = (long)blockIdx.x * blockDim.x + threadIdx.x; j < n; j += stride)
         prev[pos[j]] = (j > 0 && keys[j - 1] == keys[j]) ? pos[j - 1] : 0xFFFFFFFFu;
 }
-__global__ __launch_bounds__(256) void k_runs_form(const unsigned *ikeys, const unsigned *ipos, long n, unsigned num_item, const unsigned *prev, int R,
-                                                   unsigned *head, unsigned *head_of, unsigned char *idx) {
-    const long stride = (long)gridDim.x * blockDim.x;
-    for (long it = (long)blockIdx.x * blockDim.x + threadIdx.x; it < (long)num_item; it += stride) {
+__global__ __launch_bounds__(256) void k_runs_iptr(const unsigned *ikeys, long n, unsigned num_item, unsigned *iptr, unsigned *cursor) {
+    const long stride = (long)gridDim.x * blockDim.x;
+    for (long it = (long)blockIdx.x * blockDim.x + threadIdx.x; it <= (long)num_item; it += stride) {
         long lo = 0, hi = n;
         while (lo < hi) { const long mid = (lo + hi) >> 1; if (ikeys[mid] < (unsigned)it) lo = mid + 1; else hi = mid; }
-        unsigned h = 0u;
-        int len = 0;
-        for (long j = lo; j < n && ikeys[j] == (unsigned)it; j++) {
-            const unsigned p = ipos[j];
-            const unsigned pv = prev[p];
-            if (len > 0 && len < R && (pv == 0xFFFFFFFFu || pv < h)) {
-                head[p] = 0u; head_of[p] = h; idx[p] = (unsigned char)len;
-                len++;
-            } else {
-                head[p] = 1u; head_of[p] = p; idx[p] = 0;
-                h = p; len = 1;
-            }
-        }
+        iptr[it] = (unsigned)lo;
+        if (it < (long)num_item) cursor[it] = (unsigned)lo;
+    }
+}
+#define RUNS_NONE 0xFFFFFFFFu
+#define RUNS_MAX_CAP 7
+__device__ __forceinline__ unsigned runs_lvl_load(const unsigned *lvl, unsigned p) { return __hip_atomic_load(lvl + p, __ATOMIC_RELAXED, __HIP_MEMORY_SCOPE_AGENT); }
+__device__ __forceinline__ void runs_lvl_store(unsigned *lvl, unsigned p, unsigned v) { __hip_atomic_store(lvl + p, v, __ATOMIC_RELAXED, __HIP_MEMORY_SCOPE_AGENT); }
+__device__ __forceinline__ bool runs_peel_item(unsigned it, unsigned L, int cap, const unsigned *ipos, const unsigned *iptr, const unsigned *prev, unsigned *cursor,
+                                               unsigned *lvl, unsigned *head_of, unsigned char *idx, unsigned *ctr) {
+    const unsigned cur = cursor[it], end = iptr[it + 1];
+    if (cur >= end) {
+        if (L == 1u) atomicAdd(ctr, 1u);
+        return false;
+    }
+    const int m = (int)min((unsigned)cap, end - cur);
+    unsigned p[RUNS_MAX_CAP], lv[RUNS_MAX_CAP];
+#pragma unroll
+    for (int j = 0; j < RUNS_MAX_CAP; j++) p[j] = j < m ? ipos[cur + j] : 0u;
+#pragma unroll
+    for (int j = 0; j < RUNS_MAX_CAP; j++) lv[j] = j < m ? prev[p[j]] : RUNS_NONE;
+#pragma unroll
+    for (int j = 0; j < RUNS_MAX_CAP; j++) lv[j] = (j < m && lv[j] != RUNS_NONE) ? runs_lvl_load(lvl, lv[j]) : (j < m ? RUNS_NONE : 0u);
+    int take = 0;
+#pragma unroll
+    for (int j = 0; j < RUNS_MAX_CAP; j++) {
+        const bool ready = j < m && (lv[j] == RUNS_NONE || (lv[j] != 0u && lv[j] < L));
+        if (j == take && ready) take = j + 1;
+    }
+#pragma unroll
+    for (int j = 0; j < RUNS_MAX_CAP; j++)
+        if (j < take) { runs_lvl_store(lvl, p[j], L); idx[p[j]] = (unsigned char)j; head_of[p[j]] = p[0]; }
+    if (take == 0) return true;
+    cursor[it] = cur + (unsigned)take;
+    if (cur + (unsigned)take == end) { atomicAdd(ctr, 1u); atomicMax(ctr + 1, L); return false; }
+    return true;
+}
+__global__ __launch_bounds__(256) void k_runs_peel(const unsigned *open, unsigned nopen, unsigned L, int cap, const unsigned *ipos, const unsigned *iptr, const unsigned *prev,
+                                                   unsigned *cursor, unsigned *lvl, unsigned *head_of, unsigned char *idx, unsigned *ctr) {
+    const unsigned t = blockIdx.x * blockDim.x + threadIdx.x;
+    if (t < nopen) (void)runs_peel_item(open ? open[t] : t, L, cap, ipos, iptr, prev, cursor, lvl, head_of, idx, ctr);
+}
+#define RUNS_NARROW 1024
+__global__ __launch_bounds__(RUNS_NARROW) void k_runs_peel_narrow(const unsigned *open, unsigned nopen, unsigned L0, unsigned iters, int cap, const unsigned *ipos,
+                                                                  const unsigned *iptr, const unsigned *prev, unsigned *cursor, unsigned *lvl, unsigned *head_of,
+                                                                  unsigned char *idx, unsigned *ctr) {
+    const unsigned t = threadIdx.x;
+    const unsigned it = t < nopen ? (open ? open[t] : t) : 0u;
+    bool live = t < nopen;
+    for (unsigned k = 1; k <= iters; k++) {
+        if (live) live = runs_peel_item(it, L0 + k, cap, ipos, iptr, prev, cursor, lvl, head_of, idx, ctr);
+        if (__syncthreads_count(live ? 1 : 0) == 0) break;
+    }
+}
+__global__ __launch_bounds__(256) void k_runs_open(const unsigned *open, unsigned nopen, const unsigned *cursor, const unsigned *iptr, unsigned *out, unsigned *count) {
+    const unsigned t = blockIdx.x * blockDim.x + threadIdx.x;
+    if (t >= nopen) return;
+    const unsigned it = open ? open[t] : t;
+    if (cursor[it] < iptr[it + 1]) out[atomicAdd(count, 1u)] = it;
+}
+__global__ __launch_bounds__(256) void k_runs_heads(const unsigned *ipos, const unsigned char *idx, long n, unsigned *head) {
+    const long stride = (long)gridDim.x * blockDim.x;
+    for (long j = (long)blockIdx.x * blockDim.x + threadIdx.x; j < n; j += stride) head[j] = idx[ipos[j]] == 0 ? 1u : 0u;
+}
+__global__ __launch_bounds__(256) void k_runs_keys(const unsigned *ipos, const unsigned char *idx, const unsigned *lvl, const unsigned *head, const unsigned *slot, long n,
+                                                   int cap, int order, unsigned *key, unsigned *val) {
+    const long stride = (long)gridDim.x * blockDim.x;
+    for (long j = (long)blockIdx.x * blockDim.x + threadIdx.x; j < n; j += stride) {
+        if (!head[j]) continue;
+        const unsigned p = ipos[j];
+        int len = 1;
+        while (len < cap && j + len < n && idx[ipos[j + len]] == (unsigned char)len) len++;
+        key[slot[j]] = lvl[p] * 8u + (order ? (unsigned)(RUNS_MAX_CAP - len) : 0u);
+        val[slot[j]] = p;
+    }
+}
+__global__ __launch_bounds__(256) void k_runs_rank(const unsigned *key, const unsigned *val, long nunit, unsigned *unit_at, unsigned *level_ptr, unsigned num_levels) {
+    const long stride = (long)gridDim.x * blockDim.x;
+    for (long r = (long)blockIdx.x * blockDim.x + threadIdx.x; r < nunit; r += stride) {
+        unit_at[val[r]] = (unsigned)r;
+        const unsigned l = key[r] >> 3;
+        if (l >= 1u && l <= num_levels && (r == 0 || (key[r - 1] >> 3) != l)) level_ptr[l - 1] = (unsigned)r;
     }
 }
 __global__ __launch_bounds__(256) void k_runs_fill(const unsigned *user, const unsigned *item, const float *label, long n, const unsigned *unit_at,
-                                                   const unsigned *head_of, const unsigned char *idx, long nunit, unsigned *c_item, unsigned *c_user, float *c_label) {
+                                                   const unsigned *head_of, const unsigned char *idx, const RunColumns C, long nunit, int R) {
     const long stride = (long)gridDim.x * blockDim.x;
     for (long p = (long)blockIdx.x * blockDim.x + threadIdx.x; p < n; p += stride) {
         const unsigned un = unit_at[head_of[p]];
         const int j = idx[p];
-        c_user[(size_t)j * (size_t)nunit + un] = user[p];
-        c_label[(size_t)j * (size_t)nunit + un] = label[p];
-        if (j == 0) c_item[un] = item[p];
+        if ((long)un >= nunit || j >= R) continue;
+        C.user[j][un] = user[p];
+        C.label[j][un] = label[p];
+        if (j == 0) C.item[un] = item[p];
     }
 }
 __global__ __launch_bounds__(256) void k_runs_fill_u32(unsigned *v, long n, unsigned x) {
@@ -59,13 +128,33 @@
 void launch_runs_prev(const unsigned *keys, const unsigned *pos, long n, unsigned *prev, hipStream_t st) {
     if (n > 0) hipLaunchKernelGGL(k_runs_prev, dim3(runs_grid(n)), dim3(256), 0, st, keys, pos, n, prev);
 }
-void launch_runs_form(const unsigned *ikeys, const unsigned *ipos, long n, unsigned num_item, const unsigned *prev, int R, unsigned *head, unsigned *head_of,
-                      unsigned char *idx, hipStream_t st) {
-    if (n > 0 && num_item > 0) hipLaunchKernelGGL(k_runs_form, dim3(runs_grid((long)num_item)), dim3(256), 0, st, ikeys, ipos, n, num_item, prev, R, head, head_of, idx);
+void launch_runs_iptr(const unsigned *ikeys, long n, unsigned num_item, unsigned *iptr, unsigned *cursor, hipStream_t st) {
+    hipLaunchKernelGGL(k_runs_iptr, dim3(runs_grid((long)num_item + 1)), dim3(256), 0, st, ikeys, n, num_item, iptr, cursor);
+}
+void launch_runs_peel(const RunsPeel &S, const unsigned *open, unsigned nopen, unsigned L, hipStream_t st) {
+    if (nopen > 0) hipLaunchKernelGGL(k_runs_peel, dim3((nopen + 255) / 256), dim3(256), 0, st, open, nopen, L, S.cap, S.ipos, S.iptr, S.prev, S.cursor, S.lvl, S.head_of, S.idx, S.ctr);
+}
+unsigned runs_peel_narrow_width() { return RUNS_NARROW; }
+void launch_runs_peel_narrow(const RunsPeel &S, const unsigned *open, unsigned nopen, unsigned L0, unsigned iters, hipStream_t st) {
+    if (nopen > 0 && nopen <= RUNS_NARROW)
+        hipLaunchKernelGGL(k_runs_peel_narrow, dim3(1), dim3(RUNS_NARROW), 0, st, open, nopen, L0, iters, S.cap, S.ipos, S.iptr, S.prev, S.cursor, S.lvl, S.head_of, S.idx, S.ctr);
+}
+void launch_runs_open(const RunsPeel &S, const unsigned *open, unsigned nopen, unsigned *out, unsigned *count, hipStream_t st) {
+    if (nopen > 0) hipLaunchKernelGGL(k_runs_open, dim3((nopen + 255) / 256), dim3(256), 0, st, open, nopen, S.cursor, S.iptr, out, count);
+}
+void launch_runs_heads(const unsigned *ipos, const unsigned char *idx, long n, unsigned *head, hipStream_t st) {
+    if (n > 0) hipLaunchKernelGGL(k_runs_heads, dim3(runs_grid(n)), dim3(256), 0, st, ipos, idx, n, head);
+}
+void launch_runs_keys(const unsigned *ipos, const unsigned char *idx, const unsigned *lvl, const unsigned *head, const unsigned *slot, long n, int cap, int order,
+                      unsigned *key, unsigned *val, hipStream_t st) {
+    if (n > 0) hipLaunchKernelGGL(k_runs_keys, dim3(runs_grid(n)), dim3(256), 0, st, ipos, idx, lvl, head, slot, n, cap, order, key, val);
+}
+void launch_runs_rank(const unsigned *key, const unsigned *val, long nunit, unsigned *unit_at, unsigned *level_ptr, unsigned num_levels, hipStream_t st) {
+    if (nunit > 0) hipLaunchKernelGGL(k_runs_rank, dim3(runs_grid(nunit)), dim3(256), 0, st, key, val, nunit, unit_at, level_ptr, num_levels);
 }
 void launch_runs_fill(const unsigned *user, const unsigned *item, const float *label, long n, const unsigned *unit_at, const unsigned *head_of,
-                      const unsigned char *idx, long nunit, unsigned *c_item, unsigned *c_user, float *c_label, hipStream_t st) {
-    if (n > 0) hipLaunchKernelGGL(k_runs_fill, dim3(runs_grid(n)), dim3(256), 0, st, user, item, label, n, unit_at, head_of, idx, nunit, c_item, c_user, c_label);
+                      const unsigned char *idx, const RunColumns &C, long nunit, int R, hipStream_t st) {
+    if (n > 0) hipLaunchKernelGGL(k_runs_fill, dim3(runs_grid(n)), dim3(256), 0, st, user, item, label, n, unit_at, head_of, idx, C, nunit, R);
 }
 __global__ __launch_bounds__(256) void k_runs_iota(unsigned *v, long n) {
     const long stride = (long)gridDim.x * blockDim.x;
@@ -191,6 +280,8 @@
 #define RUNS_BY_R(L_)                                                                                                          \
     if (R == 2) { if (G >= 2) RUNS_LAUNCH(L_, 2, 2); else RUNS_LAUNCH(L_, 2, 1); }       \
     else if (R == 4) { if (G >= 2) RUNS_LAUNCH(L_, 4, 2); else RUNS_LAUNCH(L_, 4, 1); }                                       \
+    else if (R == 5) { if (G >= 2) RUNS_LAUNCH(L_, 5, 2); else RUNS_LAUNCH(L_, 5, 1); }                                       \
+    else if (R == 6) { if (G >= 2) RUNS_LAUNCH(L_, 6, 2); else RUNS_LAUNCH(L_, 6, 1); }                                       \
     else { if (G >= 2) RUNS_LAUNCH(L_, 7, 2); else RUNS_LAUNCH(L_, 7, 1); }
     if (P.k == 128) { RUNS_BY_R(16) } else { RUNS_BY_R(8) }
 #undef RUNS_BY_R
diff --git a/svdfeature_amd/csrc/svdf_kernels.h b/svdfeature_amd/csrc/svdf_kernels.h
--- a/svdfeature_amd/csrc/svdf_kernels.h
+++ b/svdfeature_amd/csrc/svdf_kernels.h
@@ -93,10 +93,25 @@
 long device_exclusive_scan_u32(const unsigned *in, unsigned *out, long n, void **tmp, size_t *tmp_bytes, hipStream_t st);
 void launch_runs_check(const unsigned *user, const unsigned *item, long n, unsigned nu, unsigned ni, unsigned *flag, hipStream_t st);
 void launch_runs_prev(const unsigned *keys, const unsigned *pos, long n, unsigned *prev, hipStream_t st);
-void launch_runs_form(const unsigned *ikeys, const unsigned *ipos, long n, unsigned num_item, const unsigned *prev, int R, unsigned *head, unsigned *head_of,
-                      unsigned char *idx, hipStream_t st);
+void launch_runs_iptr(const unsigned *ikeys, long n, unsigned num_item, unsigned *iptr, unsigned *cursor, hipStream_t st);
+struct RunsPeel {
+    int cap;
+    const unsigned *ipos, *iptr, *prev;
+    unsigned *cursor, *lvl, *head_of;
+    unsigned char *idx;
+    unsigned *ctr;
+};
+void launch_runs_peel(const RunsPeel &S, const unsigned *open, unsigned nopen, unsigned L, hipStream_t st);
+unsigned runs_peel_narrow_width();
+void launch_runs_peel_narrow(const RunsPeel &S, const unsigned *open, unsigned nopen, unsigned L0, unsigned iters, hipStream_t st);
+void launch_runs_open(const RunsPeel &S, const unsigned *open, unsigned nopen, unsigned *out, unsigned *count, hipStream_t st);
+void launch_runs_heads(const unsigned *ipos, const unsigned char *idx, long n, unsigned *head, hipStream_t st);
+void launch_runs_keys(const unsigned *ipos, const unsigned char *idx, const unsigned *lvl, const unsigned *head, const unsigned *slot, long n, int cap, int order,
+                      unsigned *key, unsigned *val, hipStream_t st);
+void launch_runs_rank(const unsigned *key, const unsigned *val, long nunit, unsigned *unit_at, unsigned *level_ptr, unsigned num_levels, hipStream_t st);
+long runs_peel_host(long n, const unsigned *user, const unsigned *item, int cap, int *lvl, int *idx);
 void launch_runs_fill(const unsigned *user, const unsigned *item, const float *label, long n, const unsigned *unit_at, const unsigned *head_of,
-                      const unsigned char *idx, long nunit, unsigned *c_item, unsigned *c_user, float *c_label, hipStream_t st);
+                      const unsigned char *idx, const RunColumns &C, long nunit, int R, hipStream_t st);
 bool pair_units_applies(const DevParams &P);
 void launch_pair_units(const DevParams &P, const PairUnitSchedule &S, long begin, long end, float *out, hipStream_t st);
 void launch_runs_iota(unsigned *v, long n, hipStream_t st);
diff --git a/svdfeature_amd/csrc/svdf_runs.cpp b/svdfeature_amd/csrc/svdf_runs.cpp
--- a/svdfeature_amd/csrc/svdf_runs.cpp
+++ b/svdfeature_amd/csrc/svdf_runs.cpp
@@ -17,63 +17,130 @@
 Dataset *Engine::runs_dataset_from_triples(long n, const unsigned *user, const unsigned *item, const float *label) {
     if (!runs_config_ok() || n < runs_min_rows_ || n >= 0x7FFFFFF0L) return nullptr;
     const int RF = std::max(2, std::min(7, runs_len_));
-    const int R = RF <= 2 ? 2 : (RF <= 4 ? 4 : 7);
+    const int R = RF <= 2 ? 2 : (RF <= 4 ? 4 : RF);
     const unsigned NU = (unsigned)mp_.num_user, NI = (unsigned)mp_.num_item;
     std::unique_ptr<Dataset> ds(new Dataset());
     adopt(ds.get());
-    ds->kind = 10; ds->num_row = n; ds->rn_len = R;
+    ds->kind = 10; ds->num_row = n; ds->rn_len = R; ds->rn_cap = RF; ds->rn_order = runs_order_;
     ds->user.upload(user, (size_t)n, stream_);
     ds->item.upload(item, (size_t)n, stream_);
     ds->label.upload(label, (size_t)n, stream_);
     ds->unit_values = true;
-    DevBuf<unsigned> flag, ka, kb, va, vb, prev, head, head_of, unit_at, c_item, c_user;
-    DevBuf<unsigned char> idx;
-    DevBuf<float> c_label;
-    flag.reserve(4);
-    HIPCHECK(hipMemsetAsync(flag.p, 0, 4 * sizeof(unsigned), stream_));
-    launch_runs_check(ds->user.p, ds->item.p, n, NU, NI, flag.p, stream_);
-    unsigned hflag = 0;
-    HIPCHECK(hipMemcpyAsync(&hflag, flag.p, sizeof(unsigned), hipMemcpyDeviceToHost, stream_));
-    HIPCHECK(hipStreamSynchronize(stream_));
-    if (hflag & 1u) fail("user feature index exceed bound");
-    if (hflag & 2u) fail("item feature index exceed bound");
-    ka.reserve((size_t)n); kb.reserve((size_t)n); va.reserve((size_t)n); vb.reserve((size_t)n);
-    prev.reserve((size_t)n); head.reserve((size_t)n); head_of.reserve((size_t)n); unit_at.reserve((size_t)n); idx.reserve((size_t)n);
+    DevBuf<unsigned> slab;
+    const size_t nw = ((size_t)n + 3) & ~(size_t)3, niw = ((size_t)NI + 4) & ~(size_t)3;
+    slab.reserve(7 * nw + nw / 4 + 4 * niw + 8);
+    unsigned *ka = slab.p, *kb = ka + nw, *va = kb + nw, *vb = va + nw, *prev = vb + nw, *lvl = prev + nw, *head_of = lvl + nw;
+    unsigned char *idx = reinterpret_cast<unsigned char *>(head_of + nw);
+    unsigned *iptr = head_of + nw + nw / 4, *cursor = iptr + niw, *open = cursor + niw, *spare = open + niw, *ctr = spare + niw;
+    HIPCHECK(hipMemsetAsync(ctr, 0, 4 * sizeof(unsigned), stream_));
+    launch_runs_check(ds->user.p, ds->item.p, n, NU, NI, ctr + 3, stream_);
     void *tmp = nullptr;
     size_t tmp_bytes = 0;
     struct FreeTmp { void *&p; ~FreeTmp() { if (p) (void)hipFree(p); } } free_tmp{tmp};
-    HIPCHECK(hipMemcpyAsync(ka.p, ds->user.p, (size_t)n * sizeof(unsigned), hipMemcpyDeviceToDevice, stream_));
-    launch_runs_iota(va.p, n, stream_);
-    device_sort_pairs_u32(ka.p, kb.p, va.p, vb.p, n, &tmp, &tmp_bytes, stream_);
-    launch_runs_prev(kb.p, vb.p, n, prev.p, stream_);
-    HIPCHECK(hipMemcpyAsync(ka.p, ds->item.p, (size_t)n * sizeof(unsigned), hipMemcpyDeviceToDevice, stream_));
-    launch_runs_iota(va.p, n, stream_);
-    device_sort_pairs_u32(ka.p, kb.p, va.p, vb.p, n, &tmp, &tmp_bytes, stream_);
-    launch_runs_form(kb.p, vb.p, n, NI, prev.p, RF, head.p, head_of.p, idx.p, stream_);
-    const long nunit = device_exclusive_scan_u32(head.p, unit_at.p, n, &tmp, &tmp_bytes, stream_);
+    HIPCHECK(hipMemcpyAsync(ka, ds->user.p, (size_t)n * sizeof(unsigned), hipMemcpyDeviceToDevice, stream_));
+    launch_runs_iota(va, n, stream_);
+    device_sort_pairs_u32(ka, kb, va, vb, n, &tmp, &tmp_bytes, stream_);
+    launch_runs_prev(kb, vb, n, prev, stream_);
+    HIPCHECK(hipMemcpyAsync(ka, ds->item.p, (size_t)n * sizeof(unsigned), hipMemcpyDeviceToDevice, stream_));
+    launch_runs_iota(va, n, stream_);
+    device_sort_pairs_u32(ka, kb, va, vb, n, &tmp, &tmp_bytes, stream_);
+    const unsigned *ipos = vb;
+    launch_runs_iptr(kb, n, NI, iptr, cursor, stream_);
+    HIPCHECK(hipMemsetAsync(lvl, 0, (size_t)n * sizeof(unsigned), stream_));
+    RunsPeel S{RF, ipos, iptr, prev, cursor, lvl, head_of, idx, ctr};
+    unsigned hctr[4] = {0u, 0u, 0u, 0u};
+    auto read_ctr = [&]() {
+        HIPCHECK(hipMemcpyAsync(hctr, ctr, 4 * sizeof(unsigned), hipMemcpyDeviceToHost, stream_));
+        HIPCHECK(hipStreamSynchronize(stream_));
+        if (hctr[3] & 1u) fail("user feature index exceed bound");
+        if (hctr[3] & 2u) fail("item feature index exceed bound");
+    };
+    const unsigned *list = nullptr;
+    unsigned nlist = NI, nopen = NI;
+    const unsigned narrow = runs_peel_narrow_width();
+    unsigned L = 0;
+    while (nopen > 0) {
+        check(L < (1u << 28) - 8192u, "dataset_from_triples: more than 2^28 levels of runs");
+        if (nlist <= narrow) { launch_runs_peel_narrow(S, list, nlist, L, 8192u, stream_); L += 8192u; }
+        else for (int b = 0; b < 64; b++) launch_runs_peel(S, list, nlist, ++L, stream_);
+        HIPCHECK(hipGetLastError());
+        read_ctr();
+        nopen = nlist - hctr[0];
+        if (nopen > 0 && (2 * nopen <= nlist || (nopen <= narrow && nlist > narrow))) {
+            HIPCHECK(hipMemsetAsync(ctr + 2, 0, sizeof(unsigned), stream_));
+            launch_runs_open(S, list, nlist, spare, ctr + 2, stream_);
+            HIPCHECK(hipMemsetAsync(ctr, 0, sizeof(unsigned), stream_));
+            list = spare;
+            std::swap(open, spare);
+            nlist = nopen;
+        }
+    }
+    const long num_levels = (long)hctr[1];
+    unsigned *head = ka, *slot = va;
+    launch_runs_heads(ipos, idx, n, head, stream_);
+    const long nunit = device_exclusive_scan_u32(head, slot, n, &tmp, &tmp_bytes, stream_);
+    unsigned *rkey = kb, *rval = prev;
+    launch_runs_keys(ipos, idx, lvl, head, slot, n, RF, runs_order_, rkey, rval, stream_);
+    device_sort_pairs_u32(rkey, ka, rval, va, nunit, &tmp, &tmp_bytes, stream_);
+    unsigned *unit_at = kb, *lptr = prev;
+    launch_runs_rank(ka, va, nunit, unit_at, lptr, (unsigned)num_levels, stream_);
     HIPCHECK(hipGetLastError());
-    c_item.reserve((size_t)nunit); c_user.reserve((size_t)R * (size_t)nunit); c_label.reserve((size_t)R * (size_t)nunit);
-    launch_runs_fill_u32(c_user.p, (long)R * nunit, (unsigned)SLOT_ABSENT, stream_);
-    HIPCHECK(hipMemsetAsync(c_label.p, 0, (size_t)R * (size_t)nunit * sizeof(float), stream_));
-    launch_runs_fill(ds->user.p, ds->item.p, ds->label.p, n, unit_at.p, head_of.p, idx.p, nunit, c_item.p, c_user.p, c_label.p, stream_);
+    ds->rn_item.reserve((size_t)nunit);
+    for (int j = 0; j < R; j++) {
+        ds->rn_user[j].reserve((size_t)nunit); ds->rn_label[j].reserve((size_t)nunit);
+        launch_runs_fill_u32(ds->rn_user[j].p, nunit, (unsigned)SLOT_ABSENT, stream_);
+        HIPCHECK(hipMemsetAsync(ds->rn_label[j].p, 0, (size_t)nunit * sizeof(float), stream_));
+    }
+    RunColumns C;
+    memset(&C, 0, sizeof(C));
+    C.item = ds->rn_item.p;
+    for (int j = 0; j < R; j++) { C.user[j] = ds->rn_user[j].p; C.label[j] = ds->rn_label[j].p; }
+    launch_runs_fill(ds->user.p, ds->item.p, ds->label.p, n, unit_at, head_of, idx, C, nunit, R, stream_);
     HIPCHECK(hipGetLastError());
+    std::vector<unsigned> hl((size_t)num_levels + 1, 0u);
+    if (num_levels > 0) HIPCHECK(hipMemcpyAsync(hl.data(), lptr, (size_t)num_levels * sizeof(unsigned), hipMemcpyDeviceToHost, stream_));
     HIPCHECK(hipStreamSynchronize(stream_));
-    ka.release(); kb.release(); va.release(); vb.release(); prev.release(); head.release(); head_of.release(); unit_at.release(); idx.release();
-    const unsigned *res[SVDF_SCHED_MAX_SLOTS];
-    unsigned off[SVDF_SCHED_MAX_SLOTS], limit[SVDF_SCHED_MAX_SLOTS];
-    const char *msg[SVDF_SCHED_MAX_SLOTS];
-    res[0] = c_item.p; off[0] = NU; limit[0] = NI; msg[0] = "item feature index exceed bound";
-    std::vector<DUCol> du{DUCol{c_item.p, &ds->rn_item}};
-    std::vector<DFCol> df;
-    for (int j = 0; j < R; j++) {
-        res[1 + j] = c_user.p + (size_t)j * (size_t)nunit; off[1 + j] = 0u; limit[1 + j] = NU; msg[1 + j] = "user feature index exceed bound";
-        du.push_back(DUCol{c_user.p + (size_t)j * (size_t)nunit, &ds->rn_user[j]});
-        df.push_back(DFCol{c_label.p + (size_t)j * (size_t)nunit, &ds->rn_label[j]});
-    }
-    schedule_device_columns(ds.get(), nunit, 1 + R, res, off, limit, msg, sort_batches_ == 1 ? c_item.p : nullptr, NI, du, df);
+    hl[(size_t)num_levels] = (unsigned)nunit;
+    Schedule &sc = ds->sched;
+    sc.order.clear();
+    sc.level_ptr.assign(hl.begin(), hl.end());
+    sc.max_level_size = 0;
+    for (long l = 0; l < num_levels; l++) sc.max_level_size = std::max(sc.max_level_size, sc.level_ptr[(size_t)l + 1] - sc.level_ptr[(size_t)l]);
     ds->num_units = nunit;
     ds->algorithmic_bytes = n * (8L * mp_.num_factor * 2 + 8 * 2 + 16 + 8 * 2);
     return ds.release();
+}
+
+long runs_peel_host(long n, const unsigned *user, const unsigned *item, int cap, int *lvl, int *idx) {
+    if (n <= 0) return 0;
+    check(cap >= 1 && cap <= 7, "runs_peel_host: cap must be in 1 .. 7");
+    unsigned nu = 0, ni = 0;
+    for (long p = 0; p < n; p++) { nu = std::max(nu, user[p] + 1u); ni = std::max(ni, item[p] + 1u); }
+    std::vector<long> prev((size_t)n), last((size_t)nu, -1), iptr((size_t)ni + 1, 0), ipos((size_t)n);
+    for (long p = 0; p < n; p++) { prev[(size_t)p] = last[user[p]]; last[user[p]] = p; iptr[(size_t)item[p] + 1]++; }
+    for (unsigned it = 0; it < ni; it++) iptr[(size_t)it + 1] += iptr[it];
+    std::vector<long> cur(iptr.begin(), iptr.end() - 1);
+    for (long p = 0; p < n; p++) ipos[(size_t)cur[item[p]]++] = p;
+    std::copy(iptr.begin(), iptr.end() - 1, cur.begin());
+    std::vector<unsigned> open;
+    for (unsigned it = 0; it < ni; it++) if (cur[it] < iptr[(size_t)it + 1]) open.push_back(it);
+    for (long p = 0; p < n; p++) lvl[p] = 0;
+    long L = 0;
+    while (!open.empty()) {
+        L++;
+        size_t keep = 0;
+        for (unsigned it : open) {
+            int take = 0;
+            while (take < cap && cur[it] < iptr[(size_t)it + 1]) {
+                const long p = ipos[(size_t)cur[it]], pv = prev[(size_t)p];
+                if (pv >= 0 && !(lvl[pv] > 0 && lvl[pv] < L)) break;
+                lvl[p] = (int)L; idx[p] = take; take++; cur[it]++;
+            }
+            if (cur[it] < iptr[(size_t)it + 1]) open[keep++] = it;
+        }
+        open.resize(keep);
+    }
+    return L;
 }
 
 void Engine::runs_train(Dataset *ds) {
diff --git a/svdfeature_amd/csrc/svdf_types.h b/svdfeature_amd/csrc/svdf_types.h
--- a/svdfeature_amd/csrc/svdf_types.h
+++ b/svdfeature_amd/csrc/svdf_types.h
@@ -98,6 +98,8 @@
     const float *label[8];
 };
 
+struct RunColumns { unsigned *item; unsigned *user[8]; float *label[8]; };
+
 struct PairUnit { unsigned user; int begin; int count; int pad; };
 struct PairUnitSchedule {
     const PairUnit *units;
```

After: 5.069 billion instances/s. -12.9%, worse.
